# CZY-Code/PHNet

Hardware: AMD Instinct MI355X
Metric: clips/s (5x3x320x800) fwd+bwd (higher is better)
Workload: dtype f32 storage / accumulation, every product as an EXACT three-term bf16 split (6 bf16 MFMAs, f32-MFMA accuracy); 1 GPU; 5-frame clip 3x320x800, resnet34 + router + lane head, fwd+bwd+AdamW, 1 clip/GPU/step, random-init weights; parallelism=dp1, launch=hipGraph replay of the whole step

## Files before the change

include/phnet_hip.h:

```cpp
#ifndef PHNET_HIP_H
#define PHNET_HIP_H
#include <stdint.h>
#ifdef __cplusplus
extern "C" {
#endif

#define PHNET_OK 0
#define PHNET_ERR_ARG (-1)
#define PHNET_ERR_WORKSPACE (-2)
#define PHNET_ERR_LAUNCH (-3)
#define PHNET_ABI_VERSION 1

int phnet_abi_version(void);

int phnet_lane_nms(const float* rows, const float* scores, const int32_t* counts, int64_t frames,
                   int64_t k_max, int32_t n_offsets, float thresh, int64_t top_k,
                   int64_t* keep, int64_t* num_to_keep, int64_t* parent, void* stream);

int phnet_lane_decode(const float* lines, int64_t frames, int32_t N, int32_t n_offsets, float conf_thresh,
                      float nms_thresh, int64_t top_k, float img_w, uint8_t* keep_mask, int64_t* num,
                      int64_t* keep_c, int64_t* anchors, int64_t* anchors_sorted, float* kept_rows, void* stream);

int phnet_roi_pool_fwd(const float* fmap, const float* xs, const float* ys, float* out, float* out_cp,
                       int32_t B, int32_t N, int32_t P, int32_t h, int32_t w, int32_t C, void* stream);
int phnet_roi_pool_bwd(const float* dout, const float* fmap, const float* xs, const float* ys,
                       float* dmap, float* dxs,
                       int32_t B, int32_t N, int32_t P, int32_t h, int32_t w, int32_t C, void* stream);

int phnet_conv2d_fwd(const float* x, const float* w, const float* bias, float* y,
                     int32_t N, int32_t Hi, int32_t Wi, int32_t Ci, int32_t Co, int32_t R, int32_t S,
                     int32_t stride, int32_t pad, int32_t relu, void* workspace, uint64_t ws_bytes, void* stream);
uint64_t phnet_conv2d_stats_blocks(int64_t M, int32_t Co, int32_t K, uint64_t ws_bytes);
int phnet_conv2d_fwd_fused(const float* x, const float* w, const float* bias, const float* addend, float* y, float* stats,
                           int32_t N, int32_t Hi, int32_t Wi, int32_t Ci, int32_t Co, int32_t R, int32_t S,
                           int32_t stride, int32_t pad, int32_t relu, void* workspace, uint64_t ws_bytes, void* stream);
int phnet_conv2d_dgrad(const float* dy, const float* w, const float* addend, float* dx,
                       int32_t N, int32_t Hi, int32_t Wi, int32_t Ci, int32_t Co, int32_t R, int32_t S,
                       int32_t stride, int32_t pad, void* workspace, uint64_t ws_bytes, void* stream);
int phnet_conv3p_applies(int64_t M, int32_t Ca, int32_t Nn);
uint64_t phnet_conv3p_packed_bytes(int32_t Co, int32_t Ci);
int phnet_conv3p_pack(const float* w, void* packed, int32_t Co, int32_t Ci, int32_t dgrad, void* stream);
int phnet_conv3p_pack_jobs(const void* jobs, int32_t njobs, int64_t total, void* stream);
uint64_t phnet_conv3p_stats_blocks(int64_t M, int32_t Ca, int32_t Nn, uint64_t ws_bytes);
int phnet_conv3p_splits(int64_t M, int32_t Ca, int32_t Nn, uint64_t ws_bytes);
int phnet_conv3p_fwd(const float* x, const void* packed, const float* bias, const float* addend, float* y, float* stats,
                     int32_t N, int32_t H, int32_t W, int32_t Ca, int32_t Nn, int32_t relu,
                     void* workspace, uint64_t ws_bytes, void* stream);
int phnet_conv2d_plan(int64_t M, int32_t Co, int32_t K, uint64_t ws_bytes, int32_t* bm, int32_t* bn, int32_t* splits,
                      int32_t* k_tile);
uint64_t phnet_conv2d_wgrad_workspace(int32_t N, int32_t Hi, int32_t Wi, int32_t Ci, int32_t Co,
                                      int32_t R, int32_t S, int32_t stride, int32_t pad);
int phnet_conv2d_wgrad(const float* dy, const float* x, float* dw, float* dbias,
                       int32_t N, int32_t Hi, int32_t Wi, int32_t Ci, int32_t Co, int32_t R, int32_t S,
                       int32_t stride, int32_t pad, int32_t accumulate, void* workspace, uint64_t ws_bytes, void* stream);
int phnet_linear_bwd_fusable(int64_t M, int64_t K, int64_t N);
int phnet_linear_bwd(const float* dy, const float* x, const float* w, const float* relu_y, float* dx, float* dw, float* dbias,
                     int32_t M, int32_t K, int32_t N, int32_t accumulate, void* stream);
int phnet_nchw3_to_nhwc4(const float* x, float* y, int32_t N, int32_t H, int32_t W, void* stream);
int phnet_pad_channels(const float* src, float* dst, int64_t rows, int32_t cs, int32_t cd, void* stream);

uint64_t phnet_ipc_buffer_bytes(int32_t world, uint64_t max_bytes);
int phnet_ipc_alloc(uint64_t bytes, void** ptr);
int phnet_ipc_free(void* ptr);
int phnet_ipc_get_handle(void* ptr, void* handle64);
int phnet_ipc_open_handle(const void* handle64, void** ptr);
int phnet_ipc_close_handle(void* ptr);
int phnet_oneshot_allreduce(void* data, int32_t count, int32_t dtype, const void* peers, int32_t rank, int32_t world,
                            int32_t cap, void* ctrl, void* stream);

uint64_t phnet_channel_partials_size(int64_t M, int32_t C);
int phnet_bn_fwd_stats(const float* x, int64_t M, int32_t C, float eps, float momentum,
                       const float* gamma, const float* beta, float* running_mean, float* running_var,
                       float* save_mean, float* save_invstd, float* scale, float* shift,
                       float* partial, int32_t training, void* stream);
int phnet_bn_finalize_partials(const float* partial, int64_t nblk, int64_t M, int32_t C, float eps, float momentum,
                               const float* gamma, const float* beta, float* running_mean, float* running_var,
                               float* save_mean, float* save_invstd, float* scale, float* shift, void* stream);
int phnet_bn_apply(const float* x, const float* scale, const float* shift, const float* residual, float* y,
                   int64_t M, int32_t C, int32_t relu, void* stream);
int phnet_bn_bwd(const float* dy, const float* x, const float* y, const float* save_mean,
                 const float* save_invstd, const float* gamma, float* dx, float* dres,
                 float* dgamma, float* dbeta, float* partial, float* c1, float* c2,
                 int64_t M, int32_t C, int32_t relu, int32_t dres_accumulate, int32_t param_accumulate, void* stream);

int phnet_bn_bwd_reduce(const float* dy, const float* x, const float* y, const float* mean, const float* invstd,
                        float* sums, float* partial, float* c1_scratch, float* c2_scratch,
                        int64_t M, int32_t C, int32_t relu, void* stream);
int phnet_bn_bwd_apply(const float* dy, const float* x, const float* y, const float* mean, const float* invstd,
                       const float* gamma, const float* c1, const float* c2, float* dx, float* dres,
                       int64_t M, int32_t C, int32_t relu, int32_t dres_accumulate, void* stream);

int phnet_bn_local_sums(const float* x, int64_t M, int32_t C, float* partial, double* sums, void* stream);
int phnet_bn_partials_to_sums(const float* partial, int64_t nblk, int64_t M, int32_t C, double* sums, void* stream);
int phnet_bn_finalize_sums(const double* sums, int32_t C, float eps, float momentum, const float* gamma, const float* beta,
                           float* running_mean, float* running_var, float* save_mean, float* save_invstd,
                           float* scale, float* shift, void* stream);
int phnet_bn_bwd_apply_sums(const float* dy, const float* x, const float* y, const float* mean, const float* invstd,
                            const float* gamma, const float* sums, const double* count, float* c1, float* c2,
                            float* dx, float* dres, int64_t M, int32_t C, int32_t relu, int32_t dres_accumulate, void* stream);

int phnet_preprocess_u8(const uint8_t* frames, float* out, uint8_t* out_u8,
                        const int32_t* xi, const int16_t* xc, const int32_t* yi, const int16_t* yc,
                        int32_t T, int32_t H0, int32_t W0, int32_t crop_top, int32_t out_h, int32_t out_w, int32_t flip,
                        int32_t layout, const float* mean3_host, const float* std3_host, void* stream);

int phnet_lane_raster(const int32_t* segs, int64_t n_segs, uint32_t* masks, int32_t n_lanes, int32_t height, int32_t width,
                      int32_t lane_width, void* stream);
int phnet_lane_mask_stats(const uint32_t* masks, int32_t n_lanes, int32_t height, int32_t width, const int32_t* pairs,
                          int32_t n_pairs, int64_t* area, int64_t* inter, void* stream);

int phnet_maxpool3x3s2_fwd(const float* x, float* y, uint8_t* argmax, int32_t N, int32_t Hi, int32_t Wi, int32_t C, void* stream);
int phnet_maxpool3x3s2_bwd(const float* dy, const uint8_t* argmax, float* dx, int32_t N, int32_t Hi, int32_t Wi, int32_t C, void* stream);

int phnet_upsample_add(float* fine, const float* coarse, int32_t N, int32_t H, int32_t W, int32_t h, int32_t w, int32_t C, void* stream);
int phnet_upsample_add_bwd(const float* dfine, float* dcoarse, int32_t N, int32_t H, int32_t W, int32_t h, int32_t w, int32_t C, void* stream);

int phnet_layernorm_fwd(const float* x, const float* w, const float* b, const float* res, float* y,
                        float* mean, float* rstd, int64_t rows, int32_t L, float eps, int32_t relu, void* stream);
uint64_t phnet_layernorm_bwd_workspace(int64_t rows, int32_t L);
int phnet_layernorm_bwd(const float* dy, const float* x, const float* y, const float* w,
                        const float* mean, const float* rstd, float* dx, float* dres, float* dw, float* db,
                        int64_t rows, int32_t L, int32_t relu, int32_t param_accumulate,
                        void* workspace, uint64_t ws_bytes, void* stream);

int phnet_dwconv3x3(const float* x, const float* w, const float* bias, float* y,
                    int32_t N, int32_t C, int32_t P, int32_t flip, void* stream);
int phnet_dwconv3x3_wgrad(const float* dy, const float* x, float* dw, float* db,
                          int32_t N, int32_t C, int32_t P, int32_t accumulate, void* stream);

int phnet_lane_assign(const float* pred, const float* tgt, int32_t N, int32_t L, int32_t S,
                      float img_w, float img_h, int64_t* rows_by_col, int64_t* rows_sorted,
                      int32_t* n_valid, float* cost, void* stream);
int phnet_lane_assign_one2many(const float* pred, const float* tgt, int32_t N, int32_t L, int32_t S,
                               float img_w, float img_h, int64_t* rows, int64_t* cols, int32_t* n_pairs, void* stream);
int phnet_lane_assign_tokens(const float* pred, const float* tgt, int32_t N, int32_t L, int32_t S, float img_w, float img_h,
                             int64_t* rows_by_col, int64_t* rows_sorted, const float* feat, int32_t E,
                             float* tokens, uint8_t* valid, void* stream);

int phnet_frame_loss(const float* const* pred, const float* const* gate, const float* tgt,
                     int32_t N, int32_t L, int32_t S, float img_w, float img_h,
                     float cls_w, float reg_w, float iou_w,
                     float liou_half_width, float liou_img_h, float liou_img_w,
                     float* loss, float* const* dpred, float* dgate,
                     int64_t* rows_by_col, int64_t* rows_sorted, float* focal, float* scalars, void* stream);
int phnet_clip_loss(const float* const* pred, const float* const* gate, const float* tgt, int32_t T,
                    int32_t N, int32_t L, int32_t S, float img_w, float img_h,
                    float cls_w, float reg_w, float iou_w,
                    float liou_half_width, float liou_img_h, float liou_img_w,
                    float* loss, float* const* dpred, float* dgate,
                    int64_t* rows_by_col, int64_t* rows_sorted, float* focal, float* scalars, void* stream);
int phnet_frame_loss_variant(int32_t variant, const float* const* pred, const float* const* gate, const float* tgt,
                             int32_t N, int32_t L, int32_t S, float img_w, float img_h,
                             float cls_w, float reg_w, float iou_w,
                             float* loss, float* const* dpred, float* dgate,
                             int64_t* pair_rows, int64_t* pair_cols, int64_t* rows_sorted, float* scratch, void* stream);

int phnet_lane_update_fwd(const float* priors, const float* head, const float* ys, float* preds, float* lines,
                          int32_t N, int32_t S, int32_t HW, float img_w, float img_h, void* stream);
int phnet_lane_update_bwd(const float* dpreds, const float* dlines, const float* lines, const float* head,
                          const float* ys, float* dhead, float* dpriors,
                          int32_t N, int32_t S, int32_t HW, float img_w, float img_h, void* stream);

int phnet_relu_bwd(const float* dy, const float* y, float* dx, int64_t n, void* stream);

uint64_t phnet_gate_stack_saved_floats(int32_t N, int32_t C, int32_t P);
uint64_t phnet_gate_stack_bwd_workspace(int32_t N, int32_t C, int32_t P);
int phnet_gate_stack_fwd(const float* x, const float* const* params, float* out, float* saved,
                         int32_t N, int32_t anchors, int32_t C, int32_t P, float eps, void* stream);
int phnet_gate_stack_bwd(const float* gout, const float* x, const float* out, const float* const* params,
                         const float* saved, float* const* grads, int32_t N, int32_t anchors, int32_t C, int32_t P, float eps,
                         int32_t accumulate, void* workspace, uint64_t ws_bytes, void* stream);
int phnet_gate_wave_applies(int32_t C, int32_t P);
int phnet_gate_wave_partial_planes(int32_t N);
int phnet_gate_wave_fwd(const float* x, const float* const* params, float* out, float* saved,
                        int32_t N, int32_t anchors, float eps, void* stream);
int phnet_gate_wave_bwd(const float* gout, const float* x, const float* out, const float* const* params, const float* saved,
                        float* const* grads, int32_t N, int32_t anchors, float eps, int32_t accumulate,
                        void* workspace, void* stream);

int phnet_attention_fwd(const float* q, const float* k, const float* v, const uint8_t* key_valid, const uint8_t* keep,
                        float* o, float* lse, int32_t B, int32_t Lq, int32_t Lk, int32_t H, int32_t E,
                        int64_t sq, int64_t sk, int64_t sv, int64_t so, float keep_scale,
                        const uint64_t* rng_state, uint64_t rng_call, float drop_p, void* stream);
int phnet_attention_bwd(const float* q, const float* k, const float* v, const float* o, const float* dout,
                        const float* lse, const uint8_t* key_valid, const uint8_t* keep,
                        float* dq, float* dk, float* dv, int32_t B, int32_t Lq, int32_t Lk, int32_t H, int32_t E,
                        int64_t sq, int64_t sk, int64_t sv, int64_t so, int64_t sdq, int64_t sdk, int64_t sdv,
                        float keep_scale, const uint64_t* rng_state, uint64_t rng_call, float drop_p, void* stream);

int phnet_dropout_add(const float* x, const float* res, float* y, int64_t n,
                      const uint64_t* rng_state, uint64_t rng_call, float drop_p, void* stream);
int phnet_gelu_dropout_fwd(const float* x, float* y, int64_t n, const uint64_t* rng_state, uint64_t rng_call, float drop_p,
                           void* stream);
int phnet_gelu_dropout_bwd(const float* dy, const float* x, float* dx, int64_t n, const uint64_t* rng_state,
                           uint64_t rng_call, float drop_p, void* stream);

int phnet_memory_tokens(const float* feat, const int64_t* rows, float* tokens, uint8_t* valid,
                        int32_t B, int32_t N, int32_t E, int32_t L, void* stream);
int phnet_gate_tail_fwd(const float* h, const float* w, const float* b, float* out, int32_t N, int32_t K, void* stream);
int phnet_gate_tail_bwd(const float* dout, const float* out, const float* h, const float* w, float* dh, float* dw, float* db,
                        int32_t N, int32_t K, int32_t accumulate, void* stream);
int phnet_blend_priors(const float* gate, const float* a, const float* b, const int64_t* idx, float* priors, float* on_map,
                       int32_t N, int32_t W, int32_t P, void* stream);

int phnet_gate_v2_fwd(const float* x, const float* w1, const float* s1, const float* t1, const float* w2,
                      const float* s2, const float* t2, const float* wl, const float* bl, float* out,
                      int32_t M, int32_t C, int32_t P, int32_t C1, int32_t C2, void* stream);
int phnet_dyn_bmm_ln_relu_fwd_any(const float* x, const float* w, const float* gamma, const float* beta, float* y,
                                  int32_t N, int32_t P, int32_t K, int32_t J, float eps, void* stream);
int phnet_route_lines(const float* gates, const float* a, const float* b, float* out,
                      int32_t S, int32_t M, int32_t W, int32_t hard, void* stream);

int phnet_rowchain_fwd(const float* in, const float* resid, const float* Wa, const float* ba, const float* ln1w, const float* ln1b,
                       const float* W1, const float* b1, const float* W2, const float* b2, const float* ln2w, const float* ln2b,
                       const float* Wg, const float* bg, float* t_out, float* h_out, float* y_out,
                       int32_t R, int32_t E, int32_t FF, int32_t NG, float eps,
                       const uint64_t* rng_state, uint64_t call_a, uint64_t call_f, uint64_t call_3, float drop_p, void* stream);

uint64_t phnet_tower_layout(int32_t T, int32_t C, const int32_t* head_out, int64_t* offsets, int32_t* hw);
int phnet_assemble_towers(const float* const* params, int32_t T, int32_t C, const int32_t* head_out, float* dst, void* stream);
int phnet_scatter_tower_grads(const float* src, float* const* grads, int32_t T, int32_t C, const int32_t* head_out,
                              int32_t accumulate, void* stream);

int phnet_tower_chain_fwd(const float* x, const float* const* params, int32_t T, int32_t C, const int32_t* head_out,
                          const float* priors, const float* ys, float* preds, float* lines, int32_t R, int32_t S,
                          float img_w, float img_h, void* stream);

int phnet_adamw_step(float* p, const float* g, float* m, float* v, int64_t n, int64_t n_decay, const int64_t* step,
                     float lr, const float* lr_dev, float beta1, float beta2, float eps, float weight_decay, void* stream);

int phnet_dropout_add_ln_fwd(const float* x, const float* res, const float* w, const float* b, float* t, float* h,
                             float* mean, float* rstd, int64_t rows, int32_t L, float eps,
                             const uint64_t* rng_state, uint64_t rng_call, float drop_p, void* stream);
int phnet_dropout_add_ln_bwd(const float* dh, const float* dt, const float* t, const float* w, const float* mean,
                             const float* rstd, float* dres, float* dx, float* dw, float* db,
                             int64_t rows, int32_t L, int32_t param_accumulate,
                             const uint64_t* rng_state, uint64_t rng_call, float drop_p,
                             void* workspace, uint64_t ws_bytes, void* stream);

int phnet_dyn_bmm_ln_relu_fwd(const float* x, const float* w, const float* gamma, const float* beta, float* y,
                              float* stats, int32_t N, int32_t P, int32_t K, int32_t J, float eps, void* stream);
int phnet_dyn_bmm_ln_relu_bwd(const float* dy, const float* x, const float* w, const float* y, const float* stats,
                              const float* gamma, float* dx, float* dw, float* dgamma, float* dbeta,
                              int32_t N, int32_t P, int32_t K, int32_t J, float eps, int32_t param_accumulate,
                              void* workspace, uint64_t ws_bytes, void* stream);
int phnet_dyn_mfma_applies(int32_t P, int32_t K, int32_t J);
int phnet_dyn_mfma_fwd(const float* x, const float* w, const float* gamma, const float* beta, float* y, float* stats,
                       int32_t N, int32_t P, int32_t K, int32_t J, float eps, void* stream);
int phnet_dyn_mfma_bwd(const float* dy, const float* x, const float* w, const float* y, const float* stats, const float* gamma,
                       float* dx, float* dw, float* lnpart, int32_t N, int32_t P, int32_t K, int32_t J, void* stream);

uint64_t phnet_colsum_workspace(int64_t M, int32_t C);
int phnet_colsum(const float* a, float* out, int64_t M, int32_t C, int32_t accumulate, void* workspace, uint64_t ws_bytes, void* stream);

#ifdef __cplusplus
}
#endif
#endif
```

phnet_amd/csrc/conv.hip:

```cpp
#include <type_traits>
#include "igemm.h"
#include "wgrad3s.h"
static constexpr bool g_interleave = true;

using namespace igemm;

namespace {

struct ConvShape {
    int N, Hi, Wi, Ci;
    int Ho, Wo, Co;
    int R, S;
    int stride, pad, in_dil;
    int splits;
    int k_per_split;
};

struct RowCoord { int base, iy0, ix0; bool ok; };

template <int N, int I = 0, typename F>
__device__ __forceinline__ void unroll_iterations(F& f, int t) {
    if constexpr (I < N) {
        f(std::integral_constant<int, I>{}, t + I);
        unroll_iterations<N, I + 1>(f, t);
    }
}
template <int N, int I = 0, typename F>
__device__ __forceinline__ void tail_iterations(F& f, int t, int end) {
    if constexpr (I < N) {
        if (t + I < end) {
            f(std::integral_constant<int, I>{}, t + I);
            tail_iterations<N, I + 1>(f, t, end);
        }
    }
}

template <int BM, int BN, bool B_DGRAD, int BKT, bool UNI, bool AMASK = false, int MMA = 0, int PF = 1, bool BUF = false>
__device__ __forceinline__ void igemm_tile(
    const float* __restrict__ X, const float* __restrict__ W, const float* __restrict__ bias,
    const float* __restrict__ addend, float* __restrict__ out, const ConvShape& g, int relu,
    float* lds, unsigned block, unsigned nblocks, unsigned split, const float* __restrict__ amask = nullptr,
    float* __restrict__ stats = nullptr)
{
    constexpr int TM = BM / 2, TN = BN / 2, FM = TM / 32, FN = TN / 32;
    constexpr int A_PITCH = KContigTile<BM, BKT>::PITCH;
    constexpr int A_FLOATS = KContigTile<BM, BKT>::FLOATS;
    constexpr int B_PITCH = B_DGRAD ? KStridedTile<BN, BKT>::PITCH : KContigTile<BN, BKT>::PITCH;
    constexpr int B_FLOATS = B_DGRAD ? KStridedTile<BN, BKT>::FLOATS : KContigTile<BN, BKT>::FLOATS;
    constexpr int CHUNKS = BKT / 4;
    constexpr int ROWS_PER_PASS = THREADS / CHUNKS;
    constexpr int A_LOADS = BM / ROWS_PER_PASS;
    constexpr int B_LOADS = B_DGRAD ? (BKT * BN / 4) / THREADS : BN / ROWS_PER_PASS;
    float* As = lds;
    float* Bs = lds + 2 * A_FLOATS;
    constexpr bool S3 = MMA == 3;
    typedef KContigPlanes<BM, BKT> AP3;
    typedef KContigPlanes<BN, BKT> BP3C;
    typedef KStridedPlanes<BN, BKT> BP3S;
    constexpr int B3_BYTES = B_DGRAD ? BP3S::BYTES : BP3C::BYTES;
    unsigned char* A3 = reinterpret_cast<unsigned char*>(lds);
    unsigned char* B3 = A3 + 2 * AP3::BYTES;

    const int M = g.N * g.Ho * g.Wo;
    const int K = g.R * g.S * g.Ci;
    const int tiles_n = (g.Co + BN - 1) / BN;
    const unsigned tile = xcd_remap(block, nblocks);
    const int m0 = (int)(tile / tiles_n) * BM, n0 = (int)(tile % tiles_n) * BN;
    const int k_begin = split * g.k_per_split;
    const int k_end = min(K, k_begin + g.k_per_split);
    const int tid = threadIdx.x, lane = tid & 63, wave = tid >> 6;
    const int wm = (wave >> 1) * TM, wn = (wave & 1) * TN;

    RowCoord rc[A_LOADS];
    const int a_chunk = tid % CHUNKS, a_row = tid / CHUNKS;
#pragma unroll
    for (int i = 0; i < A_LOADS; ++i) {
        const int m = m0 + a_row + ROWS_PER_PASS * i;
        rc[i].ok = m < M;
        const int mm = rc[i].ok ? m : 0;
        const int n = mm / (g.Ho * g.Wo), rem = mm - n * (g.Ho * g.Wo);
        const int oy = rem / g.Wo, ox = rem - oy * g.Wo;
        rc[i].base = n * g.Hi * g.Wi;
        rc[i].iy0 = oy * g.stride - g.pad;
        rc[i].ix0 = ox * g.stride - g.pad;
    }

    struct KPos { int c, r, q; };
    auto kpos_init = [&](int k, int ci) {
        KPos p;
        const int rs = k / ci;
        p.c = k - rs * ci;
        p.r = rs / g.S;
        p.q = rs - p.r * g.S;
        return p;
    };
    auto kpos_advance = [&](KPos& p, int ci) {
        p.c += BKT;
        while (p.c >= ci) {
            p.c -= ci;
            if (++p.q == g.S) { p.q = 0; ++p.r; }
        }
    };
    KPos ka = kpos_init(k_begin + a_chunk * 4, g.Ci);
    KPos kb[B_LOADS];
    int b_kk[B_LOADS], b_ch[B_LOADS];
    if (B_DGRAD) {
#pragma unroll
        for (int i = 0; i < B_LOADS; ++i) {
            const int idx = tid + THREADS * i;
            b_kk[i] = idx / (BN / 4);
            b_ch[i] = idx - b_kk[i] * (BN / 4);
            kb[i] = kpos_init(k_begin + b_kk[i], g.Ci);
        }
    }

    constexpr bool uni = UNI;
    int ur = 0, uq = 0, uc0 = 0;
    if (uni) {
        const int rs = k_begin / g.Ci;
        uc0 = k_begin - rs * g.Ci;
        ur = rs / g.S;
        uq = rs - ur * g.S;
    }

    f32x4 a_set[PF][A_LOADS], b_set[PF][B_LOADS];
    f32x4 r_set[PF][AMASK ? A_LOADS : 1];
    unsigned mask_set[PF];
    constexpr unsigned OOB = 0x80000000u;
    int a_off[BUF ? A_LOADS : 1], b_off[BUF ? B_LOADS : 1];
    __amdgpu_buffer_rsrc_t x_rsrc, w_rsrc;
    if constexpr (BUF) {
        static_assert(UNI && !AMASK, "buffer-load path: uniform tap, no ReLU mask");
        x_rsrc = __builtin_amdgcn_make_buffer_rsrc((void*)X, 0, (int)min((long)g.N * g.Hi * g.Wi * g.Ci * 4, (long)0x7fffffff), 0x00020000);
        w_rsrc = __builtin_amdgcn_make_buffer_rsrc((void*)W, 0, (int)min((long)g.Co * K * 4, (long)0x7fffffff), 0x00020000);
#pragma unroll
        for (int i = 0; i < A_LOADS; ++i) {
            a_off[i] = ((rc[i].base + rc[i].iy0 * g.Wi + rc[i].ix0) * g.Ci + a_chunk * 4) * 4;
            if (!rc[i].ok) rc[i].iy0 = -(1 << 28);
        }
#pragma unroll
        for (int i = 0; i < B_LOADS; ++i) {
            if (!B_DGRAD) {
                const int n = n0 + a_row + ROWS_PER_PASS * i;
                b_off[i] = n < g.Co ? (n * K + a_chunk * 4) * 4 : (int)OOB;
            } else {
                const int n = n0 + b_ch[i] * 4;
                b_off[i] = n < g.Co ? (b_kk[i] * g.R * g.S * g.Co + n) * 4 : (int)OOB;
            }
        }
    }
    auto load_global = [&](int kt, f32x4 (&a_reg)[A_LOADS], f32x4 (&b_reg)[B_LOADS], f32x4 (&a_relu)[AMASK ? A_LOADS : 1], unsigned& mask) {
        mask = 0;
        if constexpr (BUF) {
            const bool tile_ok = kt < k_end;
            const int s_tap = ((ur * g.Wi + uq) * g.Ci + uc0) * 4;
#pragma unroll
            for (int i = 0; i < A_LOADS; ++i) {
                const bool ok = tile_ok && (unsigned)(rc[i].iy0 + ur) < (unsigned)g.Hi && (unsigned)(rc[i].ix0 + uq) < (unsigned)g.Wi;
                a_reg[i] = __builtin_bit_cast(f32x4, __builtin_amdgcn_raw_buffer_load_b128(x_rsrc, ok ? a_off[i] + s_tap : (int)OOB, 0, 0));
            }
            int s_b;
            if (!B_DGRAD) s_b = kt * 4;
            else s_b = ((uc0 * g.R + (g.R - 1 - ur)) * g.S + (g.S - 1 - uq)) * g.Co * 4;
#pragma unroll
            for (int i = 0; i < B_LOADS; ++i)
                b_reg[i] = __builtin_bit_cast(f32x4, __builtin_amdgcn_raw_buffer_load_b128(w_rsrc, tile_ok ? b_off[i] + s_b : (int)OOB, 0, 0));
            uc0 += BKT;
            const int wc = uc0 >= g.Ci;
            uc0 = wc ? 0 : uc0;
            uq += wc;
            const int wq = uq == g.S;
            uq = wq ? 0 : uq;
            ur += wq;
            return;
        }
        const int k0 = kt + a_chunk * 4;
        const bool kok = k0 < k_end;
        const int tap_r = uni ? ur : ka.r, tap_q = uni ? uq : ka.q, tap_c = uni ? uc0 + a_chunk * 4 : ka.c;
#pragma unroll
        for (int i = 0; i < A_LOADS; ++i) {
            int ty = rc[i].iy0 + tap_r, tx = rc[i].ix0 + tap_q;
            bool ok = kok && rc[i].ok && ty >= 0 && tx >= 0;
            if (g.in_dil == 2) {
                ok = ok && !((ty | tx) & 1);
                ty >>= 1; tx >>= 1;
            }
            ok = ok && ty < g.Hi && tx < g.Wi;
            const int pix = ok ? rc[i].base + ty * g.Wi + tx : 0;
            a_reg[i] = *reinterpret_cast<const f32x4*>(X + (size_t)pix * g.Ci + (kok ? tap_c : 0));
            if (AMASK) a_relu[i] = *reinterpret_cast<const f32x4*>(amask + (size_t)pix * g.Ci + (kok ? tap_c : 0));
            mask |= (unsigned)ok << i;
        }
        if (!uni) kpos_advance(ka, g.Ci);
        if (!B_DGRAD) {
#pragma unroll
            for (int i = 0; i < B_LOADS; ++i) {
                const int n = n0 + a_row + ROWS_PER_PASS * i;
                const bool ok = kok && n < g.Co;
                b_reg[i] = *reinterpret_cast<const f32x4*>(W + (size_t)(ok ? n : 0) * K + (kok ? k0 : 0));
                mask |= (unsigned)ok << (16 + i);
            }
        } else {
#pragma unroll
            for (int i = 0; i < B_LOADS; ++i) {
                const int k = kt + b_kk[i], n = n0 + b_ch[i] * 4;
                const bool ok = k < k_end && n < g.Co;
                const int wc = uni ? uc0 + b_kk[i] : kb[i].c, wr = uni ? ur : kb[i].r, wq = uni ? uq : kb[i].q;
                const int wrow = ok ? (wc * g.R + (g.R - 1 - wr)) * g.S + (g.S - 1 - wq) : 0;
                b_reg[i] = *reinterpret_cast<const f32x4*>(W + (size_t)wrow * g.Co + (ok ? n : 0));
                mask |= (unsigned)ok << (16 + i);
                if (!uni) kpos_advance(kb[i], g.Ci);
            }
        }
        if (uni) {
            uc0 += BKT;
            const int wc = uc0 >= g.Ci;
            uc0 = wc ? 0 : uc0;
            uq += wc;
            const int wq = uq == g.S;
            uq = wq ? 0 : uq;
            ur += wq;
        }
    };
    auto store_lds = [&](int buf, const f32x4 (&a_reg)[A_LOADS], const f32x4 (&b_reg)[B_LOADS], const f32x4 (&a_relu)[AMASK ? A_LOADS : 1],
                         unsigned mask) {
        float* a = As + buf * A_FLOATS;
        float* b = Bs + buf * B_FLOATS;
        unsigned char* a3 = A3 + buf * AP3::BYTES;
        unsigned char* b3 = B3 + buf * B3_BYTES;
        const f32x4 zero{0.f, 0.f, 0.f, 0.f};
#pragma unroll
        for (int i = 0; i < A_LOADS; ++i) {
            f32x4 v = BUF ? a_reg[i] : ((mask >> i) & 1u ? a_reg[i] : zero);
            if (AMASK) {
                v.x = a_relu[i].x > 0.f ? v.x : 0.f; v.y = a_relu[i].y > 0.f ? v.y : 0.f;
                v.z = a_relu[i].z > 0.f ? v.z : 0.f; v.w = a_relu[i].w > 0.f ? v.w : 0.f;
            }
            if (S3) store_split3<AP3::PLANE>(a3, (a_row + ROWS_PER_PASS * i) * AP3::PITCH + a_chunk * 8, v);
            else
            *reinterpret_cast<f32x4*>(a + (a_row + ROWS_PER_PASS * i) * A_PITCH + a_chunk * 4) = v;
        }
        if (!B_DGRAD) {
#pragma unroll
            for (int i = 0; i < B_LOADS; ++i) {
                const f32x4 v = BUF ? b_reg[i] : ((mask >> (16 + i)) & 1u ? b_reg[i] : zero);
                if (S3) store_split3<BP3C::PLANE>(b3, (a_row + ROWS_PER_PASS * i) * BP3C::PITCH + a_chunk * 8, v);
                else *reinterpret_cast<f32x4*>(b + (a_row + ROWS_PER_PASS * i) * B_PITCH + a_chunk * 4) = v;
            }
        } else {
#pragma unroll
            for (int i = 0; i < B_LOADS; ++i) {
                const f32x4 v = BUF ? b_reg[i] : ((mask >> (16 + i)) & 1u ? b_reg[i] : zero);
                if (S3) store_split3<BP3S::PLANE>(b3, b_kk[i] * BP3S::PITCH + b_ch[i] * 8, v);
                else *reinterpret_cast<f32x4*>(b + b_kk[i] * B_PITCH + b_ch[i] * 4) = v;
            }
        }
    };

    const bool final_pass = g.splits == 1;
    f32x16 acc[FM][FN];
#pragma unroll
    for (int j = 0; j < FN; ++j) {
        const int n = n0 + wn + j * 32 + frag_col(lane);
        const bool nok = n < g.Co;
        const float bv = (final_pass && bias && nok) ? bias[n] : 0.f;
#pragma unroll
        for (int i = 0; i < FM; ++i)
#pragma unroll
            for (int e = 0; e < 16; ++e) {
                const int m = m0 + wm + i * 32 + frag_row(lane, e);
                const bool ok = final_pass && addend && nok && m < M;
                acc[i][j][e] = bv + (ok ? addend[(size_t)(ok ? m : 0) * g.Co + (ok ? n : 0)] : 0.f);
            }
    }

    auto multiply_tile = [&](int buf, int kt) {
        if (S3) {
#pragma unroll
            for (int ks = 0; ks < BKT / BK; ++ks) {
                Frag3 a[FM], b[FN];
                read_kcontig3<FM, AP3::PITCH, AP3::PLANE>(A3 + buf * AP3::BYTES + wm * AP3::PITCH, lane, ks, a);
                if (!B_DGRAD) read_kcontig3<FN, BP3C::PITCH, BP3C::PLANE>(B3 + buf * B3_BYTES + wn * BP3C::PITCH, lane, ks, b);
                else read_kstrided3<FN, BP3S::PITCH, BP3S::PLANE>(B3 + buf * B3_BYTES + wn * 2, lane, ks, b);
                mma3_step<FM, FN>(a, b, acc);
            }
            return;
        }
#pragma unroll
        for (int ks = 0; ks < BKT / BK; ++ks) {
            if (BKT > BK && kt + ks * BK >= k_end) break;
            float a[FM][8], b[FN][8];
            read_kcontig<FM, A_PITCH>(As + buf * A_FLOATS + wm * A_PITCH, lane, ks, a);
            if (!B_DGRAD) read_kcontig<FN, B_PITCH>(Bs + buf * B_FLOATS + wn * B_PITCH, lane, ks, b);
            else read_kstrided<FN, B_PITCH>(Bs + buf * B_FLOATS + wn, lane, ks, b);
            mma_any<S3 ? 0 : MMA, FM, FN>(a, b, acc);
        }
    };

    if (k_begin < k_end) {
        const int ntiles = (k_end - k_begin + BKT - 1) / BKT;
#pragma unroll
        for (int d = 0; d < PF; ++d) load_global(k_begin + d * BKT, a_set[d], b_set[d], r_set[d], mask_set[d]);
        store_lds(0, a_set[0], b_set[0], r_set[0], mask_set[0]);
        __syncthreads();
        int buf = 0;
        auto iteration = [&](auto U, int tt) {
            constexpr int u = decltype(U)::value;
            load_global(k_begin + (tt + PF) * BKT, a_set[u], b_set[u], r_set[u], mask_set[u]);
            multiply_tile(buf, k_begin + tt * BKT);
            if (PF == 1) __builtin_amdgcn_sched_barrier(0);
            constexpr int v = (u + 1) % PF;
            store_lds(buf ^ 1, a_set[v], b_set[v], r_set[v], mask_set[v]);
            if (PF > 1 && S3 && g_interleave) {
#pragma unroll
                for (int i = 0; i < 6 * FM * FN * (BKT / BK); ++i) {
                    __builtin_amdgcn_sched_group_barrier(0x008, 1, 0);
                    __builtin_amdgcn_sched_group_barrier(0x002, (14 + FM * FN - 1) / (FM * FN), 0);
                }
            }
            __syncthreads();
            buf ^= 1;
        };
        int t = 0;
        for (; t + PF <= ntiles; t += PF) unroll_iterations<PF>(iteration, t);
        if (PF > 1) tail_iterations<PF - 1>(iteration, t, ntiles);
    }

    if (stats != nullptr && final_pass) {
#pragma unroll
        for (int j = 0; j < FN; ++j) {
            const int n = n0 + wn + j * 32 + frag_col(lane);
#pragma unroll
            for (int i = 0; i < FM; ++i) {
                float sm = 0.f, sq = 0.f;
#pragma unroll
                for (int e = 0; e < 16; ++e) { const float v = acc[i][j][e]; sm += v; sq += v * v; }
                sm += __shfl_xor(sm, 32, 64);
                sq += __shfl_xor(sq, 32, 64);
                if (lane < 32 && n < g.Co) {
                    float* p = stats + (size_t)((m0 + wm + i * 32) >> 5) * 2 * g.Co;
                    p[n] = sm;
                    p[g.Co + n] = sq;
                }
            }
        }
    }

    float* dst = out + (size_t)split * M * g.Co;
#pragma unroll
    for (int j = 0; j < FN; ++j) {
        const int n = n0 + wn + j * 32 + frag_col(lane);
        if (n >= g.Co) continue;
#pragma unroll
        for (int i = 0; i < FM; ++i)
#pragma unroll
            for (int e = 0; e < 16; ++e) {
                const int m = m0 + wm + i * 32 + frag_row(lane, e);
                if (m < M) dst[(size_t)m * g.Co + n] = (final_pass && relu) ? fmaxf(acc[i][j][e], 0.f) : acc[i][j][e];
            }
    }
}

template <int BM, int BN, bool B_DGRAD, int BKT, bool UNI, int MMA = 0, int PF = 1, bool BUF = false>
__global__ __launch_bounds__(THREADS) void conv_igemm_kernel(
    const float* __restrict__ X, const float* __restrict__ W, const float* __restrict__ bias,
    const float* __restrict__ addend, float* __restrict__ out, ConvShape g, int relu, float* __restrict__ stats)
{
    extern __shared__ __attribute__((aligned(16))) float lds[];
    igemm_tile<BM, BN, B_DGRAD, BKT, UNI, false, MMA, PF, BUF>(X, W, bias, addend, out, g, relu, lds, blockIdx.x, gridDim.x, blockIdx.z,
                                                               nullptr, stats);
}

constexpr int T3_AROWS = 66;
int g_taps3 = 1;
template <bool DGRAD>
__global__ __launch_bounds__(THREADS) void conv3x3s1_kernel(
    const float* __restrict__ X, const float* __restrict__ Wt, const float* __restrict__ bias,
    const float* __restrict__ addend, float* __restrict__ out, ConvShape g, int relu, float* __restrict__ stats)
{
    constexpr int APITCH = KContigPlanes<64, 16>::PITCH;
    constexpr int APLANE = T3_AROWS * APITCH, AIMG = 3 * APLANE;
    typedef KContigPlanes<64, 16> BP3C;
    typedef KStridedPlanes<64, 16> BP3S;
    constexpr int BIMG = DGRAD ? BP3S::BYTES : BP3C::BYTES;
    constexpr int BPLANE = DGRAD ? BP3S::PLANE : BP3C::PLANE;
    extern __shared__ __attribute__((aligned(16))) float lds[];
    unsigned char* A3 = reinterpret_cast<unsigned char*>(lds);
    unsigned char* B3 = A3 + 2 * AIMG;
    unsigned char* dump = B3 + 2 * BIMG;

    const int W = g.Wi, H = g.Hi, Ca = g.Ci;
    const int M = g.N * H * W, K = 9 * Ca;
    const int CC = Ca >> 4;
    const int tiles_n = (g.Co + 63) >> 6;
    const unsigned tile = xcd_remap(blockIdx.x, gridDim.x);
    const int m0 = (int)(tile / tiles_n) * 64, n0 = (int)(tile % tiles_n) * 64;
    const int u_begin = blockIdx.z * g.k_per_split, u_end = min(3 * CC, u_begin + g.k_per_split);
    const int tid = threadIdx.x, lane = tid & 63, wave = tid >> 6;
    const int wm = (wave >> 1) * 32, wn = (wave & 1) * 32;

    constexpr unsigned OOB = 0x80000000u;
    __amdgpu_buffer_rsrc_t x_rsrc = __builtin_amdgcn_make_buffer_rsrc((void*)X, 0, (int)min((long)M * Ca * 4, (long)0x7fffffff), 0x00020000);
    __amdgpu_buffer_rsrc_t w_rsrc = __builtin_amdgcn_make_buffer_rsrc((void*)Wt, 0, (int)min((long)g.Co * K * 4, (long)0x7fffffff), 0x00020000);
    int a_off[2], a_ok[2], a_lds[2];
#pragma unroll
    for (int i = 0; i < 2; ++i) {
        const int idx = tid + 256 * i, row = idx >> 2, chunk = idx & 3;
        const bool rowok = idx < 4 * T3_AROWS;
        const int t = m0 - 1 + row;
        const bool tok = rowok && (unsigned)t < (unsigned)M;
        const int tt = tok ? t : 0;
        const int y = (tt / W) % H;
        a_ok[i] = (tok && y >= 1 ? 1 : 0) | (tok ? 2 : 0) | (tok && y + 1 < H ? 4 : 0);
        a_off[i] = (t * Ca + chunk * 4) * 4;
        a_lds[i] = rowok ? row * APITCH + chunk * 8 : -1;
    }
    const int a_row = tid >> 2, a_chunk = tid & 3;
    const int b_kk = tid >> 4, b_ch = tid & 15;
    int b_off, b_lds;
    if (!DGRAD) {
        const int n = n0 + a_row;
        b_off = n < g.Co ? (n * K + a_chunk * 4) * 4 : (int)OOB;
        b_lds = a_row * BP3C::PITCH + a_chunk * 8;
    } else {
        const int n = n0 + b_ch * 4;
        b_off = n < g.Co ? (b_kk * 9 * g.Co + n) * 4 : (int)OOB;
        b_lds = b_kk * BP3S::PITCH + b_ch * 8;
    }
    int la_dy = u_begin / CC, la_cc = u_begin - la_dy * CC, la_u = u_begin;
    int lb_dy = la_dy, lb_cc = la_cc, lb_u = u_begin, lb_dx = 0;
    const bool wave0 = __builtin_amdgcn_readfirstlane(wave) == 0;
    auto load_a = [&](f32x4 (&reg)[2]) {
        const bool uok = la_u < u_end;
        const int s_a = ((la_dy - 1) * W * Ca + la_cc * 16) * 4;
        {
            const bool ok = uok && ((a_ok[0] >> la_dy) & 1);
            reg[0] = __builtin_bit_cast(f32x4, __builtin_amdgcn_raw_buffer_load_b128(x_rsrc, ok ? a_off[0] + s_a : (int)OOB, 0, 0));
        }
        if (wave0) {
            const bool ok = uok && ((a_ok[1] >> la_dy) & 1);
            reg[1] = __builtin_bit_cast(f32x4, __builtin_amdgcn_raw_buffer_load_b128(x_rsrc, ok ? a_off[1] + s_a : (int)OOB, 0, 0));
        }
        ++la_u; ++la_cc;
        const int wrap = la_cc == CC;
        la_cc = wrap ? 0 : la_cc;
        la_dy += wrap;
    };
    auto load_b = [&](f32x4& reg) {
        const bool uok = lb_u < u_end;
        const int s_b = !DGRAD ? ((lb_dy * 3 + lb_dx) * Ca + lb_cc * 16) * 4
                               : ((lb_cc * 16 * 3 + (2 - lb_dy)) * 3 + (2 - lb_dx)) * g.Co * 4;
        reg = __builtin_bit_cast(f32x4, __builtin_amdgcn_raw_buffer_load_b128(w_rsrc, uok ? b_off + s_b : (int)OOB, 0, 0));
        ++lb_dx;
        const int w3 = lb_dx == 3;
        lb_dx = w3 ? 0 : lb_dx;
        lb_u += w3; lb_cc += w3;
        const int wrap = lb_cc == CC;
        lb_cc = wrap ? 0 : lb_cc;
        lb_dy += wrap;
    };
    auto store_a = [&](int aoff, const f32x4 (&reg)[2]) {
        store_split3<APLANE>(A3 + aoff, a_lds[0], reg[0]);
        if (wave0) {
            unsigned h0, m0_, l0, h1, m1, l1;
            split3_pair(reg[1].x, reg[1].y, h0, m0_, l0);
            split3_pair(reg[1].z, reg[1].w, h1, m1, l1);
            const bool has = a_lds[1] >= 0;
            unsigned char* q = has ? A3 + aoff + a_lds[1] : dump + lane * 8;
            const int ps = has ? APLANE : 512;
            *reinterpret_cast<u32x2*>(q) = (u32x2){h0, h1};
            *reinterpret_cast<u32x2*>(q + ps) = (u32x2){m0_, m1};
            *reinterpret_cast<u32x2*>(q + 2 * ps) = (u32x2){l0, l1};
        }
    };
    auto store_b = [&](int boff, const f32x4& reg) { store_split3<BPLANE>(B3 + boff, b_lds, reg); };

    const bool final_pass = g.splits == 1;
    f32x16 acc[1][1];
    {
        const int n = n0 + wn + frag_col(lane);
        const bool nok = n < g.Co;
        const float bv = (final_pass && bias && nok) ? bias[n] : 0.f;
#pragma unroll
        for (int e = 0; e < 16; ++e) {
            const int m = m0 + wm + frag_row(lane, e);
            const bool ok = final_pass && addend && nok && m < M;
            acc[0][0][e] = bv + (ok ? addend[(size_t)(ok ? m : 0) * g.Co + (ok ? n : 0)] : 0.f);
        }
    }
    const int pr = m0 + wm + (lane & 31);
    const int px = (pr < M ? pr : 0) % W;
    const bool edge_l = px == 0, edge_r = px == W - 1;
    const bool any_l = __builtin_amdgcn_ballot_w64(edge_l) != 0, any_r = __builtin_amdgcn_ballot_w64(edge_r) != 0;

    if (u_begin < u_end) {
        f32x4 a_reg[2], b_set[3];
        load_a(a_reg);
#pragma unroll
        for (int d = 0; d < 3; ++d) load_b(b_set[d]);
        store_a(0, a_reg);
        load_a(a_reg);
        store_b(0, b_set[0]);
        load_b(b_set[0]);
        __syncthreads();
        int aoff = 0, boff = 0;
        const int r = lane & 31, hb = (lane >> 5) * 16;
        auto step = [&](auto DX) {
            constexpr int dxi = decltype(DX)::value;
            {
                Frag3 a[1], b[1];
                {
                    const unsigned char* p = A3 + aoff + (wm + r + dxi) * APITCH + hb;
                    a[0].hi = *reinterpret_cast<const bf16x8*>(p);
                    a[0].mid = *reinterpret_cast<const bf16x8*>(p + APLANE);
                    a[0].lo = *reinterpret_cast<const bf16x8*>(p + 2 * APLANE);
                }
                if (!DGRAD) read_kcontig3<1, BP3C::PITCH, BP3C::PLANE>(B3 + boff + wn * BP3C::PITCH, lane, 0, b);
                else read_kstrided3<1, BP3S::PITCH, BP3S::PLANE>(B3 + boff + wn * 2, lane, 0, b);
                if (dxi != 1 && (dxi == 0 ? any_l : any_r)) {
                    const bool z = dxi == 0 ? edge_l : edge_r;
                    typedef unsigned u32x4 __attribute__((ext_vector_type(4)));
                    const u32x4 keep = z ? (u32x4){0u, 0u, 0u, 0u} : (u32x4){~0u, ~0u, ~0u, ~0u};
                    a[0].hi = __builtin_bit_cast(bf16x8, __builtin_bit_cast(u32x4, a[0].hi) & keep);
                    a[0].mid = __builtin_bit_cast(bf16x8, __builtin_bit_cast(u32x4, a[0].mid) & keep);
                    a[0].lo = __builtin_bit_cast(bf16x8, __builtin_bit_cast(u32x4, a[0].lo) & keep);
                }
                mma3_step<1, 1>(a, b, acc);
                store_b(boff ^ BIMG, b_set[(dxi + 1) % 3]);
                load_b(b_set[(dxi + 1) % 3]);
                if (dxi == 2) {
                    store_a(aoff ^ AIMG, a_reg);
                    load_a(a_reg);
                }
#pragma unroll
                for (int i = 0; i < 6; ++i) {
                    __builtin_amdgcn_sched_group_barrier(0x008, 1, 0);
                    __builtin_amdgcn_sched_group_barrier(0x002, dxi == 2 ? 14 : 8, 0);
                }
                __syncthreads();
                boff ^= BIMG;
            }
        };
        for (int u = u_begin; u < u_end; ++u) {
            step(std::integral_constant<int, 0>{});
            step(std::integral_constant<int, 1>{});
            step(std::integral_constant<int, 2>{});
            aoff ^= AIMG;
        }
    }

    if (stats != nullptr && final_pass) {
        const int n = n0 + wn + frag_col(lane);
        float sm = 0.f, sq = 0.f;
#pragma unroll
        for (int e = 0; e < 16; ++e) { const float v = acc[0][0][e]; sm += v; sq += v * v; }
        sm += __shfl_xor(sm, 32, 64);
        sq += __shfl_xor(sq, 32, 64);
        if (lane < 32 && n < g.Co) {
            float* p = stats + (size_t)((m0 + wm) >> 5) * 2 * g.Co;
            p[n] = sm;
            p[g.Co + n] = sq;
        }
    }
    float* dst = out + (size_t)blockIdx.z * M * g.Co;
    const int n = n0 + wn + frag_col(lane);
    if (n < g.Co) {
#pragma unroll
        for (int e = 0; e < 16; ++e) {
            const int m = m0 + wm + frag_row(lane, e);
            if (m < M) dst[(size_t)m * g.Co + n] = (final_pass && relu) ? fmaxf(acc[0][0][e], 0.f) : acc[0][0][e];
        }
    }
}

__global__ __launch_bounds__(256) void splitk_reduce_kernel(const float* __restrict__ part, float* __restrict__ out,
                                                            const float* __restrict__ bias, const float* __restrict__ addend,
                                                            long total4, int ncols, int splits, int relu, int accumulate,
                                                            float* __restrict__ stats)
{
    __shared__ f32x4 red_s[2][256];
    const long i = (long)blockIdx.x * blockDim.x + threadIdx.x;
    if (stats != nullptr) {
        const bool ok = i < total4;
        f32x4 s{0.f, 0.f, 0.f, 0.f};
        if (ok) {
            const f32x4* p = reinterpret_cast<const f32x4*>(part) + i;
            s = p[0];
            for (int z = 1; z < splits; ++z) s += p[(long)z * total4];
            reinterpret_cast<f32x4*>(out)[i] = s;
        }
        red_s[0][threadIdx.x] = s;
        red_s[1][threadIdx.x] = s * s;
        __syncthreads();
        const int c4 = ncols >> 2;
        if ((int)threadIdx.x < c4) {
            f32x4 a = red_s[0][threadIdx.x], b = red_s[1][threadIdx.x];
            for (int r = c4; r < 256; r += c4) { a += red_s[0][r + threadIdx.x]; b += red_s[1][r + threadIdx.x]; }
            float* q = stats + (size_t)blockIdx.x * 2 * ncols + threadIdx.x * 4;
            *reinterpret_cast<f32x4*>(q) = a;
            *reinterpret_cast<f32x4*>(q + ncols) = b;
        }
        return;
    }
    if (i >= total4) return;
    const f32x4* p = reinterpret_cast<const f32x4*>(part) + i;
    const f32x4 zero{0.f, 0.f, 0.f, 0.f};
    f32x4 v[8];
#pragma unroll
    for (int z = 0; z < 8; ++z) v[z] = p[(long)min(z, splits - 1) * total4];
    const f32x4 bv = bias ? *reinterpret_cast<const f32x4*>(bias + (int)((i * 4) % ncols)) : zero;
    const f32x4 av = addend ? reinterpret_cast<const f32x4*>(addend)[i] : zero;
    const f32x4 ov = accumulate ? reinterpret_cast<const f32x4*>(out)[i] : zero;
    f32x4 s = v[0];
#pragma unroll
    for (int z = 1; z < 8; ++z)
        if (z < splits) s += v[z];
    for (int z = 8; z < splits; ++z) s += p[(long)z * total4];
    if (bias) s += bv;
    if (addend) s += av;
    if (relu) { s.x = fmaxf(s.x, 0.f); s.y = fmaxf(s.y, 0.f); s.z = fmaxf(s.z, 0.f); s.w = fmaxf(s.w, 0.f); }
    if (accumulate) s += ov;
    reinterpret_cast<f32x4*>(out)[i] = s;
}

struct WgradShape {
    int N, Hi, Wi, Ci;
    int Ho, Wo, Co;
    int R, S, stride, pad;
    int splits, pix_per_split;
};

template <int BM, int BN, int MMA = 0, int BKW = BK, int PF = 1, bool BUF = false>
__global__ __launch_bounds__(THREADS) void conv_wgrad_kernel(
    const float* __restrict__ dY, const float* __restrict__ X, float* __restrict__ out, float* __restrict__ dbias,
    WgradShape g, int want_bias, int accumulate)
{
    constexpr int TM = BM / 2, TN = BN / 2, FM = TM / 32, FN = TN / 32;
    constexpr int A_PITCH = KStridedTile<BM, BKW>::PITCH, B_PITCH = KStridedTile<BN, BKW>::PITCH;
    constexpr int A_FLOATS = KStridedTile<BM, BKW>::FLOATS, B_FLOATS = KStridedTile<BN, BKW>::FLOATS;
    constexpr int A_LOADS = BKW * BM / 4 / THREADS, B_LOADS = BKW * BN / 4 / THREADS;
    constexpr bool S3 = MMA == 3;
    typedef KStridedPlanes<BM, BKW> AP3;
    typedef KStridedPlanes<BN, BKW> BP3;
    constexpr int LDS_BYTES = S3 ? 2 * (AP3::BYTES + BP3::BYTES) : 2 * (A_FLOATS + B_FLOATS) * 4;
    __shared__ __attribute__((aligned(16))) unsigned char lds_raw[LDS_BYTES];
    float* lds = reinterpret_cast<float*>(lds_raw);
    float* As = lds;
    float* Bs = lds + 2 * A_FLOATS;
    unsigned char* A3 = lds_raw;
    unsigned char* B3 = lds_raw + 2 * AP3::BYTES;

    const int NC = g.R * g.S * g.Ci;
    const int P = g.N * g.Ho * g.Wo;
    const int tiles_n = (NC + BN - 1) / BN;
    const unsigned tile = xcd_remap(blockIdx.x, gridDim.x);
    const int m0 = (int)(tile / tiles_n) * BM, n0 = (int)(tile % tiles_n) * BN;
    const int p_begin = blockIdx.z * g.pix_per_split, p_end = min(P, p_begin + g.pix_per_split);
    const int tid = threadIdx.x, lane = tid & 63, wave = tid >> 6;
    const int wm = (wave >> 1) * TM, wn = (wave & 1) * TN;

    int b_kk[B_LOADS], b_col[B_LOADS], b_r[B_LOADS], b_q[B_LOADS], b_c[B_LOADS];
    bool b_ok[B_LOADS];
#pragma unroll
    for (int i = 0; i < B_LOADS; ++i) {
        const int idx = tid + THREADS * i;
        b_kk[i] = idx / (BN / 4);
        b_col[i] = (idx - b_kk[i] * (BN / 4)) * 4;
        const int col = n0 + b_col[i];
        b_ok[i] = col < NC;
        const int rs = b_ok[i] ? col / g.Ci : 0;
        b_c[i] = col - rs * g.Ci;
        b_r[i] = rs / g.S;
        b_q[i] = rs - b_r[i] * g.S;
    }

    int b_n[B_LOADS], b_oy[B_LOADS], b_ox[B_LOADS];
#pragma unroll
    for (int i = 0; i < B_LOADS; ++i) {
        const int pp = min(p_begin + b_kk[i], max(P - 1, 0));
        b_n[i] = pp / (g.Ho * g.Wo);
        const int rem = pp - b_n[i] * (g.Ho * g.Wo);
        b_oy[i] = rem / g.Wo;
        b_ox[i] = rem - b_oy[i] * g.Wo;
    }
    int a_kk[A_LOADS], a_ch[A_LOADS];
#pragma unroll
    for (int i = 0; i < A_LOADS; ++i) {
        const int idx = tid + THREADS * i;
        a_kk[i] = idx / (BM / 4);
        a_ch[i] = (idx - a_kk[i] * (BM / 4)) * 4;
    }

    f32x4 a_set[PF][A_LOADS], b_set[PF][B_LOADS], bsum[A_LOADS];
    unsigned m_set[PF];
#pragma unroll
    for (int i = 0; i < A_LOADS; ++i) bsum[i] = f32x4{0.f, 0.f, 0.f, 0.f};
    constexpr unsigned OOB = 0x80000000u;
    __amdgpu_buffer_rsrc_t y_rsrc, x_rsrc;
    int a_off[BUF ? A_LOADS : 1];
    float inv_wo = 0.f, inv_ho = 0.f;
    if constexpr (BUF) {
        y_rsrc = __builtin_amdgcn_make_buffer_rsrc((void*)dY, 0, (int)min((long)P * g.Co * 4, (long)0x7fffffff), 0x00020000);
        x_rsrc = __builtin_amdgcn_make_buffer_rsrc((void*)X, 0, (int)min((long)g.N * g.Hi * g.Wi * g.Ci * 4, (long)0x7fffffff), 0x00020000);
#pragma unroll
        for (int i = 0; i < A_LOADS; ++i) a_off[i] = m0 + a_ch[i] < g.Co ? (a_kk[i] * g.Co + m0 + a_ch[i]) * 4 : (int)OOB;
        inv_wo = 1.0f / (float)g.Wo; inv_ho = 1.0f / (float)g.Ho;
    }
    const bool bias_block = want_bias && n0 == 0;
    auto load_global = [&](int pt, bool advance, f32x4 (&a_reg)[A_LOADS], f32x4 (&b_reg)[B_LOADS], unsigned& lmask) {
        lmask = 0;
        if (advance) {
#pragma unroll
            for (int i = 0; i < B_LOADS; ++i) {
                if constexpr (BUF) {
                    int ox = b_ox[i] + BKW;
                    int w = (int)((float)ox * inv_wo);
                    ox -= w * g.Wo;
                    const int lo = ox < 0, hi = ox >= g.Wo;
                    ox += lo ? g.Wo : 0; ox -= hi ? g.Wo : 0; w += hi - lo;
                    int oy = b_oy[i] + w;
                    int v = (int)((float)oy * inv_ho);
                    oy -= v * g.Ho;
                    const int lo2 = oy < 0, hi2 = oy >= g.Ho;
                    oy += lo2 ? g.Ho : 0; oy -= hi2 ? g.Ho : 0; v += hi2 - lo2;
                    b_ox[i] = ox; b_oy[i] = oy; b_n[i] += v;
                } else {
                    b_ox[i] += BKW;
                    while (b_ox[i] >= g.Wo) {
                        b_ox[i] -= g.Wo;
                        if (++b_oy[i] == g.Ho) { b_oy[i] = 0; ++b_n[i]; }
                    }
                }
            }
        }
        if constexpr (BUF) {
            const int s_a = pt * g.Co * 4;
#pragma unroll
            for (int i = 0; i < A_LOADS; ++i) {
                const bool ok = pt + a_kk[i] < p_end;
                a_reg[i] = __builtin_bit_cast(f32x4, __builtin_amdgcn_raw_buffer_load_b128(y_rsrc, ok ? a_off[i] + s_a : (int)OOB, 0, 0));
            }
#pragma unroll
            for (int i = 0; i < B_LOADS; ++i) {
                const int iy = b_oy[i] * g.stride - g.pad + b_r[i], ix = b_ox[i] * g.stride - g.pad + b_q[i];
                const bool ok = b_ok[i] && pt + b_kk[i] < p_end && (unsigned)iy < (unsigned)g.Hi && (unsigned)ix < (unsigned)g.Wi;
                const int off = (((b_n[i] * g.Hi + iy) * g.Wi + ix) * g.Ci + b_c[i]) * 4;
                b_reg[i] = __builtin_bit_cast(f32x4, __builtin_amdgcn_raw_buffer_load_b128(x_rsrc, ok ? off : (int)OOB, 0, 0));
            }
            return;
        }
#pragma unroll
        for (int i = 0; i < A_LOADS; ++i) {
            const int p = pt + a_kk[i], co = m0 + a_ch[i];
            const bool ok = p < p_end && co < g.Co;
            a_reg[i] = *reinterpret_cast<const f32x4*>(dY + (ok ? (size_t)p * g.Co + co : 0));
            lmask |= (unsigned)ok << i;
        }
#pragma unroll
        for (int i = 0; i < B_LOADS; ++i) {
            const int p = pt + b_kk[i];
            const int iy = b_oy[i] * g.stride - g.pad + b_r[i], ix = b_ox[i] * g.stride - g.pad + b_q[i];
            const bool ok = b_ok[i] && p < p_end && iy >= 0 && iy < g.Hi && ix >= 0 && ix < g.Wi;
            const int pix = ok ? (b_n[i] * g.Hi + iy) * g.Wi + ix : 0;
            b_reg[i] = *reinterpret_cast<const f32x4*>(X + (size_t)pix * g.Ci + (ok ? b_c[i] : 0));
            lmask |= (unsigned)ok << (16 + i);
        }
    };
    auto store_lds = [&](int buf, const f32x4 (&a_reg)[A_LOADS], const f32x4 (&b_reg)[B_LOADS], unsigned lmask) {
        const f32x4 zero{0.f, 0.f, 0.f, 0.f};
#pragma unroll
        for (int i = 0; i < A_LOADS; ++i) {
            const f32x4 v = BUF ? a_reg[i] : ((lmask >> i) & 1u ? a_reg[i] : zero);
            if (bias_block) bsum[i] += v;
            if (S3) store_split3<AP3::PLANE>(A3 + buf * AP3::BYTES, a_kk[i] * AP3::PITCH + a_ch[i] * 2, v);
            else *reinterpret_cast<f32x4*>(As + buf * A_FLOATS + a_kk[i] * A_PITCH + a_ch[i]) = v;
        }
#pragma unroll
        for (int i = 0; i < B_LOADS; ++i) {
            const f32x4 v = BUF ? b_reg[i] : ((lmask >> (16 + i)) & 1u ? b_reg[i] : zero);
            if (S3) store_split3<BP3::PLANE>(B3 + buf * BP3::BYTES, b_kk[i] * BP3::PITCH + b_col[i] * 2, v);
            else *reinterpret_cast<f32x4*>(Bs + buf * B_FLOATS + b_kk[i] * B_PITCH + b_col[i]) = v;
        }
    };

    const bool from_old = g.splits == 1 && accumulate;
    f32x16 acc[FM][FN];
#pragma unroll
    for (int i = 0; i < FM; ++i)
#pragma unroll
        for (int j = 0; j < FN; ++j)
#pragma unroll
            for (int e = 0; e < 16; ++e) {
                const int n = n0 + wn + j * 32 + frag_col(lane), m = m0 + wm + i * 32 + frag_row(lane, e);
                const bool ok = from_old && n < NC && m < g.Co;
                const float v = out[ok ? (size_t)m * NC + n : 0];
                acc[i][j][e] = ok ? v : 0.f;
            }

    if (p_begin < p_end) {
        const int nsteps = (p_end - p_begin + BKW - 1) / BKW;
#pragma unroll
        for (int d = 0; d < PF; ++d) load_global(p_begin + d * BKW, d > 0, a_set[d], b_set[d], m_set[d]);
        store_lds(0, a_set[0], b_set[0], m_set[0]);
        __syncthreads();
        int buf = 0;
        auto iteration = [&](auto U, int tt) {
            constexpr int u = decltype(U)::value;
            load_global(p_begin + (tt + PF) * BKW, true, a_set[u], b_set[u], m_set[u]);
#pragma unroll
            for (int ks = 0; ks < BKW / BK; ++ks) {
                if (S3) {
                    Frag3 a[FM], b[FN];
                    read_kstrided3<FM, AP3::PITCH, AP3::PLANE>(A3 + buf * AP3::BYTES + wm * 2, lane, ks, a);
                    read_kstrided3<FN, BP3::PITCH, BP3::PLANE>(B3 + buf * BP3::BYTES + wn * 2, lane, ks, b);
                    mma3_step<FM, FN>(a, b, acc);
                } else {
                    float a[FM][8], b[FN][8];
                    read_kstrided<FM, A_PITCH>(As + buf * A_FLOATS + wm, lane, ks, a);
                    read_kstrided<FN, B_PITCH>(Bs + buf * B_FLOATS + wn, lane, ks, b);
                    mma_any<S3 ? 0 : MMA, FM, FN>(a, b, acc);
                }
            }
            if (PF == 1) __builtin_amdgcn_sched_barrier(0);
            constexpr int v = (u + 1) % PF;
            store_lds(buf ^ 1, a_set[v], b_set[v], m_set[v]);
            if (PF > 1 && S3 && g_interleave) {
#pragma unroll
                for (int i = 0; i < 6 * FM * FN * (BKW / BK); ++i) {
                    __builtin_amdgcn_sched_group_barrier(0x008, 1, 0);
                    __builtin_amdgcn_sched_group_barrier(0x002, (14 + FM * FN - 1) / (FM * FN), 0);
                }
            }
            __syncthreads();
            buf ^= 1;
        };
        int t = 0;
        for (; t + PF <= nsteps; t += PF) unroll_iterations<PF>(iteration, t);
        if (PF > 1) tail_iterations<PF - 1>(iteration, t, nsteps);
    }
    const bool direct = g.splits == 1;
    float* dst = direct ? out : out + (size_t)blockIdx.z * ((size_t)g.Co * NC + g.Co);
#pragma unroll
    for (int j = 0; j < FN; ++j) {
        const int n = n0 + wn + j * 32 + frag_col(lane);
        if (n >= NC) continue;
#pragma unroll
        for (int i = 0; i < FM; ++i)
#pragma unroll
            for (int e = 0; e < 16; ++e) {
                const int m = m0 + wm + i * 32 + frag_row(lane, e);
                if (m < g.Co) {
                    float* q = dst + (size_t)m * NC + n;
                    *q = acc[i][j][e];
                }
            }
    }
    if (bias_block) {
        __syncthreads();
#pragma unroll
        for (int i = 0; i < A_LOADS; ++i)
            *reinterpret_cast<f32x4*>(As + a_kk[i] * A_PITCH + a_ch[i]) = bsum[i];
        __syncthreads();
        if (tid < BM && m0 + tid < g.Co) {
            float t = 0.f;
#pragma unroll
            for (int k = 0; k < BKW; ++k) t += As[k * A_PITCH + tid];
            if (direct) dbias[m0 + tid] = accumulate ? dbias[m0 + tid] + t : t;
            else dst[(size_t)g.Co * NC + m0 + tid] = t;
        }
    }
}

constexpr int W3_THREADS = 768;
int g_wgrad3 = 1, g_wgrad3_target = 256;
int g_wgrad3_bkw = 16;
// ... 109 lines not shown
            read_kstrided3<1, PITCH, PLANE>(b_src + buf_off, lane, ks, b1);
        };
        const int h8 = (lane >> 5) * 8;
        auto mask_edge = [&](Frag3& a, int ke) {
            const int j = ke - h8;
            const int ji = j >> 1;
            const unsigned wmask = (j & 1) ? 0x0000ffffu : 0xffff0000u;
            typedef unsigned u32x4 __attribute__((ext_vector_type(4)));
            u32x4 m;
            m.x = ji == 0 ? wmask : 0xffffffffu; m.y = ji == 1 ? wmask : 0xffffffffu;
            m.z = ji == 2 ? wmask : 0xffffffffu; m.w = ji == 3 ? wmask : 0xffffffffu;
            a.hi = __builtin_bit_cast(bf16x8, __builtin_bit_cast(u32x4, a.hi) & m);
            a.mid = __builtin_bit_cast(bf16x8, __builtin_bit_cast(u32x4, a.mid) & m);
            a.lo = __builtin_bit_cast(bf16x8, __builtin_bit_cast(u32x4, a.lo) & m);
        };
        read_frags(0, 0, fa[0], fb[0]);
        int o_cur = 0, o_nxt = 2 * IMG, o_st = 4 * IMG;
        auto iteration = [&](auto U, int tt) {
            constexpr int u = decltype(U)::value;
            constexpr int slot = (u + 2) % PF;
#pragma unroll
            for (int ks = 0; ks < NSUB; ++ks) {
                const int cur = (u * NSUB + ks) & 1, nxt = cur ^ 1;
                {
                    const int ke = dx < 0 ? (mx == 0 ? 0 : W - mx) : W - 1 - mx;
                    if (dx != 0 && ke < BK) mask_edge(fa[cur], ke);
                    mx += BK;
                    mx -= mx >= W ? W : 0;
                }
                if (ks + 1 < NSUB) read_frags(o_cur, ks + 1, fa[nxt], fb[nxt]);
                else read_frags(o_nxt, 0, fa[nxt], fb[nxt]);
                Frag3 (&a)[1] = *reinterpret_cast<Frag3 (*)[1]>(&fa[cur]);
                Frag3 (&b)[1] = *reinterpret_cast<Frag3 (*)[1]>(&fb[cur]);
                mma3_step<1, 1>(a, b, acc);
            }
            store_lds(o_st, set[slot]);
            load_global(p_begin + (tt + 2 + PF) * BKW, set[slot]);
#pragma unroll
            for (int i = 0; i < 6; ++i) {
                __builtin_amdgcn_sched_group_barrier(0x008, 1, 0);
                __builtin_amdgcn_sched_group_barrier(0x002, 8, 0);
            }
            __syncthreads();
            const int o = o_cur; o_cur = o_nxt; o_nxt = o_st; o_st = o;
        };
        int t = 0;
        for (; t + PF <= nsteps; t += PF) unroll_iterations<PF>(iteration, t);
        if (PF > 1) tail_iterations<PF - 1>(iteration, t, nsteps);
    }
    const bool direct = g.splits == 1;
    float* dst = direct ? out : out + (size_t)blockIdx.z * ((size_t)g.Co * NC + g.Co);
#pragma unroll
    for (int e = 0; e < 16; ++e)
        dst[(size_t)(m0 + wm + frag_row(lane, e)) * NC + n_base + frag_col(lane)] = acc[0][0][e];
    if (bias_block) {
        float* fold = reinterpret_cast<float*>(lds_raw);
        __syncthreads();
        if (role_a) *reinterpret_cast<f32x4*>(fold + kk * 68 + col) = bsum;
        __syncthreads();
        if (tid < 64) {
            float tsum = 0.f;
#pragma unroll
            for (int k = 0; k < BK; ++k) tsum += fold[k * 68 + tid];
            if (direct) dbias[m0 + tid] = accumulate ? dbias[m0 + tid] + tsum : tsum;
            else dst[(size_t)g.Co * NC + m0 + tid] = tsum;
        }
    }
}

constexpr int SMALLP_MAX = 256;
template <int BM, int BN, bool AMASK = false, int MMA = 0>
__device__ __forceinline__ void smallp_tile(
    const float* __restrict__ dY, const float* __restrict__ X, float* __restrict__ dw, float* __restrict__ dbias,
    int P, int Co, int Ci, int want_bias, int accumulate, float* lds, unsigned block, unsigned nblocks,
    const float* __restrict__ ymask = nullptr)
{
    constexpr int TM = BM / 2, TN = BN / 2, FM = TM / 32, FN = TN / 32;
    constexpr int AP = BM + 4, BP = BN + 4;
    constexpr int A_CH = BM / 4, B_CH = BN / 4;
    constexpr int A_LOADS = SMALLP_MAX * A_CH / THREADS, B_LOADS = SMALLP_MAX * B_CH / THREADS;
    const int P16 = (P + 15) & ~15;
    float* As = lds;
    float* Bs = lds + P16 * AP;
    const int tiles_n = (Ci + BN - 1) / BN;
    const unsigned tile = xcd_remap(block, nblocks);
    const int m0 = (int)(tile / tiles_n) * BM, n0 = (int)(tile % tiles_n) * BN;
    const int tid = threadIdx.x, lane = tid & 63, wave = tid >> 6;
    const int wm = (wave >> 1) * TM, wn = (wave & 1) * TN;

    f32x4 ar[A_LOADS], br[B_LOADS], ay[AMASK ? A_LOADS : 1];
    unsigned am = 0, bm = 0;
#pragma unroll
    for (int i = 0; i < A_LOADS; ++i) {
        const int idx = tid + THREADS * i, p = idx / A_CH, m = m0 + (idx - p * A_CH) * 4;
        const bool ok = p < P && m < Co;
        ar[i] = *reinterpret_cast<const f32x4*>(dY + (ok ? (size_t)p * Co + m : 0));
        if (AMASK) ay[i] = *reinterpret_cast<const f32x4*>(ymask + (ok ? (size_t)p * Co + m : 0));
        am |= (unsigned)ok << i;
    }
#pragma unroll
    for (int i = 0; i < B_LOADS; ++i) {
        const int idx = tid + THREADS * i, p = idx / B_CH, n = n0 + (idx - p * B_CH) * 4;
        const bool ok = p < P && n < Ci;
        br[i] = *reinterpret_cast<const f32x4*>(X + (ok ? (size_t)p * Ci + n : 0));
        bm |= (unsigned)ok << i;
    }
    f32x16 acc[FM][FN];
#pragma unroll
    for (int j = 0; j < FN; ++j)
#pragma unroll
        for (int i = 0; i < FM; ++i)
#pragma unroll
            for (int e = 0; e < 16; ++e) {
                const int n = n0 + wn + j * 32 + frag_col(lane), m = m0 + wm + i * 32 + frag_row(lane, e);
                acc[i][j][e] = (accumulate && n < Ci && m < Co) ? dw[(size_t)m * Ci + n] : 0.f;
            }
    const f32x4 zero{0.f, 0.f, 0.f, 0.f};
#pragma unroll
    for (int i = 0; i < A_LOADS; ++i) {
        const int idx = tid + THREADS * i, p = idx / A_CH;
        f32x4 v = (am >> i) & 1u ? ar[i] : zero;
        if (AMASK) {
            v.x = ay[i].x > 0.f ? v.x : 0.f; v.y = ay[i].y > 0.f ? v.y : 0.f;
            v.z = ay[i].z > 0.f ? v.z : 0.f; v.w = ay[i].w > 0.f ? v.w : 0.f;
        }
        if (p < P16) *reinterpret_cast<f32x4*>(As + p * AP + (idx - p * A_CH) * 4) = v;
    }
#pragma unroll
    for (int i = 0; i < B_LOADS; ++i) {
        const int idx = tid + THREADS * i, p = idx / B_CH;
        if (p < P16) *reinterpret_cast<f32x4*>(Bs + p * BP + (idx - p * B_CH) * 4) = (bm >> i) & 1u ? br[i] : zero;
    }
    __syncthreads();

    for (int ks = 0; ks < P16 / BK; ++ks) {
        float a[FM][8], b[FN][8];
        read_kstrided<FM, AP>(As + wm, lane, ks, a);
        read_kstrided<FN, BP>(Bs + wn, lane, ks, b);
        mma_any<MMA, FM, FN>(a, b, acc);
    }
#pragma unroll
    for (int j = 0; j < FN; ++j) {
        const int n = n0 + wn + j * 32 + frag_col(lane);
        if (n >= Ci) continue;
#pragma unroll
        for (int i = 0; i < FM; ++i)
#pragma unroll
            for (int e = 0; e < 16; ++e) {
                const int m = m0 + wm + i * 32 + frag_row(lane, e);
                if (m < Co) dw[(size_t)m * Ci + n] = acc[i][j][e];
            }
    }
    if (want_bias && n0 == 0) {
        static_assert(BM == 64, "bias fold assumes 64 columns x 4 row groups");
        const int c = tid & 63, grp = tid >> 6;
        float t = 0.f;
#pragma unroll 4
        for (int p = grp; p < P16; p += 4) t += As[p * AP + c];
        __syncthreads();
        Bs[grp * 64 + c] = t;
        __syncthreads();
        if (tid < 64 && m0 + tid < Co) {
            const float v = (Bs[tid] + Bs[64 + tid]) + (Bs[128 + tid] + Bs[192 + tid]);
            dbias[m0 + tid] = accumulate ? dbias[m0 + tid] + v : v;
        }
    }
}

template <int BM, int BN, int MMA = 0>
__global__ __launch_bounds__(THREADS) void linear_wgrad_smallp_kernel(
    const float* __restrict__ dY, const float* __restrict__ X, float* __restrict__ dw, float* __restrict__ dbias,
    int P, int Co, int Ci, int want_bias, int accumulate)
{
    extern __shared__ __attribute__((aligned(16))) float lds[];
    smallp_tile<BM, BN, false, MMA>(dY, X, dw, dbias, P, Co, Ci, want_bias, accumulate, lds, blockIdx.x, gridDim.x);
}

template <bool UNI, bool AMASK, int MMA = 0>
__global__ __launch_bounds__(THREADS) void linear_bwd_fused_kernel(
    const float* __restrict__ dY, const float* __restrict__ W, const float* __restrict__ X, const float* __restrict__ ymask,
    float* __restrict__ dX, float* __restrict__ dw, float* __restrict__ dbias,
    ConvShape gd, unsigned dgrad_tiles, int P, int Co, int Ci, int want_bias, int accumulate)
{
    extern __shared__ __attribute__((aligned(16))) float lds[];
    if (blockIdx.x < dgrad_tiles)
        igemm_tile<64, 64, true, 64, UNI, AMASK, MMA>(dY, W, nullptr, nullptr, dX, gd, 0, lds, blockIdx.x, dgrad_tiles, 0, ymask);
    else
        smallp_tile<64, 64, AMASK, MMA>(dY, X, dw, dbias, P, Co, Ci, want_bias, accumulate, lds, blockIdx.x - dgrad_tiles,
                                   gridDim.x - dgrad_tiles, ymask);
}

__global__ __launch_bounds__(256) void wgrad_reduce_kernel(const float* __restrict__ part, float* __restrict__ dw,
                                                           float* __restrict__ dbias, long nw, long nb, int splits, int accumulate)
{
    __shared__ f32x4 red[3][64];
    const int lane = threadIdx.x & 63, zg = threadIdx.x >> 6;
    const long total4 = (nw + nb) >> 2;
    const long i4 = (long)blockIdx.x * 64 + lane;
    const bool ok = i4 < total4;
    const long i = i4 * 4;
    const bool is_w = i < nw;
    const bool writer = zg == 0 && ok && (is_w || dbias);
    const f32x4 zero{0.f, 0.f, 0.f, 0.f};
    f32x4 old = zero;
    if (writer && accumulate) {
        if (is_w) old = *reinterpret_cast<const f32x4*>(dw + i);
        else { const float* b = dbias + (i - nw); old = f32x4{b[0], b[1], b[2], b[3]}; }
    }
    const f32x4* p = reinterpret_cast<const f32x4*>(part) + (ok ? i4 : 0);
    f32x4 s = zero;
    int z = zg;
    for (; z + 12 < splits; z += 16) {
        const f32x4 v0 = p[(long)z * total4], v1 = p[(long)(z + 4) * total4], v2 = p[(long)(z + 8) * total4],
                    v3 = p[(long)(z + 12) * total4];
        s += v0; s += v1; s += v2; s += v3;
    }
    for (; z < splits; z += 4) s += p[(long)z * total4];
    if (zg) red[zg - 1][lane] = s;
    __syncthreads();
    if (writer) {
        const f32x4 t = old + ((s + red[0][lane]) + (red[1][lane] + red[2][lane]));
        if (is_w) *reinterpret_cast<f32x4*>(dw + i) = t;
        else { float* b = dbias + (i - nw); b[0] = t.x; b[1] = t.y; b[2] = t.z; b[3] = t.w; }
    }
}

__global__ void nchw3_to_nhwc4_kernel(const float* __restrict__ x, float* __restrict__ y, int N, int HW)
{
    const long i = (long)blockIdx.x * blockDim.x + threadIdx.x;
    if (i >= (long)N * HW) return;
    const long n = i / HW, p = i - n * HW;
    const float* s = x + n * 3 * (long)HW + p;
    reinterpret_cast<f32x4*>(y)[i] = f32x4{s[0], s[HW], s[2 * (long)HW], 0.f};
}

__global__ void pad_channels_kernel(const float* __restrict__ src, float* __restrict__ dst, long rows, int cs, int cd)
{
    const long i = (long)blockIdx.x * blockDim.x + threadIdx.x;
    if (i >= rows * cd) return;
    const long r = i / cd;
    const int c = (int)(i - r * cd);
    dst[i] = c < cs ? src[r * cs + c] : 0.f;
}

struct TileChoice { int bm, bn; };

int g_mma_mode = 3;
int g_buf_loads = 1;
int g_pf = 4;
int g_deep_kt3 = 64;

TileChoice pick_tile(long M, long N)
{
    if (g_mma_mode == 3 && M <= 2048) return {64, 64};
    if (g_mma_mode >= 1) {
        if (N >= 128 && ceil_div64(M, 128) * ceil_div64(N, 128) >= 300) return {128, 128};
        if (ceil_div64(M, 128) * ceil_div64(N, 64) >= 1250) return {128, 64};
    }
    return {64, 64};
}

struct ConvPlan { int bm, bn, splits; long tiles; };

int k_tile_for(long M, int K, int ci, int bm, int bn)
{
    if (M <= (g_mma_mode == 3 ? 256 : 2048) && K >= 64) return (g_mma_mode == 3 && g_deep_kt3 == 32) ? 32 : 64;
    if (g_mma_mode == 3) return BK;
    if (g_mma_mode >= 1 && bm == 64 && bn == 64 && ci % 32 == 0) return 32;
    return BK;
}

int g_force_bm = 0, g_force_bn = 0, g_force_splits = 0;
int g_force_kt = 0;
int g_uniform_tap = 1;
int g_wgrad_bm128 = 1, g_wgrad_target = 768;
int g_wgrad_bkw = 16;
int g_wgrad_smallp = 1;
int g_smallp_max_tiles = 400;

ConvPlan plan_conv(long M, int Co, int K, bool has_ws, size_t ws_bytes)
{
    TileChoice t = pick_tile(M, Co);
    if (g_force_bm) {
        t = {g_force_bm, g_force_bn};
        ConvPlan f{t.bm, t.bn, 1, ceil_div64(M, t.bm) * ceil_div64(Co, t.bn)};
        int splits = g_force_splits > 0 ? g_force_splits : 1;
        while (splits > 1 && (!has_ws || (size_t)splits * M * Co * sizeof(float) > ws_bytes)) --splits;
        f.splits = splits;
        return f;
    }
    ConvPlan p{t.bm, t.bn, 1, ceil_div64(M, t.bm) * ceil_div64(Co, t.bn)};
    const bool deep = M <= (g_mma_mode == 3 ? 256 : 2048) && K >= 64;
    if (has_ws && p.tiles < (deep ? 400 : 900)) {
        int splits = (int)min((long)8, max((long)1, (1250 + p.tiles / 2) / p.tiles));
        while (splits > 1 && K / splits < 256) --splits;
        while (splits > 1 && (size_t)splits * M * Co * sizeof(float) > ws_bytes) --splits;
        p.splits = splits;
    }
    return p;
}

template <bool DGRAD>
int launch_conv(const float* X, const float* W, const float* bias, const float* addend, float* out, float* workspace,
                size_t ws_bytes, ConvShape g, int relu, hipStream_t st, float* stats = nullptr)
{
    const long M = (long)g.N * g.Ho * g.Wo;
    const int K = g.R * g.S * g.Ci;
    const ConvPlan t = plan_conv(M, g.Co, K, workspace != nullptr, ws_bytes);
    const long tiles = t.tiles;
    const int splits = t.splits;
    g.splits = splits;
    float* dst = splits > 1 ? workspace : out;
    dim3 grid((unsigned)tiles, 1, (unsigned)splits);
    const int bkt = g_force_kt ? g_force_kt : k_tile_for(M, K, g.Ci, t.bm, t.bn);
    const int ksteps = (K + bkt - 1) / bkt;
    g.k_per_split = ((ksteps + splits - 1) / splits) * bkt;
#define PHNET_LAUNCH_CONV___(BM_, BN_, BKT_, UNI_, MMA_, PF_)                                                           \
    do {                                                                                                                \
        if (UNI_ && g.in_dil == 1 && g_buf_loads && MMA_ == 3) PHNET_LAUNCH_CONV____(BM_, BN_, BKT_, UNI_, MMA_, PF_, UNI_); \
        else PHNET_LAUNCH_CONV____(BM_, BN_, BKT_, UNI_, MMA_, PF_, false);                                             \
    } while (0)
#define PHNET_LAUNCH_CONV____(BM_, BN_, BKT_, UNI_, MMA_, PF_, BUF_)                                                    \
    do {                                                                                                                \
        constexpr size_t lds_ = MMA_ == 3                                                                               \
            ? 2 * (size_t)(KContigPlanes<BM_, BKT_>::BYTES +                                                            \
                           (DGRAD ? KStridedPlanes<BN_, BKT_>::BYTES : KContigPlanes<BN_, BKT_>::BYTES))                \
            : 2 * (size_t)(KContigTile<BM_, BKT_>::FLOATS +                                                             \
                           (DGRAD ? KStridedTile<BN_, BKT_>::FLOATS : KContigTile<BN_, BKT_>::FLOATS)) * 4;             \
        static bool attr_set_ = false;                                                                                  \
        if (lds_ > 64 * 1024 && !attr_set_) {                                                                           \
            (void)hipFuncSetAttribute((const void*)conv_igemm_kernel<BM_, BN_, DGRAD, BKT_, UNI_, MMA_, PF_, BUF_>,     \
                                hipFuncAttributeMaxDynamicSharedMemorySize, (int)lds_);                                 \
            attr_set_ = true;                                                                                           \
        }                                                                                                               \
        hipLaunchKernelGGL((conv_igemm_kernel<BM_, BN_, DGRAD, BKT_, UNI_, MMA_, PF_, BUF_>), grid, dim3(THREADS), lds_, st, \
                           X, W, bias, addend, dst, g, relu, splits > 1 ? (float*)nullptr : stats);                     \
    } while (0)
#define PHNET_LAUNCH_CONV__(BM_, BN_, BKT_, UNI_, MMA_) PHNET_LAUNCH_CONV___(BM_, BN_, BKT_, UNI_, MMA_, 1)
#define PHNET_LAUNCH_CONV_(BM_, BN_, BKT_, UNI_)                                                                        \
    do {                                                                                                                \
        if (g_mma_mode == 1) PHNET_LAUNCH_CONV__(BM_, BN_, BKT_, UNI_, 1);                                              \
        else if (g_mma_mode == 2) PHNET_LAUNCH_CONV__(BM_, BN_, BKT_, UNI_, 2);                                         \
        else if (g_mma_mode == 3 && g_pf == 4) PHNET_LAUNCH_CONV___(BM_, BN_, BKT_, UNI_, 3, 4);                        \
        else if (g_mma_mode == 3 && g_pf == 2) PHNET_LAUNCH_CONV___(BM_, BN_, BKT_, UNI_, 3, 2);                        \
        else if (g_mma_mode == 3) PHNET_LAUNCH_CONV___(BM_, BN_, BKT_, UNI_, 3, 1);                                     \
        else if (g_pf == 4) PHNET_LAUNCH_CONV___(BM_, BN_, BKT_, UNI_, 0, 4);                                           \
        else PHNET_LAUNCH_CONV__(BM_, BN_, BKT_, UNI_, 0);                                                              \
    } while (0)
#define PHNET_LAUNCH_CONV(BM_, BN_, UNI_)                                                                               \
    do {                                                                                                                \
        if (bkt == 64) PHNET_LAUNCH_CONV_(BM_, BN_, 64, UNI_);                                                          \
        else if (bkt == 32) PHNET_LAUNCH_CONV_(BM_, BN_, 32, UNI_);                                                     \
        else PHNET_LAUNCH_CONV_(BM_, BN_, 16, UNI_);                                                                    \
    } while (0)
    const bool uni = (g.Ci % bkt) == 0 && g_uniform_tap;
    if (g_taps3 && uni && g.R == 3 && g.S == 3 && g.stride == 1 && g.pad == 1 && g.in_dil == 1 && g.Ho == g.Hi && g.Wo == g.Wi &&
        t.bm == 64 && t.bn == 64 && bkt == 16 && g_mma_mode == 3 && g_buf_loads && g_pf == 4 && g.Wi >= 2 &&
        M * (long)g.Ci * 4 < 0x7fffffffL && (long)g.Co * K * 4 < 0x7fffffffL) {
        const int units = 3 * (g.Ci / 16);
        g.k_per_split = (units + splits - 1) / splits;
        constexpr size_t lds_ = 2 * 3 * T3_AROWS * KContigPlanes<64, 16>::PITCH +
                                2 * (size_t)(DGRAD ? KStridedPlanes<64, 16>::BYTES : KContigPlanes<64, 16>::BYTES) + 3 * 512;
        hipLaunchKernelGGL((conv3x3s1_kernel<DGRAD>), grid, dim3(THREADS), lds_, st,
                           X, W, bias, addend, dst, g, relu, splits > 1 ? (float*)nullptr : stats);
    } else
    {
    if (t.bm == 128 && t.bn == 128) PHNET_LAUNCH_CONV(128, 128, false);
    else if (t.bm == 128 && t.bn == 64) PHNET_LAUNCH_CONV(128, 64, false);
    else if (t.bm == 64 && t.bn == 128) PHNET_LAUNCH_CONV(64, 128, false);
    else if (uni) PHNET_LAUNCH_CONV(64, 64, true);
    else PHNET_LAUNCH_CONV(64, 64, false);
    }
#undef PHNET_LAUNCH_CONV____
#undef PHNET_LAUNCH_CONV___
#undef PHNET_LAUNCH_CONV__
#undef PHNET_LAUNCH_CONV_
#undef PHNET_LAUNCH_CONV
    if (splits > 1) {
        const long total4 = M * g.Co / 4;
        hipLaunchKernelGGL(splitk_reduce_kernel, dim3((unsigned)ceil_div64(total4, 256)), dim3(256), 0, st,
                           workspace, out, bias, addend, total4, g.Co, splits, relu, 0, stats);
    }
    return phnet_launch_status();
}

}

PHNET_API int phnet_conv2d_plan(int64_t M, int32_t Co, int32_t K, uint64_t ws_bytes, int32_t* bm, int32_t* bn, int32_t* splits,
                                int32_t* k_tile)
{
    if (M < 1 || Co < 1 || K < 1 || !bm || !bn || !splits || !k_tile) return PHNET_ERR_ARG;
    const ConvPlan p = plan_conv((long)M, Co, K, ws_bytes > 0, (size_t)ws_bytes);
    *bm = p.bm; *bn = p.bn; *splits = p.splits;
    *k_tile = g_force_kt ? g_force_kt : k_tile_for((long)M, K, K, p.bm, p.bn);
    return PHNET_OK;
}

PHNET_API int phnet_tune_force_conv_tile(int32_t bm, int32_t bn, int32_t splits)
{
    if (bm != 0 && !((bm == 64 || bm == 128) && (bn == 64 || bn == 128))) return PHNET_ERR_ARG;
    g_force_bm = bm; g_force_bn = bn; g_force_splits = splits;
    return PHNET_OK;
}

PHNET_API int phnet_tune_wgrad(int32_t allow_bm128, int32_t target_blocks)
{
    if (target_blocks == 0 || target_blocks < -1024) return PHNET_ERR_ARG;
    g_wgrad_bm128 = allow_bm128 & 1; g_wgrad_smallp = !(allow_bm128 & 2); g_wgrad_bkw = (allow_bm128 & 4) ? 32 : 16;
    g_wgrad3 = !(allow_bm128 & 8);
    g_wgrad3_bkw = (allow_bm128 & 16) ? 32 : 16;
    g_wgrad3s = !(allow_bm128 & 32);
    g_wgrad1s = !(allow_bm128 & 64);
    if (target_blocks < 0) g_wgrad3_target = -target_blocks;
    else g_wgrad_target = target_blocks;
    return PHNET_OK;
}


PHNET_API int phnet_tune_mma(int32_t mode)
{
    if (mode < 0 || mode > 3) return PHNET_ERR_ARG;
    g_mma_mode = mode;
    g_pf = mode == 3 ? 4 : 1;
    return PHNET_OK;
}

PHNET_API int phnet_tune_force_k_tile(int32_t kt)
{
    if (kt == -1 || kt == -2) { g_uniform_tap = kt == -2; return PHNET_OK; }
    if (kt == -5 || kt == -6) { g_taps3 = kt == -6; return PHNET_OK; }
    if (kt == -32 || kt == -64) { g_deep_kt3 = -kt; return PHNET_OK; }
    if (kt == -101 || kt == -102 || kt == -104) { g_pf = -kt - 100; return PHNET_OK; }
    if (kt == -200 || kt == -201) { g_buf_loads = -kt - 200; return PHNET_OK; }
    if (kt != 0 && kt != 16 && kt != 32 && kt != 64) return PHNET_ERR_ARG;
    g_force_kt = kt;
    return PHNET_OK;
}

PHNET_API int phnet_conv2d_fwd(const float* x, const float* w, const float* bias, float* y,
                               int32_t N, int32_t Hi, int32_t Wi, int32_t Ci, int32_t Co, int32_t R, int32_t S,
                               int32_t stride, int32_t pad, int32_t relu,
                               void* workspace, uint64_t ws_bytes, void* stream)
{
    if (N < 0 || Hi < 1 || Wi < 1 || Ci < 4 || Co < 4 || (Ci & 3) || (Co & 3) || R < 1 || S < 1 || stride < 1 || pad < 0)
        return PHNET_ERR_ARG;
    if (N == 0) return PHNET_OK;
    if (!x || !w || !y) return PHNET_ERR_ARG;
    ConvShape g{};
    g.N = N; g.Hi = Hi; g.Wi = Wi; g.Ci = Ci; g.Co = Co; g.R = R; g.S = S;
    g.Ho = (Hi + 2 * pad - R) / stride + 1;
    g.Wo = (Wi + 2 * pad - S) / stride + 1;
    if (g.Ho < 1 || g.Wo < 1) return PHNET_ERR_ARG;
    g.stride = stride; g.pad = pad; g.in_dil = 1;
    return launch_conv<false>(x, w, bias, nullptr, y, (float*)workspace, ws_bytes, g, relu, (hipStream_t)stream);
}

static long conv_stats_blocks(long M, int Co, int K, bool has_ws, size_t ws_bytes)
{
    const ConvPlan t = plan_conv(M, Co, K, has_ws, ws_bytes);
    return t.splits > 1 ? ceil_div64(M * Co / 4, 256) : t.tiles / ceil_div64(Co, t.bn) * (t.bm / 32);
}

PHNET_API uint64_t phnet_conv2d_stats_blocks(int64_t M, int32_t Co, int32_t K, uint64_t ws_bytes)
{
    if (M < 1 || Co < 4 || K < 1) return 0;
    return (uint64_t)conv_stats_blocks((long)M, Co, K, ws_bytes > 0, (size_t)ws_bytes);
}

PHNET_API int phnet_conv2d_fwd_fused(const float* x, const float* w, const float* bias, const float* addend, float* y, float* stats,
                                     int32_t N, int32_t Hi, int32_t Wi, int32_t Ci, int32_t Co, int32_t R, int32_t S,
                                     int32_t stride, int32_t pad, int32_t relu,
                                     void* workspace, uint64_t ws_bytes, void* stream)
{
    if (N < 0 || Hi < 1 || Wi < 1 || Ci < 4 || Co < 4 || (Ci & 3) || (Co & 3) || R < 1 || S < 1 || stride < 1 || pad < 0)
        return PHNET_ERR_ARG;
    if (stats && (bias || addend || relu || (Co & (Co - 1)) || Co > 1024)) return PHNET_ERR_ARG;
    if (N == 0) return PHNET_OK;
    if (!x || !w || !y) return PHNET_ERR_ARG;
    ConvShape g{};
    g.N = N; g.Hi = Hi; g.Wi = Wi; g.Ci = Ci; g.Co = Co; g.R = R; g.S = S;
    g.Ho = (Hi + 2 * pad - R) / stride + 1;
    g.Wo = (Wi + 2 * pad - S) / stride + 1;
    if (g.Ho < 1 || g.Wo < 1) return PHNET_ERR_ARG;
    g.stride = stride; g.pad = pad; g.in_dil = 1;
    return launch_conv<false>(x, w, bias, addend, y, (float*)workspace, ws_bytes, g, relu, (hipStream_t)stream, stats);
}

PHNET_API int phnet_conv2d_dgrad(const float* dy, const float* w, const float* addend, float* dx,
                                 int32_t N, int32_t Hi, int32_t Wi, int32_t Ci, int32_t Co, int32_t R, int32_t S,
                                 int32_t stride, int32_t pad, void* workspace, uint64_t ws_bytes, void* stream)
{
    if (N < 0 || Hi < 1 || Wi < 1 || Ci < 4 || Co < 4 || (Ci & 3) || (Co & 3) || R < 1 || S < 1 || stride < 1 || pad < 0)
        return PHNET_ERR_ARG;
    if (stride > 2) return PHNET_ERR_ARG;
    if (N == 0) return PHNET_OK;
    if (!dy || !w || !dx) return PHNET_ERR_ARG;
    ConvShape g{};
    g.N = N;
    g.Hi = (Hi + 2 * pad - R) / stride + 1;
    g.Wi = (Wi + 2 * pad - S) / stride + 1;
    g.Ci = Co;
    g.Ho = Hi; g.Wo = Wi; g.Co = Ci;
    g.R = R; g.S = S;
    g.stride = 1; g.pad = R - 1 - pad; g.in_dil = stride;
    if (R != S && (S - 1 - pad) != g.pad) return PHNET_ERR_ARG;
    if (g.pad < 0) return PHNET_ERR_ARG;
    return launch_conv<true>(dy, w, nullptr, addend, dx, (float*)workspace, ws_bytes, g, 0, (hipStream_t)stream);
}

static long wgrad_splits(long P, long Co, long NC, int* bm_out)
{
    const int bm = (Co >= 128 && (Co < 256 || P > 8192) && g_wgrad_bm128) ? 128 : 64;
    const long tiles = ceil_div64(Co, bm) * ceil_div64(NC, 64);
    const long target = tiles >= 64 ? max((long)g_wgrad_target, (long)1250) : (long)g_wgrad_target;
    long splits = max((long)1, min((long)256, target / max((long)1, tiles)));
    splits = max((long)1, min(splits, P / 64));
    if (P <= 1024 && tiles >= 32) splits = 1;
    if (bm_out) *bm_out = bm;
    return splits;
}

static bool wgrad3_applies(long P, int Hi, int Wi, int Ci, int Co, int R, int S, int stride, int pad)
{
    return g_wgrad3 && g_mma_mode == 3 && R == 3 && S == 3 && stride == 1 && pad == 1 && (Ci & 63) == 0 && (Co & 63) == 0 &&
           Wi >= BK && P >= 64 && P * (long)max(Ci, Co) * 4 < 0x7fffffffL;
}
static long wgrad3_splits(long P, long Co, long Ci)
{
    const long tiles = (Co / 64) * (Ci / 64) * 3;
    return max((long)1, min(min((long)256, P / 64), (g_wgrad3_target + tiles / 2) / tiles));
}

PHNET_API uint64_t phnet_conv2d_wgrad_workspace(int32_t N, int32_t Hi, int32_t Wi, int32_t Ci, int32_t Co,
                                                int32_t R, int32_t S, int32_t stride, int32_t pad)
{
    const long Ho = (Hi + 2 * pad - R) / stride + 1, Wo = (Wi + 2 * pad - S) / stride + 1;
    const long P = (long)N * Ho * Wo, NC = (long)R * S * Ci;
    long splits = wgrad_splits(P, Co, NC, nullptr);
    if (R == 3 && S == 3 && stride == 1 && pad == 1 && (Ci & 63) == 0 && (Co & 63) == 0)
        splits = max(splits, min(min((long)256, max((long)1, P / 64)), (long)(1024 / ((Co / 64) * (Ci / 64) * 3) + 1)));
    return (uint64_t)(splits * (Co * NC + Co) * sizeof(float));
}

PHNET_API int phnet_conv2d_wgrad(const float* dy, const float* x, float* dw, float* dbias,
                                 int32_t N, int32_t Hi, int32_t Wi, int32_t Ci, int32_t Co, int32_t R, int32_t S,
                                 int32_t stride, int32_t pad, int32_t accumulate,
                                 void* workspace, uint64_t ws_bytes, void* stream)
{
    if (N < 0 || Hi < 1 || Wi < 1 || Ci < 4 || Co < 4 || (Ci & 3) || (Co & 3) || R < 1 || S < 1 || stride < 1 || pad < 0)
        return PHNET_ERR_ARG;
    if (!dy || !x || !dw) return PHNET_ERR_ARG;
    WgradShape g{};
    g.N = N; g.Hi = Hi; g.Wi = Wi; g.Ci = Ci; g.Co = Co; g.R = R; g.S = S; g.stride = stride; g.pad = pad;
    g.Ho = (Hi + 2 * pad - R) / stride + 1;
    g.Wo = (Wi + 2 * pad - S) / stride + 1;
    const long P = (long)N * g.Ho * g.Wo, NC = (long)R * S * Ci;
    hipStream_t st = (hipStream_t)stream;
    if (R == 1 && S == 1 && stride == 1 && pad == 0 && P <= SMALLP_MAX && g_wgrad_smallp &&
        ceil_div64(Co, 64) * ceil_div64(Ci, 64) < g_smallp_max_tiles) {
        const int P16 = ((int)P + 15) & ~15;
        const size_t lds = (size_t)P16 * (64 + 4) * 2 * sizeof(float);
        static bool attr = false;
        if (!attr) {
            const int cap = (int)((size_t)SMALLP_MAX * 68 * 2 * sizeof(float));
            if (hipFuncSetAttribute((const void*)linear_wgrad_smallp_kernel<64, 64, 0>, hipFuncAttributeMaxDynamicSharedMemorySize, cap) != hipSuccess ||
                hipFuncSetAttribute((const void*)linear_wgrad_smallp_kernel<64, 64, 1>, hipFuncAttributeMaxDynamicSharedMemorySize, cap) != hipSuccess)
                return PHNET_ERR_LAUNCH;
            attr = true;
        }
        const long tiles = ceil_div64(Co, 64) * ceil_div64(Ci, 64);
        if (g_mma_mode == 1)
            hipLaunchKernelGGL((linear_wgrad_smallp_kernel<64, 64, 1>), dim3((unsigned)tiles), dim3(THREADS), lds, st, dy, x, dw, dbias,
                               (int)P, Co, Ci, dbias != nullptr, accumulate);
        else
        hipLaunchKernelGGL((linear_wgrad_smallp_kernel<64, 64, 0>), dim3((unsigned)tiles), dim3(THREADS), lds, st, dy, x, dw, dbias,
                           (int)P, Co, Ci, dbias != nullptr, accumulate);
        return phnet_launch_status();
    }
    if (wgrad3_applies(P, Hi, Wi, Ci, Co, R, S, stride, pad)) {
        long splits = wgrad3_splits(P, Co, Ci);
        const long row = (long)Co * NC + Co;
        while (splits > 1 && (!workspace || (uint64_t)(splits * row * sizeof(float)) > ws_bytes)) --splits;
        const bool pc = g_wgrad3s && !dbias && (long)Hi * Wi >= phnet_wgrad3s_kstep();
        const int bkw = pc ? phnet_wgrad3s_kstep() : g_wgrad3_bkw == 16 ? 16 : 32;
        const long psteps = ceil_div64(P, bkw);
        g.splits = (int)splits;
        g.pix_per_split = (int)(ceil_div64(psteps, splits) * bkw);
        float* out = splits > 1 ? (float*)workspace : dw;
        if (pc) {
            Wgrad3sShape s{N, Hi, Wi, Ci, Co, g.splits, g.pix_per_split};
            const int rc = phnet_wgrad3s_launch(dy, x, out, s, accumulate, st);
            if (rc != PHNET_OK) return rc;
            if (splits > 1) {
                const long nw = (long)Co * NC, nb = Co;
                hipLaunchKernelGGL(wgrad_reduce_kernel, dim3((unsigned)ceil_div64((nw + nb) >> 2, 64)), dim3(256), 0, st,
                                   (const float*)workspace, dw, (float*)nullptr, nw, nb, (int)splits, accumulate);
            }
            return phnet_launch_status();
        }
        dim3 grid((unsigned)((Co / 64) * (Ci / 64) * 3), 1, (unsigned)splits);
        static bool attr = false;
        if (!attr) {
            if (hipFuncSetAttribute((const void*)conv_wgrad3x3_kernel<4, 16>, hipFuncAttributeMaxDynamicSharedMemorySize, Wgrad3Lds<16>::BYTES) != hipSuccess ||
                hipFuncSetAttribute((const void*)conv_wgrad3x3_kernel<4, 32>, hipFuncAttributeMaxDynamicSharedMemorySize, Wgrad3Lds<32>::BYTES) != hipSuccess)
                return PHNET_ERR_LAUNCH;
            attr = true;
        }
        if (bkw == 16)
            hipLaunchKernelGGL((conv_wgrad3x3_kernel<4, 16>), grid, dim3(W3_THREADS), Wgrad3Lds<16>::BYTES, st, dy, x, out, dbias, g, dbias != nullptr, accumulate);
        else
            hipLaunchKernelGGL((conv_wgrad3x3_kernel<4, 32>), grid, dim3(W3_THREADS), Wgrad3Lds<32>::BYTES, st, dy, x, out, dbias, g, dbias != nullptr, accumulate);
        if (splits > 1) {
            const long nw = (long)Co * NC, nb = Co;
            hipLaunchKernelGGL(wgrad_reduce_kernel, dim3((unsigned)ceil_div64((nw + nb) >> 2, 64)), dim3(256), 0, st,
                               (const float*)workspace, dw, dbias, nw, nb, (int)splits, accumulate);
        }
        return phnet_launch_status();
    }
    if (g_wgrad1s && g_mma_mode == 3 && R == 1 && S == 1 && stride == 1 && pad == 0 && (Co & 127) == 0 && (Ci & 127) == 0 && P >= 256 &&
        (long)(Co / 128) * (Ci / 128) >= 64 && P * (long)max(Ci, Co) * 4 < 0x7fffffffL) {
        const long tiles1 = (long)(Co / 128) * (Ci / 128);
        long splits1 = max((long)1, min((long)(P / 128), (long)256 / tiles1));
        const long row = (long)Co * NC + Co;
        while (splits1 > 1 && (!workspace || (uint64_t)(splits1 * row * sizeof(float)) > ws_bytes)) --splits1;
        const int ks = phnet_wgrad1s_kstep();
        Wgrad1sShape s1{(int)P, Ci, Co, (int)splits1, (int)(ceil_div64(ceil_div64(P, ks), splits1) * ks)};
        const int rc = phnet_wgrad1s_launch(dy, x, splits1 > 1 ? (float*)workspace : dw, dbias, s1, accumulate, st);
        if (rc != PHNET_OK) return rc;
        if (splits1 > 1) {
            const long nw = (long)Co * NC, nb = Co;
            hipLaunchKernelGGL(wgrad_reduce_kernel, dim3((unsigned)ceil_div64((nw + nb) >> 2, 64)), dim3(256), 0, st,
                               (const float*)workspace, dw, dbias, nw, nb, (int)splits1, accumulate);
        }
        return phnet_launch_status();
    }
    int bm = 64;
    const int bn = 64;
    long splits = wgrad_splits(P, Co, NC, &bm);
    const long tiles = ceil_div64(Co, bm) * ceil_div64(NC, bn);
    const long row = (long)Co * NC + Co;
    while (splits > 1 && (!workspace || (uint64_t)(splits * row * sizeof(float)) > ws_bytes)) --splits;
    const int bkw = (g_mma_mode == 3 && g_wgrad_bkw == 32) ? 32 : BK;
    const long psteps = ceil_div64(max(P, (long)1), bkw);
    g.splits = (int)splits;
    g.pix_per_split = (int)(ceil_div64(psteps, splits) * bkw);
    float* out = splits > 1 ? (float*)workspace : dw;
    dim3 grid((unsigned)tiles, 1, (unsigned)splits);
    const int want_bias = dbias != nullptr;
    if (g_mma_mode == 3 && bkw == 32 && bm == 128)
        hipLaunchKernelGGL((conv_wgrad_kernel<128, 64, 3, 32, 2, true>), grid, dim3(THREADS), 0, st, dy, x, out, dbias, g, want_bias, accumulate);
    else if (g_mma_mode == 3 && bkw == 32)
        hipLaunchKernelGGL((conv_wgrad_kernel<64, 64, 3, 32, 2, true>), grid, dim3(THREADS), 0, st, dy, x, out, dbias, g, want_bias, accumulate);
    else if (g_mma_mode == 3 && bm == 128)
        hipLaunchKernelGGL((conv_wgrad_kernel<128, 64, 3, 16, 4, true>), grid, dim3(THREADS), 0, st, dy, x, out, dbias, g, want_bias, accumulate);
    else if (g_mma_mode == 3)
        hipLaunchKernelGGL((conv_wgrad_kernel<64, 64, 3, 16, 4, true>), grid, dim3(THREADS), 0, st, dy, x, out, dbias, g, want_bias, accumulate);
    else if (bm == 128 && g_mma_mode == 2)
        hipLaunchKernelGGL((conv_wgrad_kernel<128, 64, 2>), grid, dim3(THREADS), 0, st, dy, x, out, dbias, g, want_bias, accumulate);
    else if (g_mma_mode == 2)
        hipLaunchKernelGGL((conv_wgrad_kernel<64, 64, 2>), grid, dim3(THREADS), 0, st, dy, x, out, dbias, g, want_bias, accumulate);
    else if (bm == 128 && g_mma_mode == 1)
        hipLaunchKernelGGL((conv_wgrad_kernel<128, 64, 1>), grid, dim3(THREADS), 0, st, dy, x, out, dbias, g, want_bias, accumulate);
    else if (g_mma_mode == 1)
        hipLaunchKernelGGL((conv_wgrad_kernel<64, 64, 1>), grid, dim3(THREADS), 0, st, dy, x, out, dbias, g, want_bias, accumulate);
    else if (bm == 128) hipLaunchKernelGGL((conv_wgrad_kernel<128, 64>), grid, dim3(THREADS), 0, st, dy, x, out, dbias, g, want_bias, accumulate);
    else hipLaunchKernelGGL((conv_wgrad_kernel<64, 64>), grid, dim3(THREADS), 0, st, dy, x, out, dbias, g, want_bias, accumulate);
    if (splits > 1) {
        const long nw = (long)Co * NC, nb = Co;
        hipLaunchKernelGGL(wgrad_reduce_kernel, dim3((unsigned)ceil_div64((nw + nb) >> 2, 64)), dim3(256), 0, st,
                           (const float*)workspace, dw, dbias, nw, nb, (int)splits, accumulate);
    }
    return phnet_launch_status();
}

PHNET_API int phnet_nchw3_to_nhwc4(const float* x, float* y, int32_t N, int32_t H, int32_t W, void* stream)
{
    if (N < 0 || H < 1 || W < 1) return PHNET_ERR_ARG;
    if (N == 0) return PHNET_OK;
    if (!x || !y) return PHNET_ERR_ARG;
    const long total = (long)N * H * W;
    hipLaunchKernelGGL(nchw3_to_nhwc4_kernel, dim3((unsigned)ceil_div64(total, 256)), dim3(256), 0, (hipStream_t)stream,
                       x, y, N, H * W);
    return phnet_launch_status();
}

PHNET_API int phnet_pad_channels(const float* src, float* dst, int64_t rows, int32_t cs, int32_t cd, void* stream)
{
    if (rows < 0 || cs < 1 || cd < 1) return PHNET_ERR_ARG;
    if (rows == 0) return PHNET_OK;
    if (!src || !dst) return PHNET_ERR_ARG;
    hipLaunchKernelGGL(pad_channels_kernel, dim3((unsigned)ceil_div64(rows * cd, 256)), dim3(256), 0, (hipStream_t)stream,
                       src, dst, (long)rows, cs, cd);
    return phnet_launch_status();
}

static bool linear_bwd_fusable(long M, long K, long N)
{
    if (!g_wgrad_smallp || M < 1 || M > SMALLP_MAX || (K & 3) || (N & 3) || K < 4 || N < 4) return false;
    const long wt = ceil_div64(N, 64) * ceil_div64(K, 64), dt = ceil_div64(M, 64) * ceil_div64(K, 64);
    return wt < g_smallp_max_tiles && N <= 640 && dt <= 256;
}

PHNET_API int phnet_linear_bwd_fusable(int64_t M, int64_t K, int64_t N) { return linear_bwd_fusable(M, K, N) ? 1 : 0; }

PHNET_API int phnet_linear_bwd(const float* dy, const float* x, const float* w, const float* relu_y, float* dx, float* dw,
                               float* dbias, int32_t M, int32_t K, int32_t N, int32_t accumulate, void* stream)
{
    if (!linear_bwd_fusable(M, K, N) || !dy || !x || !w || !dx || !dw) return PHNET_ERR_ARG;
    ConvShape g{};
    g.N = M; g.Hi = 1; g.Wi = 1; g.Ci = N;
    g.Ho = 1; g.Wo = 1; g.Co = K;
    g.R = 1; g.S = 1; g.stride = 1; g.pad = 0; g.in_dil = 1;
    g.splits = 1;
    g.k_per_split = (int)(ceil_div64(N, 64) * 64);
    const unsigned dt = (unsigned)(ceil_div64(M, 64) * ceil_div64(K, 64)), wt = (unsigned)(ceil_div64(N, 64) * ceil_div64(K, 64));
    const int P16 = (M + 15) & ~15;
    const size_t lds_dgrad = 2 * (size_t)(KContigTile<64, 64>::FLOATS + KStridedTile<64, 64>::FLOATS) * sizeof(float);
    const size_t lds_wgrad = (size_t)P16 * 68 * 2 * sizeof(float);
    const size_t lds = lds_dgrad > lds_wgrad ? lds_dgrad : lds_wgrad;
    static bool attr = false;
    if (!attr) {
        const int cap = (int)((size_t)SMALLP_MAX * 68 * 2 * sizeof(float));
        const void* fns[8] = {(const void*)linear_bwd_fused_kernel<true, true, 0>, (const void*)linear_bwd_fused_kernel<true, false, 0>,
                              (const void*)linear_bwd_fused_kernel<false, true, 0>, (const void*)linear_bwd_fused_kernel<false, false, 0>,
                              (const void*)linear_bwd_fused_kernel<true, true, 1>, (const void*)linear_bwd_fused_kernel<true, false, 1>,
                              (const void*)linear_bwd_fused_kernel<false, true, 1>, (const void*)linear_bwd_fused_kernel<false, false, 1>};
        for (const void* f : fns)
            if (hipFuncSetAttribute(f, hipFuncAttributeMaxDynamicSharedMemorySize, cap) != hipSuccess) return PHNET_ERR_LAUNCH;
        attr = true;
    }
    hipStream_t st = (hipStream_t)stream;
    const bool uni = N % 64 == 0 && g_uniform_tap;
#define PHNET_LAUNCH_BWD_(U_, A_, MMA_)                                                                                 \
    hipLaunchKernelGGL((linear_bwd_fused_kernel<U_, A_, MMA_>), dim3(dt + wt), dim3(THREADS), lds, st, dy, w, x, relu_y, dx, \
                       dw, dbias, g, dt, (int)M, (int)N, (int)K, dbias != nullptr, accumulate)
#define PHNET_LAUNCH_BWD(U_, A_)                                                                                        \
    do {                                                                                                                \
        if (g_mma_mode == 1) PHNET_LAUNCH_BWD_(U_, A_, 1);                                                              \
        else PHNET_LAUNCH_BWD_(U_, A_, 0);                                                                              \
    } while (0)
    if (uni && relu_y) PHNET_LAUNCH_BWD(true, true);
    else if (uni) PHNET_LAUNCH_BWD(true, false);
    else if (relu_y) PHNET_LAUNCH_BWD(false, true);
    else PHNET_LAUNCH_BWD(false, false);
#undef PHNET_LAUNCH_BWD
#undef PHNET_LAUNCH_BWD_
    return phnet_launch_status();
}
```

phnet_amd/csrc/conv3p.hip:

```cpp
#include "igemm.h"

using namespace igemm;

namespace {

struct P3Shape {
    int N, H, W;
    int Ca, Nn;
    int splits, units_per_split;
};

constexpr int P3_BM = 128, P3_ROWS = P3_BM + 2, P3_THREADS = 256;
constexpr int P3_APITCH = 48;
constexpr int P3_ZROW = P3_ROWS;
constexpr int P3_APLANE = (P3_ROWS + 1) * P3_APITCH, P3_AIMG = 3 * P3_APLANE;
constexpr int P3_PFB = 3;
constexpr size_t P3_LDS = 2 * P3_AIMG + 3 * 512;

struct P3PackJob { const float* w; unsigned char* dst; int Co, Ci, dgrad, pad_; long first; };

__device__ __forceinline__ void conv3p_pack_item(const float* __restrict__ w, unsigned char* __restrict__ packed, int Co, int Ci,
                                                 int dgrad, long i)
{
    const int Ca = dgrad ? Co : Ci, Nn = dgrad ? Ci : Co;
    const int CC = Ca >> 4, NF = Nn >> 5;
    const int lane = (int)(i & 63);
    const long qj = i >> 6;
    const int j = (int)(qj % NF);
    const int q = (int)(qj / NF);
    const int dx = q % 3, cc = (q / 3) % CC, dy = q / (3 * CC);
    const int r = lane & 31, h = lane >> 5;
    const int n = 32 * j + r, k0 = cc * 16 + 8 * h;
    float v[8];
#pragma unroll
    for (int e = 0; e < 8; ++e) {
        v[e] = !dgrad ? w[(((long)n * 3 + dy) * 3 + dx) * Ci + k0 + e]
                      : w[(((long)(k0 + e) * 3 + (2 - dy)) * 3 + (2 - dx)) * Ci + n];
    }
    unsigned hi[4], mid[4], lo[4];
#pragma unroll
    for (int e = 0; e < 4; ++e) split3_pair(v[2 * e], v[2 * e + 1], hi[e], mid[e], lo[e]);
    typedef unsigned u32x4 __attribute__((ext_vector_type(4)));
    unsigned char* dst = packed + ((qj * 3) * 64 + lane) * 16;
    *reinterpret_cast<u32x4*>(dst) = (u32x4){hi[0], hi[1], hi[2], hi[3]};
    *reinterpret_cast<u32x4*>(dst + 1024) = (u32x4){mid[0], mid[1], mid[2], mid[3]};
    *reinterpret_cast<u32x4*>(dst + 2048) = (u32x4){lo[0], lo[1], lo[2], lo[3]};
}

__global__ __launch_bounds__(256) void conv3p_pack_kernel(const float* __restrict__ w, unsigned char* __restrict__ packed,
                                                          int Co, int Ci, int dgrad)
{
    const int Ca = dgrad ? Co : Ci, Nn = dgrad ? Ci : Co;
    const long total = (long)9 * (Ca >> 4) * (Nn >> 5) * 64;
    const long i = (long)blockIdx.x * blockDim.x + threadIdx.x;
    if (i < total) conv3p_pack_item(w, packed, Co, Ci, dgrad, i);
}

__global__ __launch_bounds__(256) void conv3p_pack_jobs_kernel(const P3PackJob* __restrict__ jobs, int njobs, long total)
{
    const long i = (long)blockIdx.x * blockDim.x + threadIdx.x;
    if (i >= total) return;
    int lo = 0, hi = njobs - 1;
    while (lo < hi) {
        const int mid = (lo + hi + 1) >> 1;
        if (jobs[mid].first <= i) lo = mid; else hi = mid - 1;
    }
    const P3PackJob jb = jobs[lo];
    conv3p_pack_item(jb.w, jb.dst, jb.Co, jb.Ci, jb.dgrad, i - jb.first);
}

template <int FN>
__global__ __launch_bounds__(P3_THREADS, FN == 1 ? 3 : 2) void conv3p_kernel(
    const float* __restrict__ X, const unsigned char* __restrict__ Bp, const float* __restrict__ bias,
    const float* __restrict__ addend, float* __restrict__ out, P3Shape g, int relu, float* __restrict__ stats)
{
    extern __shared__ __attribute__((aligned(16))) float lds[];
    unsigned char* A3 = reinterpret_cast<unsigned char*>(lds);
    unsigned char* dump = A3 + 2 * P3_AIMG;

    const int W = g.W, H = g.H, Ca = g.Ca;
    const int M = g.N * H * W;
    const int CC = Ca >> 4, NF = g.Nn >> 5;
    constexpr int BN = 64 * FN;
    const int tiles_n = g.Nn / BN;
    const unsigned tile = xcd_remap(blockIdx.x, gridDim.x);
    const int m0 = (int)(tile / tiles_n) * P3_BM, n0 = (int)(tile % tiles_n) * BN;
    const int u_begin = blockIdx.z * g.units_per_split, u_end = min(3 * CC, u_begin + g.units_per_split);
    const int tid = threadIdx.x, lane = tid & 63, wave = tid >> 6;
    const int wm = (wave >> 1) * 64, wn = (wave & 1) * 32 * FN;

    constexpr unsigned OOB = 0x80000000u;
    __amdgpu_buffer_rsrc_t x_rsrc = __builtin_amdgcn_make_buffer_rsrc((void*)X, 0, (int)min((long)M * Ca * 4, (long)0x7fffffff), 0x00020000);
    __amdgpu_buffer_rsrc_t b_rsrc = __builtin_amdgcn_make_buffer_rsrc((void*)Bp, 0, (int)min((long)9 * Ca * g.Nn * 6, (long)0x7fffffff), 0x00020000);

    int a_off[3], a_ok[3], a_lds[3];
#pragma unroll
    for (int i = 0; i < 3; ++i) {
        const int idx = tid + 256 * i, row = idx >> 2, chunk = idx & 3;
        const bool rowok = idx < 4 * P3_ROWS;
        const int t = m0 - 1 + row;
        const bool tok = rowok && (unsigned)t < (unsigned)M;
        const int tt = tok ? t : 0;
        const int y = (tt / W) % H;
        a_ok[i] = (tok && y >= 1 ? 1 : 0) | (tok ? 2 : 0) | (tok && y + 1 < H ? 4 : 0);
        a_off[i] = (t * Ca + chunk * 4) * 4;
        a_lds[i] = rowok ? row * P3_APITCH + chunk * 8 : -1;
    }
    const bool wave0 = __builtin_amdgcn_readfirstlane(wave) == 0;
    int la_dy = u_begin / CC, la_cc = u_begin - la_dy * CC, la_u = u_begin;
    auto load_a = [&](f32x4 (&reg)[3]) {
        const bool uok = la_u < u_end;
        const int s_a = ((la_dy - 1) * W * Ca + la_cc * 16) * 4;
#pragma unroll
        for (int i = 0; i < 2; ++i) {
            const bool ok = uok && ((a_ok[i] >> la_dy) & 1);
            reg[i] = __builtin_bit_cast(f32x4, __builtin_amdgcn_raw_buffer_load_b128(x_rsrc, ok ? a_off[i] + s_a : (int)OOB, 0, 0));
        }
        if (wave0) {
            const bool ok = uok && ((a_ok[2] >> la_dy) & 1);
            reg[2] = __builtin_bit_cast(f32x4, __builtin_amdgcn_raw_buffer_load_b128(x_rsrc, ok ? a_off[2] + s_a : (int)OOB, 0, 0));
        }
        ++la_u; ++la_cc;
        const int wrap = la_cc == CC;
        la_cc = wrap ? 0 : la_cc;
        la_dy += wrap;
    };
    auto store_a = [&](int aoff, const f32x4 (&reg)[3]) {
        store_split3<P3_APLANE>(A3 + aoff, a_lds[0], reg[0]);
        store_split3<P3_APLANE>(A3 + aoff, a_lds[1], reg[1]);
        if (wave0) {
            unsigned h0, m0_, l0, h1, m1, l1;
            split3_pair(reg[2].x, reg[2].y, h0, m0_, l0);
            split3_pair(reg[2].z, reg[2].w, h1, m1, l1);
            const bool has = a_lds[2] >= 0;
            unsigned char* q = has ? A3 + aoff + a_lds[2] : dump + lane * 8;
            const int ps = has ? P3_APLANE : 512;
            *reinterpret_cast<u32x2*>(q) = (u32x2){h0, h1};
            *reinterpret_cast<u32x2*>(q + ps) = (u32x2){m0_, m1};
            *reinterpret_cast<u32x2*>(q + 2 * ps) = (u32x2){l0, l1};
        }
    };
    const int jfrag = (n0 + wn) >> 5;
    const int b_lane = (jfrag * 3 * 64 + lane) * 16;
    const int b_step = NF * 3 * 64 * 16;
    int lb_q = u_begin * 3;
    const int q_end = u_end * 3;
    auto load_b = [&](Frag3 (&f)[FN]) {
        const bool ok = lb_q < q_end;
        const int off = b_lane + lb_q * b_step;
#pragma unroll
        for (int jn = 0; jn < FN; ++jn) {
            f[jn].hi = __builtin_bit_cast(bf16x8, __builtin_amdgcn_raw_buffer_load_b128(b_rsrc, ok ? off + jn * 3072 : (int)OOB, 0, 0));
            f[jn].mid = __builtin_bit_cast(bf16x8, __builtin_amdgcn_raw_buffer_load_b128(b_rsrc, ok ? off + jn * 3072 + 1024 : (int)OOB, 0, 0));
            f[jn].lo = __builtin_bit_cast(bf16x8, __builtin_amdgcn_raw_buffer_load_b128(b_rsrc, ok ? off + jn * 3072 + 2048 : (int)OOB, 0, 0));
        }
        ++lb_q;
    };

    const bool final_pass = g.splits == 1;
    f32x16 acc[2][FN];
    {
        const bool use_add = final_pass && addend != nullptr;
        __amdgpu_buffer_rsrc_t add_rsrc = __builtin_amdgcn_make_buffer_rsrc((void*)addend, 0, use_add ? (int)min((long)M * g.Nn * 4, (long)0x7fffffff) : 0, 0x00020000);
#pragma unroll
        for (int jn = 0; jn < FN; ++jn) {
            const int n = n0 + wn + 32 * jn + frag_col(lane);
            const float bv = (final_pass && bias) ? bias[n] : 0.f;
#pragma unroll
            for (int f = 0; f < 2; ++f)
#pragma unroll
                for (int e = 0; e < 16; ++e) {
                    const int m = m0 + wm + 32 * f + frag_row(lane, e);
                    const int off = (use_add && m < M) ? (m * g.Nn + n) * 4 : (int)OOB;
                    acc[f][jn][e] = bv + __builtin_bit_cast(float, __builtin_amdgcn_raw_buffer_load_b32(add_rsrc, off, 0, 0));
                }
        }
    }
    int a_rel[2][3];
#pragma unroll
    for (int f = 0; f < 2; ++f) {
        const int rr = wm + 32 * f + (lane & 31);
        const int pr = m0 + rr;
        const int px = (pr < M ? pr : 0) % W;
        const int hb = (lane >> 5) * 16;
        a_rel[f][0] = (px == 0 ? P3_ZROW : rr) * P3_APITCH + hb;
        a_rel[f][1] = (rr + 1) * P3_APITCH + hb;
        a_rel[f][2] = (px == W - 1 ? P3_ZROW : rr + 2) * P3_APITCH + hb;
    }
    for (int i = tid; i < 2 * 3 * (P3_APITCH / 4); i += P3_THREADS) {
        const int img = i / (3 * (P3_APITCH / 4)), rem = i % (3 * (P3_APITCH / 4)), pl = rem / (P3_APITCH / 4), w4 = rem % (P3_APITCH / 4);
        *reinterpret_cast<unsigned*>(A3 + img * P3_AIMG + pl * P3_APLANE + P3_ZROW * P3_APITCH + w4 * 4) = 0u;
    }

    if (u_begin < u_end) {
        f32x4 a_reg[3];
        Frag3 bq[P3_PFB][FN];
        load_a(a_reg);
#pragma unroll
        for (int d = 0; d < P3_PFB; ++d) load_b(bq[d]);
        store_a(0, a_reg);
        load_a(a_reg);
        __syncthreads();
        int aoff = 0;
        auto step = [&](auto DX) {
            constexpr int dxi = decltype(DX)::value;
            Frag3 a[2];
#pragma unroll
            for (int f = 0; f < 2; ++f) {
                const unsigned char* p = A3 + aoff + a_rel[f][dxi];
                a[f].hi = *reinterpret_cast<const bf16x8*>(p);
                a[f].mid = *reinterpret_cast<const bf16x8*>(p + P3_APLANE);
                a[f].lo = *reinterpret_cast<const bf16x8*>(p + 2 * P3_APLANE);
            }
            mma3_step<2, FN>(a, bq[dxi], acc);
            load_b(bq[dxi]);
        };
        for (int u = u_begin; u < u_end; ++u) {
            step(std::integral_constant<int, 0>{});
            __builtin_amdgcn_sched_barrier(0);
            step(std::integral_constant<int, 1>{});
            __builtin_amdgcn_sched_barrier(0);
            store_a(aoff ^ P3_AIMG, a_reg);
            load_a(a_reg);
            step(std::integral_constant<int, 2>{});
            __syncthreads();
            aoff ^= P3_AIMG;
        }
    }

    if (stats != nullptr && final_pass) {
#pragma unroll
        for (int jn = 0; jn < FN; ++jn) {
            const int n = n0 + wn + 32 * jn + frag_col(lane);
            float sm = 0.f, sq = 0.f;
#pragma unroll
            for (int f = 0; f < 2; ++f)
#pragma unroll
                for (int e = 0; e < 16; ++e) { const float v = acc[f][jn][e]; sm += v; sq += v * v; }
            sm += __shfl_xor(sm, 32, 64);
            sq += __shfl_xor(sq, 32, 64);
            if (lane < 32) {
                float* p = stats + (size_t)((m0 + wm) >> 6) * 2 * g.Nn;
                p[n] = sm;
                p[g.Nn + n] = sq;
            }
        }
    }
    float* dst = out + (size_t)blockIdx.z * M * g.Nn;
#pragma unroll
    for (int jn = 0; jn < FN; ++jn) {
        const int n = n0 + wn + 32 * jn + frag_col(lane);
#pragma unroll
        for (int f = 0; f < 2; ++f)
#pragma unroll
            for (int e = 0; e < 16; ++e) {
                const int m = m0 + wm + 32 * f + frag_row(lane, e);
                if (m < M) dst[(size_t)m * g.Nn + n] = (final_pass && relu) ? fmaxf(acc[f][jn][e], 0.f) : acc[f][jn][e];
            }
    }
}

constexpr int P3_RCH = 4;

__device__ __forceinline__ f32x4 conv3p_reduce_one(const float* __restrict__ part, float* __restrict__ out, const float* __restrict__ bias,
                                                   const float* __restrict__ addend, long i, long total4, int ncols, int splits, int relu)
{
    const f32x4* p = reinterpret_cast<const f32x4*>(part) + i;
    f32x4 v[8];
#pragma unroll
    for (int z = 0; z < 8; ++z) v[z] = p[(long)min(z, splits - 1) * total4];
    f32x4 s = v[0];
#pragma unroll
    for (int z = 1; z < 8; ++z)
        if (z < splits) s += v[z];
    for (int z = 8; z < splits; ++z) s += p[(long)z * total4];
    if (bias) s += *reinterpret_cast<const f32x4*>(bias + (int)((i * 4) % ncols));
    if (addend) s += reinterpret_cast<const f32x4*>(addend)[i];
    if (relu) { s.x = fmaxf(s.x, 0.f); s.y = fmaxf(s.y, 0.f); s.z = fmaxf(s.z, 0.f); s.w = fmaxf(s.w, 0.f); }
    reinterpret_cast<f32x4*>(out)[i] = s;
    return s;
}

__global__ __launch_bounds__(256) void conv3p_reduce_kernel(const float* __restrict__ part, float* __restrict__ out,
                                                            const float* __restrict__ bias, const float* __restrict__ addend,
                                                            long total4, int ncols, int splits, int relu, float* __restrict__ stats)
{
    __shared__ f32x4 red_s[2][256];
    if (stats == nullptr) {
        const long i = (long)blockIdx.x * 256 + threadIdx.x;
        if (i < total4) conv3p_reduce_one(part, out, bias, addend, i, total4, ncols, splits, relu);
        return;
    }
    f32x4 a{0.f, 0.f, 0.f, 0.f}, b{0.f, 0.f, 0.f, 0.f};
#pragma unroll
    for (int c = 0; c < P3_RCH; ++c) {
        const long i = ((long)blockIdx.x * P3_RCH + c) * 256 + threadIdx.x;
        if (i < total4) {
            const f32x4 s = conv3p_reduce_one(part, out, bias, addend, i, total4, ncols, splits, relu);
            a += s; b += s * s;
        }
    }
    red_s[0][threadIdx.x] = a;
    red_s[1][threadIdx.x] = b;
    __syncthreads();
    const int c4 = ncols >> 2;
    if ((int)threadIdx.x < c4) {
        f32x4 sa = red_s[0][threadIdx.x], sb = red_s[1][threadIdx.x];
        for (int r = c4; r < 256; r += c4) { sa += red_s[0][r + threadIdx.x]; sb += red_s[1][r + threadIdx.x]; }
        float* q = stats + (size_t)blockIdx.x * 2 * ncols + threadIdx.x * 4;
        *reinterpret_cast<f32x4*>(q) = sa;
        *reinterpret_cast<f32x4*>(q + ncols) = sb;
    }
}

inline long cdiv(long a, long b) { return (a + b - 1) / b; }

int g_p3_target = 512;
int g_p3_wide = 1;

struct P3Plan { long tiles; int fn, splits, units_per_split; };

P3Plan p3_plan(long M, int Ca, int Nn, size_t ws_bytes)
{
    P3Plan p;
    p.fn = (g_p3_wide && Nn % 128 == 0 && M >= 16384) ? 2 : 1;
    p.tiles = cdiv(M, P3_BM) * (Nn / (64 * p.fn));
    const int units = 3 * (Ca / 16);
    int splits = 1;
    if (ws_bytes > 0 && p.tiles * 2 <= g_p3_target) {
        splits = (int)min((long)8, (long)g_p3_target / p.tiles);
        while (splits > 1 && units / splits < 4) --splits;
        while (splits > 1 && (size_t)splits * M * Nn * sizeof(float) > ws_bytes) --splits;
    }
    p.units_per_split = (units + splits - 1) / splits;
    p.splits = (units + p.units_per_split - 1) / p.units_per_split;
    return p;
}

bool p3_applies(long M, int Ca, int Nn)
{
    return M >= 1 && Ca >= 16 && (Ca % 16) == 0 && Nn >= 64 && (Nn % 64) == 0 &&
           M * (long)Ca * 4 < 0x7fffffffL && (long)9 * Ca * Nn * 6 < 0x7fffffffL && M * (long)Nn * 4 < 0x7fffffffL * 4;
}

}

PHNET_API int phnet_conv3p_applies(int64_t M, int32_t Ca, int32_t Nn) { return p3_applies((long)M, Ca, Nn) ? 1 : 0; }

PHNET_API uint64_t phnet_conv3p_packed_bytes(int32_t Co, int32_t Ci) { return (uint64_t)9 * Co * Ci * 6; }

PHNET_API int phnet_conv3p_pack(const float* w, void* packed, int32_t Co, int32_t Ci, int32_t dgrad, void* stream)
{
    if (!w || !packed || Co < 16 || Ci < 16) return PHNET_ERR_ARG;
    const int Ca = dgrad ? Co : Ci, Nn = dgrad ? Ci : Co;
    if ((Ca % 16) || (Nn % 32)) return PHNET_ERR_ARG;
    const long total = (long)9 * (Ca / 16) * (Nn / 32) * 64;
    hipLaunchKernelGGL(conv3p_pack_kernel, dim3((unsigned)cdiv(total, 256)), dim3(256), 0, (hipStream_t)stream,
                       w, (unsigned char*)packed, Co, Ci, dgrad);
    return phnet_launch_status();
}

PHNET_API int phnet_conv3p_pack_jobs(const void* jobs, int32_t njobs, int64_t total, void* stream)
{
    if (!jobs || njobs < 1 || total < 1) return PHNET_ERR_ARG;
    hipLaunchKernelGGL(conv3p_pack_jobs_kernel, dim3((unsigned)cdiv((long)total, 256)), dim3(256), 0, (hipStream_t)stream,
                       (const P3PackJob*)jobs, njobs, (long)total);
    return phnet_launch_status();
}

PHNET_API uint64_t phnet_conv3p_stats_blocks(int64_t M, int32_t Ca, int32_t Nn, uint64_t ws_bytes)
{
    if (!p3_applies((long)M, Ca, Nn)) return 0;
    const P3Plan p = p3_plan((long)M, Ca, Nn, (size_t)ws_bytes);
    return (uint64_t)(p.splits > 1 ? cdiv((long)M * Nn / 4, 256 * P3_RCH) : cdiv((long)M, P3_BM) * (P3_BM / 64));
}

PHNET_API int phnet_conv3p_splits(int64_t M, int32_t Ca, int32_t Nn, uint64_t ws_bytes)
{
    if (!p3_applies((long)M, Ca, Nn)) return 0;
    return p3_plan((long)M, Ca, Nn, (size_t)ws_bytes).splits;
}

PHNET_API int phnet_conv3p_tune(int32_t target_workgroups)
{
    if (target_workgroups == -1 || target_workgroups == -2) { g_p3_wide = target_workgroups == -2; return PHNET_OK; }
    if (target_workgroups < 1) return PHNET_ERR_ARG;
    g_p3_target = target_workgroups;
    return PHNET_OK;
}

PHNET_API int phnet_conv3p_fwd(const float* x, const void* packed, const float* bias, const float* addend, float* y, float* stats,
                               int32_t N, int32_t H, int32_t W, int32_t Ca, int32_t Nn, int32_t relu,
                               void* workspace, uint64_t ws_bytes, void* stream)
{
    if (N < 0 || H < 1 || W < 2 || Ca < 16 || Nn < 64) return PHNET_ERR_ARG;
    if (N == 0) return PHNET_OK;
    const long M = (long)N * H * W;
    if (!x || !packed || !y || !p3_applies(M, Ca, Nn)) return PHNET_ERR_ARG;
    if (stats && (bias || addend || relu || (Nn & (Nn - 1)) || Nn > 1024)) return PHNET_ERR_ARG;
    const P3Plan p = p3_plan(M, Ca, Nn, workspace ? (size_t)ws_bytes : 0);
    P3Shape g{N, H, W, Ca, Nn, p.splits, p.units_per_split};
    float* dst = p.splits > 1 ? (float*)workspace : y;
    hipStream_t st = (hipStream_t)stream;
    if (p.fn == 2)
        hipLaunchKernelGGL(conv3p_kernel<2>, dim3((unsigned)p.tiles, 1, (unsigned)p.splits), dim3(P3_THREADS), P3_LDS, st,
                           x, (const unsigned char*)packed, bias, addend, dst, g, relu, p.splits > 1 ? (float*)nullptr : stats);
    else
        hipLaunchKernelGGL(conv3p_kernel<1>, dim3((unsigned)p.tiles, 1, (unsigned)p.splits), dim3(P3_THREADS), P3_LDS, st,
                           x, (const unsigned char*)packed, bias, addend, dst, g, relu, p.splits > 1 ? (float*)nullptr : stats);
    if (p.splits > 1) {
        const long total4 = M * Nn / 4;
        hipLaunchKernelGGL(conv3p_reduce_kernel, dim3((unsigned)cdiv(total4, stats ? 256 * P3_RCH : 256)), dim3(256), 0, st,
                           (const float*)workspace, y, bias, addend, total4, Nn, p.splits, relu, stats);
    }
    return phnet_launch_status();
}
```

phnet_amd/hip_ops.py:

```python
import os
"""Tensor-level wrappers over the C-ABI (include/phnet_hip.h): shape checks, output allocation, stream plumbing.

PyTorch is used here only for device memory and the current HIP stream.  No op in this file has a
fallback: a non-CUDA tensor or a missing library raises.
"""
from typing import Optional, Tuple

import torch

from ._lib import check, lib

_WS = {}

TIMER = None


_MMA_MODE = 3


_TAPS3 = True


def _gemm_symbol(m, co, k, ws_bytes, dgrad, ci_a, in_dil=1, taps3=False):
    import ctypes
    bm, bn, sp, kt = ctypes.c_int32(), ctypes.c_int32(), ctypes.c_int32(), ctypes.c_int32()
    check(lib().phnet_conv2d_plan(m, co, k, ws_bytes, ctypes.byref(bm), ctypes.byref(bn), ctypes.byref(sp), ctypes.byref(kt)),
          "phnet_conv2d_plan")
    uni = bm.value == 64 and bn.value == 64 and ci_a % kt.value == 0
    pf = 4 if _MMA_MODE == 3 else 1
    buf = uni and _MMA_MODE == 3 and in_dil == 1
    if taps3 and buf and kt.value == 16 and _TAPS3:
        return f"conv3x3s1_kernel<{'true' if dgrad else 'false'}>", sp.value
    return (f"conv_igemm_kernel<{bm.value}, {bn.value}, {'true' if dgrad else 'false'}, {kt.value}, {'true' if uni else 'false'}, "
            f"{_MMA_MODE}, {pf}, {'true' if buf else 'false'}>", sp.value)


def _timed_launch(sym_fn, flops, launch, shape=None, nbytes=None):
    if TIMER is None:
        return launch()
    sym, splits = sym_fn()
    e0, e1 = torch.cuda.Event(enable_timing=True), torch.cuda.Event(enable_timing=True)
    e0.record()
    out = launch()
    e1.record()
    TIMER.append((sym, splits, flops, e0, e1, launch, shape, nbytes))
    return out


def _stream() -> int:
    return torch.cuda.current_stream().cuda_stream


def _ptr(t: Optional[torch.Tensor]) -> Optional[int]:
    return None if t is None else t.data_ptr()


def _req(t: torch.Tensor, dtype=torch.float32, name="tensor"):
    if not t.is_cuda:
        raise RuntimeError(f"{name} must be a CUDA(HIP) tensor; phnet_amd has no CPU path")
    if t.dtype != dtype:
        raise RuntimeError(f"{name} must be {dtype}, got {t.dtype}")
    if not t.is_contiguous():
        raise RuntimeError(f"{name} must be contiguous")
    return t


_WS_RETIRED = []


def workspace(nbytes: int, device, slot: int = 0) -> torch.Tensor:
    key = (torch.device(device).index, slot)
    cur = _WS.get(key)
    if cur is None or cur.numel() < nbytes:
        if cur is not None:
            _WS_RETIRED.append(cur)
        cur = torch.empty(max(int(nbytes), 1 << 20), dtype=torch.uint8, device=device)
        _WS[key] = cur
    return cur


def lane_nms(rows: torch.Tensor, scores: torch.Tensor, thresh: float, top_k: int,
             counts: Optional[torch.Tensor] = None) -> Tuple[torch.Tensor, torch.Tensor, torch.Tensor]:
    _req(rows, name="rows"); _req(scores, name="scores")
    batched = rows.dim() == 3
    f = rows.shape[0] if batched else 1
    k, prop = rows.shape[-2], rows.shape[-1]
    if scores.numel() != f * k:
        raise RuntimeError("scores must have one entry per row")
    if counts is not None:
        _req(counts, torch.int32, "counts")
    keep = torch.empty((f, k), dtype=torch.int64, device=rows.device)
    parent = torch.empty((f, k), dtype=torch.int64, device=rows.device)
    num = torch.empty((f,), dtype=torch.int64, device=rows.device)
    check(lib().phnet_lane_nms(_ptr(rows), _ptr(scores), _ptr(counts), f, k, prop - 5, float(thresh), int(top_k),
                               _ptr(keep), _ptr(num), _ptr(parent), _stream()), "phnet_lane_nms")
    if batched:
        return keep, num, parent
    return keep[0], num[0], parent[0]


def roi_pool_fwd(fmap: torch.Tensor, xs: torch.Tensor, ys: torch.Tensor, with_cp: bool = False):
    _req(fmap, name="fmap"); _req(xs, name="xs"); _req(ys, name="ys")
    b, h, w, c = fmap.shape
    _, n, p = xs.shape
    out = torch.empty((b, n, p, c), dtype=torch.float32, device=fmap.device)
    out_cp = torch.empty((b, n, c, p), dtype=torch.float32, device=fmap.device) if with_cp else None
    check(lib().phnet_roi_pool_fwd(_ptr(fmap), _ptr(xs), _ptr(ys), _ptr(out), _ptr(out_cp), b, n, p, h, w, c, _stream()),
          "phnet_roi_pool_fwd")
    return (out, out_cp) if with_cp else out


def roi_pool_bwd(dout, fmap, xs, ys, dmap: Optional[torch.Tensor], need_dxs: bool):
    _req(dout, name="dout")
    b, h, w, c = fmap.shape
    _, n, p = xs.shape
    dxs = torch.empty_like(xs) if need_dxs else None
    check(lib().phnet_roi_pool_bwd(_ptr(dout), _ptr(fmap), _ptr(xs), _ptr(ys), _ptr(dmap), _ptr(dxs),
                                   b, n, p, h, w, c, _stream()), "phnet_roi_pool_bwd")
    return dxs


def conv_out_hw(hi, wi, r, s, stride, pad):
    return (hi + 2 * pad - r) // stride + 1, (wi + 2 * pad - s) // stride + 1


def conv2d_fwd(x, w, bias, stride: int, pad: int, relu: bool = False, out: Optional[torch.Tensor] = None,
               addend: Optional[torch.Tensor] = None, stats: bool = False):
    _req(x, name="x"); _req(w, name="w")
    n, hi, wi, ci = x.shape
    co, r, s, ci2 = w.shape
    assert ci == ci2, (x.shape, w.shape)
    ho, wo = conv_out_hw(hi, wi, r, s, stride, pad)
    if out is None:
        out = torch.empty((n, ho, wo, co), dtype=torch.float32, device=x.device)
    need = 8 * n * ho * wo * co * 4 if n * ho * wo * co < (1 << 23) else 0
    ws = workspace(need, x.device) if need else None
    m, k = n * ho * wo, r * s * ci
    if addend is not None or stats:
        part, nblk = None, 0
        if stats:
            nblk = int(lib().phnet_conv2d_stats_blocks(m, co, k, need))
            part = workspace(nblk * 2 * co * 4, x.device, 1)
        if addend is not None:
            _req(addend, name="addend")
            assert addend.shape == out.shape
        _timed_launch(lambda: _gemm_symbol(m, co, k, need, False, ci, taps3=(r == 3 and s == 3 and stride == 1 and pad == 1)), 2.0 * m * co * k,
                      lambda: check(lib().phnet_conv2d_fwd_fused(_ptr(x), _ptr(w), _ptr(bias), _ptr(addend), _ptr(out), _ptr(part), n, hi, wi,
                                                                 ci, co, r, s, stride, pad, int(relu), _ptr(ws), need, _stream()),
                                    "phnet_conv2d_fwd_fused"), shape=("fwd", m, co, k, r), nbytes=4.0 * (n * hi * wi * ci + m * co + co * k))
        return (out, (part, nblk)) if stats else out
    _timed_launch(lambda: _gemm_symbol(m, co, k, need, False, ci, taps3=(r == 3 and s == 3 and stride == 1 and pad == 1)), 2.0 * m * co * k,
                  lambda: check(lib().phnet_conv2d_fwd(_ptr(x), _ptr(w), _ptr(bias), _ptr(out), n, hi, wi, ci, co, r, s, stride,
                                                       pad, int(relu), _ptr(ws), need, _stream()), "phnet_conv2d_fwd"),
                  shape=("fwd", m, co, k, r), nbytes=4.0 * (n * hi * wi * ci + m * co + co * k))
    return out


def conv3p_applies(m: int, ca: int, nn: int) -> bool:
    return bool(lib().phnet_conv3p_applies(int(m), int(ca), int(nn)))


def conv3p_pack(w: torch.Tensor, dgrad: bool, out: Optional[torch.Tensor] = None) -> torch.Tensor:
    _req(w, name="w")
    co, r, s_, ci = w.shape
    assert r == 3 and s_ == 3, w.shape
    nbytes = int(lib().phnet_conv3p_packed_bytes(co, ci))
    if out is None:
        out = torch.empty(nbytes, dtype=torch.uint8, device=w.device)
    assert out.numel() >= nbytes and out.is_contiguous()
    check(lib().phnet_conv3p_pack(_ptr(w), _ptr(out), co, ci, int(dgrad), _stream()), "phnet_conv3p_pack")
    return out


class Conv3pPackPlan:

    def __init__(self, weights, with_dgrad: bool = True):
        dev = weights[0].device
        self.ptrs = tuple(int(w.data_ptr()) for w in weights)
        sizes = [int(lib().phnet_conv3p_packed_bytes(w.shape[0], w.shape[3])) for w in weights]
        kinds = (False, True) if with_dgrad else (False,)
        self.buf = torch.empty(sum(sizes) * len(kinds), dtype=torch.uint8, device=dev)
        self.images, rows, off, first = [], [], 0, 0
        for w, nbytes in zip(weights, sizes):
            _req(w, name="w")
            co, _, _, ci = w.shape
            per = {}
            for dg in kinds:
                ca, nn = (co, ci) if dg else (ci, co)
                assert ca % 16 == 0 and nn % 32 == 0, w.shape
                img = self.buf[off:off + nbytes]
                rows.append([int(w.data_ptr()), int(img.data_ptr()), co | (ci << 32), int(dg), first])
                first += 9 * (ca // 16) * (nn // 32) * 64
                off += nbytes
                per[dg] = img
            self.images.append(per)
        self.total = first
        self.jobs = torch.tensor(rows, dtype=torch.int64).to(dev)

    def matches(self, weights) -> bool:
        return self.ptrs == tuple(int(w.data_ptr()) for w in weights)

    def refresh(self):
        check(lib().phnet_conv3p_pack_jobs(_ptr(self.jobs), self.jobs.shape[0], self.total, _stream()), "phnet_conv3p_pack_jobs")


def conv3p(x: torch.Tensor, packed: torch.Tensor, nn: int, dgrad: bool = False, bias=None, addend=None, relu: bool = False,
           stats: bool = False):
    _req(x, name="x")
    n, h, w_, ca = x.shape
    out = torch.empty((n, h, w_, nn), dtype=torch.float32, device=x.device)
    m = n * h * w_
    need = 8 * m * nn * 4 if m * nn < (1 << 23) else 0
    ws = workspace(need, x.device) if need else None
    part, nblk = None, 0
    if stats:
        nblk = int(lib().phnet_conv3p_stats_blocks(m, ca, nn, need))
        part = workspace(nblk * 2 * nn * 4, x.device, 1)
    if addend is not None:
        _req(addend, name="addend")
        assert addend.shape == out.shape
    _timed_launch(lambda: (f"conv3p_kernel<{2 if (nn % 128 == 0 and m >= 16384) else 1}>", int(lib().phnet_conv3p_splits(m, ca, nn, need))),
                  2.0 * m * nn * 9 * ca,
                  lambda: check(lib().phnet_conv3p_fwd(_ptr(x), _ptr(packed), _ptr(bias), _ptr(addend), _ptr(out), _ptr(part), n, h, w_, ca, nn,
                                                       int(relu), _ptr(ws), need, _stream()), "phnet_conv3p_fwd"),
                  shape=("dgrad" if dgrad else "fwd", m, nn, 9 * ca, 3),
                  nbytes=4.0 * m * (ca + nn) + 6.0 * 9 * ca * nn + (4.0 * m * nn if addend is not None else 0.0))
    return (out, (part, nblk)) if stats else out


def conv2d_dgrad(dy, w, in_hw: Tuple[int, int], stride: int, pad: int, addend: Optional[torch.Tensor] = None):
    _req(dy, name="dy"); _req(w, name="w")
    n = dy.shape[0]
    co, r, s, ci = w.shape
    hi, wi = in_hw
    dx = torch.empty((n, hi, wi, ci), dtype=torch.float32, device=dy.device)
    need = 8 * n * hi * wi * ci * 4 if n * hi * wi * ci < (1 << 23) else 0
    ws = workspace(need, dy.device) if need else None
    m, k = n * hi * wi, r * s * co
    _timed_launch(lambda: _gemm_symbol(m, ci, k, need, True, co, stride, taps3=(r == 3 and s == 3 and stride == 1 and pad == 1)), 2.0 * dy.shape[0] * dy.shape[1] * dy.shape[2] * co * r * s * ci,
                  lambda: check(lib().phnet_conv2d_dgrad(_ptr(dy), _ptr(w), _ptr(addend), _ptr(dx), n, hi, wi, ci, co, r, s, stride,
                                                         pad, _ptr(ws), need, _stream()), "phnet_conv2d_dgrad"),
                  shape=("dgrad", m, ci, k, r), nbytes=4.0 * (dy.numel() + m * ci + co * r * s * ci))
    return dx


CONV3P = os.environ.get("PHNET_CONV3P", "1") != "0"
_WGRAD3 = True
_WGRAD3S = True
_WGRAD1S = True


def conv2d_wgrad(dy, x, w_shape, stride: int, pad: int, dw: Optional[torch.Tensor] = None, accumulate: bool = False,
                 dbias: Optional[torch.Tensor] = None):
    _req(dy, name="dy"); _req(x, name="x")
    n, hi, wi, ci = x.shape
    co, r, s, _ = w_shape
    if dw is None:
        dw = torch.empty((co, r, s, ci), dtype=torch.float32, device=x.device)
        assert not accumulate
    need = lib().phnet_conv2d_wgrad_workspace(n, hi, wi, ci, co, r, s, stride, pad)
    ws = workspace(need, x.device) if need else None
    ho, wo = conv_out_hw(hi, wi, r, s, stride, pad)
    smallp = (r == 1 and s == 1 and stride == 1 and pad == 0 and n * ho * wo <= 256 and
              ((co + 63) // 64) * ((ci + 63) // 64) < 400)
    taps3 = (_MMA_MODE == 3 and r == 3 and s == 3 and stride == 1 and pad == 1 and ci % 64 == 0 and co % 64 == 0 and wi >= 16 and
             n * ho * wo >= 64 and _WGRAD3)
    _timed_launch(lambda: (f"linear_wgrad_smallp_kernel<64, 64, {1 if _MMA_MODE == 1 else 0}>" if smallp
                           else "wgrad1s_kernel" if (_WGRAD1S and _MMA_MODE == 3 and r == 1 and s == 1 and stride == 1 and pad == 0 and co % 128 == 0
                                                     and ci % 128 == 0 and n * ho * wo >= 256 and (co // 128) * (ci // 128) >= 64)
                           else "wgrad3s_kernel<2>" if taps3 and dbias is None and _WGRAD3S
                           else "conv_wgrad3x3_kernel<4, 16>" if taps3
                           else f"conv_wgrad_kernel<{128 if (co >= 128 and (co < 256 or n * ho * wo > 8192)) else 64}, 64, {_MMA_MODE}, 16, {4 if _MMA_MODE == 3 else 1}, {'true' if _MMA_MODE == 3 else 'false'}>", 0),
                  2.0 * n * ho * wo * co * r * s * ci,
                  lambda: check(lib().phnet_conv2d_wgrad(_ptr(dy), _ptr(x), _ptr(dw), _ptr(dbias), n, hi, wi, ci, co, r, s, stride,
                                                         pad, int(accumulate), _ptr(ws), need, _stream()), "phnet_conv2d_wgrad"),
                  shape=("wgrad", co, r * s * ci, n * ho * wo, r), nbytes=4.0 * (dy.numel() + x.numel() + co * r * s * ci))
    return dw


def linear_fwd(x2d, w, bias, relu: bool = False):
    m, k = x2d.shape
    return conv2d_fwd(x2d.view(m, 1, 1, k), w.view(w.shape[0], 1, 1, k), bias, 1, 0, relu).view(m, w.shape[0])


def linear_dgrad(dy2d, w):
    m, n = dy2d.shape
    k = w.shape[1]
    return conv2d_dgrad(dy2d.view(m, 1, 1, n), w.view(n, 1, 1, k), (1, 1), 1, 0).view(m, k)


def linear_wgrad(dy2d, x2d, dw: Optional[torch.Tensor] = None, accumulate: bool = False, dbias: Optional[torch.Tensor] = None):
    m, n = dy2d.shape
    k = x2d.shape[1]
    out = conv2d_wgrad(dy2d.view(m, 1, 1, n), x2d.view(m, 1, 1, k), (n, 1, 1, k), 1, 0,
                       None if dw is None else dw.view(n, 1, 1, k), accumulate, dbias)
    return out.view(n, k)


def linear_bwd_fusable(m: int, k: int, n: int) -> bool:
    return bool(lib().phnet_linear_bwd_fusable(m, k, n))


def linear_bwd(dy2d, x2d, w, dw: torch.Tensor, dbias: Optional[torch.Tensor], accumulate: bool, relu_y: Optional[torch.Tensor] = None):
    _req(dy2d, name="dy"); _req(x2d, name="x"); _req(w, name="w"); _req(dw, name="dw")
    m, n = dy2d.shape
    k = x2d.shape[1]
    dx = torch.empty((m, k), dtype=torch.float32, device=dy2d.device)
    sym = f"linear_bwd_fused_kernel<{'true' if n % 64 == 0 else 'false'}, {'true' if relu_y is not None else 'false'}, {1 if _MMA_MODE == 1 else 0}>"
    _timed_launch(lambda: (sym, 0), 4.0 * m * n * k,
                  lambda: check(lib().phnet_linear_bwd(_ptr(dy2d), _ptr(x2d), _ptr(w), _ptr(relu_y), _ptr(dx), _ptr(dw), _ptr(dbias), m, k, n,
                                                       int(accumulate), _stream()), "phnet_linear_bwd"), shape=("linbwd", m, n, k, 1))
    return dx


def nchw3_to_nhwc4(x):
    _req(x, name="frames")
    n, c, h, w = x.shape
    assert c == 3
    y = torch.empty((n, h, w, 4), dtype=torch.float32, device=x.device)
    check(lib().phnet_nchw3_to_nhwc4(_ptr(x), _ptr(y), n, h, w, _stream()), "phnet_nchw3_to_nhwc4")
    return y


def pad_channels(src2d, cd: int):
    _req(src2d, name="src")
    rows, cs = src2d.shape
    dst = torch.empty((rows, cd), dtype=torch.float32, device=src2d.device)
    check(lib().phnet_pad_channels(_ptr(src2d), _ptr(dst), rows, cs, cd, _stream()), "phnet_pad_channels")
    return dst


def _partials(m, c, device, slot=1):
    nfloats = lib().phnet_channel_partials_size(m, c)
    return workspace(nfloats * 4, device, slot)


def bn_fwd(x, gamma, beta, running_mean, running_var, training: bool, eps: float, momentum: float,
           residual=None, relu: bool = True, partials=None):
    _req(x, name="x")
    c = x.shape[-1]
    m = x.numel() // c
    dev = x.device
    scale = torch.empty(c, dtype=torch.float32, device=dev)
    shift = torch.empty(c, dtype=torch.float32, device=dev)
    sm = torch.empty(c, dtype=torch.float32, device=dev) if training else None
    si = torch.empty(c, dtype=torch.float32, device=dev) if training else None
    if training and partials is not None:
        check(lib().phnet_bn_finalize_partials(_ptr(partials[0]), int(partials[1]), m, c, eps, momentum, _ptr(gamma), _ptr(beta),
                                               _ptr(running_mean), _ptr(running_var), _ptr(sm), _ptr(si), _ptr(scale), _ptr(shift),
                                               _stream()), "phnet_bn_finalize_partials")
    else:
        part = _partials(m, c, dev) if training else None
        check(lib().phnet_bn_fwd_stats(_ptr(x), m, c, eps, momentum, _ptr(gamma), _ptr(beta), _ptr(running_mean),
                                       _ptr(running_var), _ptr(sm), _ptr(si), _ptr(scale), _ptr(shift), _ptr(part),
                                       int(training), _stream()), "phnet_bn_fwd_stats")
    y = torch.empty_like(x)
    check(lib().phnet_bn_apply(_ptr(x), _ptr(scale), _ptr(shift), _ptr(residual), _ptr(y), m, c, int(relu), _stream()),
          "phnet_bn_apply")
    return y, sm, si


def bn_bwd(dy, x, y, save_mean, save_invstd, gamma, relu: bool, dres: Optional[torch.Tensor] = None,
           dres_accumulate: bool = False, dgamma: Optional[torch.Tensor] = None, dbeta: Optional[torch.Tensor] = None,
           param_accumulate: bool = False):
    _req(dy, name="dy")
    c = x.shape[-1]
    m = x.numel() // c
    dev = x.device
    dx = torch.empty_like(x)
    dgamma = torch.empty(c, dtype=torch.float32, device=dev) if dgamma is None else dgamma
    dbeta = torch.empty(c, dtype=torch.float32, device=dev) if dbeta is None else dbeta
    c12 = torch.empty(2, c, dtype=torch.float32, device=dev)
    part = _partials(m, c, dev)
    check(lib().phnet_bn_bwd(_ptr(dy), _ptr(x), _ptr(y), _ptr(save_mean), _ptr(save_invstd), _ptr(gamma), _ptr(dx),
                             _ptr(dres), _ptr(dgamma), _ptr(dbeta), _ptr(part), _ptr(c12[0]), _ptr(c12[1]),
                             m, c, int(relu), int(dres_accumulate), int(param_accumulate), _stream()), "phnet_bn_bwd")
    return dx, dgamma, dbeta


def bn_fwd_sync(x, gamma, beta, running_mean, running_var, eps: float, momentum: float, residual=None, relu: bool = True,
                group=None, partials=None):
    from . import parallel
    _req(x, name="x")
    c = x.shape[-1]
    m = x.numel() // c
    dev = x.device
    stats = torch.empty(4, c, dtype=torch.float32, device=dev)
    sums = torch.empty(2 * c + 1, dtype=torch.float64, device=dev)
    if partials is not None and partials[0] is not None:
        check(lib().phnet_bn_partials_to_sums(_ptr(partials[0]), int(partials[1]), m, c, _ptr(sums), _stream()), "phnet_bn_partials_to_sums")
    else:
        part = _partials(m, c, dev)
        check(lib().phnet_bn_local_sums(_ptr(x), m, c, _ptr(part), _ptr(sums), _stream()), "phnet_bn_local_sums")
    parallel.allreduce_sum_(sums, group)
    check(lib().phnet_bn_finalize_sums(_ptr(sums), c, eps, momentum, _ptr(gamma), _ptr(beta), _ptr(running_mean), _ptr(running_var),
                                       _ptr(stats[0]), _ptr(stats[1]), _ptr(stats[2]), _ptr(stats[3]), _stream()), "phnet_bn_finalize_sums")
    y = torch.empty_like(x)
    check(lib().phnet_bn_apply(_ptr(x), _ptr(stats[2]), _ptr(stats[3]), _ptr(residual), _ptr(y), m, c, int(relu), _stream()),
          "phnet_bn_apply")
    return y, stats[0], stats[1], sums[2 * c:]


def bn_bwd_sync(dy, x, y, mean, invstd, gamma, relu: bool, count, dres: Optional[torch.Tensor] = None, group=None,
                dres_accumulate: bool = False, dgamma: Optional[torch.Tensor] = None, dbeta: Optional[torch.Tensor] = None,
                param_accumulate: bool = False):
    from . import parallel
    _req(dy, name="dy")
    c = x.shape[-1]
    m = x.numel() // c
    dev = x.device
    sums = torch.empty(2, c, dtype=torch.float32, device=dev)
    scratch = torch.empty(2, c, dtype=torch.float32, device=dev)
    part = _partials(m, c, dev)
    check(lib().phnet_bn_bwd_reduce(_ptr(dy), _ptr(x), _ptr(y), _ptr(mean), _ptr(invstd), _ptr(sums), _ptr(part),
                                    _ptr(scratch[0]), _ptr(scratch[1]), m, c, int(relu), _stream()), "phnet_bn_bwd_reduce")
    if dgamma is None:
        dgamma, dbeta = sums[0].clone(), sums[1].clone()
    elif param_accumulate:
        dgamma.add_(sums[0]); dbeta.add_(sums[1])
    else:
        dgamma.copy_(sums[0]); dbeta.copy_(sums[1])
    parallel.allreduce_sum_(sums, group)
    dx = torch.empty_like(x)
    check(lib().phnet_bn_bwd_apply_sums(_ptr(dy), _ptr(x), _ptr(y), _ptr(mean), _ptr(invstd), _ptr(gamma), _ptr(sums), _ptr(count),
                                        _ptr(scratch[0]), _ptr(scratch[1]), _ptr(dx), _ptr(dres), m, c, int(relu),
                                        int(dres_accumulate), _stream()), "phnet_bn_bwd_apply_sums")
    return dx, dgamma, dbeta


def maxpool_fwd(x):
    _req(x, name="x")
    n, hi, wi, c = x.shape
    ho, wo = (hi - 1) // 2 + 1, (wi - 1) // 2 + 1
    y = torch.empty((n, ho, wo, c), dtype=torch.float32, device=x.device)
    arg = torch.empty((n, ho, wo, c), dtype=torch.uint8, device=x.device)
    check(lib().phnet_maxpool3x3s2_fwd(_ptr(x), _ptr(y), _ptr(arg), n, hi, wi, c, _stream()), "phnet_maxpool3x3s2_fwd")
    return y, arg


def maxpool_bwd(dy, arg, in_shape):
    n, hi, wi, c = in_shape
    dx = torch.empty(in_shape, dtype=torch.float32, device=dy.device)
    check(lib().phnet_maxpool3x3s2_bwd(_ptr(_req(dy)), _ptr(arg), _ptr(dx), n, hi, wi, c, _stream()), "phnet_maxpool3x3s2_bwd")
    return dx


def upsample_add_(fine, coarse):
    n, H, W, c = fine.shape
    _, h, w, _ = coarse.shape
    check(lib().phnet_upsample_add(_ptr(_req(fine)), _ptr(_req(coarse)), n, H, W, h, w, c, _stream()), "phnet_upsample_add")
    return fine


def upsample_add_bwd_(dfine, dcoarse):
    n, H, W, c = dfine.shape
    _, h, w, _ = dcoarse.shape
    check(lib().phnet_upsample_add_bwd(_ptr(_req(dfine)), _ptr(_req(dcoarse)), n, H, W, h, w, c, _stream()),
          "phnet_upsample_add_bwd")
    return dcoarse


def colsum(a2d, out: Optional[torch.Tensor] = None, accumulate: bool = False):
    _req(a2d, name="a")
    m, c = a2d.shape
    if out is None:
        out = torch.empty(c, dtype=torch.float32, device=a2d.device)
        accumulate = False
    ws = workspace(lib().phnet_colsum_workspace(m, c), a2d.device, 2)
    check(lib().phnet_colsum(_ptr(a2d), _ptr(out), m, c, int(accumulate), _ptr(ws), ws.numel(), _stream()), "phnet_colsum")
    return out


def layernorm_fwd(x, w, b, eps: float = 1e-5, res=None, relu: bool = False, save_stats: bool = True):
    _req(x, name="x")
    L = w.numel()
    rows = x.numel() // L
    y = torch.empty_like(x)
    mean = torch.empty(rows, dtype=torch.float32, device=x.device) if save_stats else None
    rstd = torch.empty(rows, dtype=torch.float32, device=x.device) if save_stats else None
    check(lib().phnet_layernorm_fwd(_ptr(x), _ptr(w), _ptr(b), _ptr(res), _ptr(y), _ptr(mean), _ptr(rstd), rows, L, eps,
                                    int(relu), _stream()), "phnet_layernorm_fwd")
    return y, mean, rstd


def layernorm_bwd(dy, x, y, w, mean, rstd, relu: bool, need_dres: bool = False,
                  dw: Optional[torch.Tensor] = None, db: Optional[torch.Tensor] = None, accumulate: bool = False):
    _req(dy, name="dy")
    L = w.numel()
    rows = x.numel() // L
    dx = torch.empty_like(x)
    dres = torch.empty_like(x) if need_dres else None
    if dw is None:
        dw, db, accumulate = torch.empty_like(w), torch.empty_like(w), False
    ws = workspace(lib().phnet_layernorm_bwd_workspace(rows, L), x.device, 2)
    check(lib().phnet_layernorm_bwd(_ptr(dy), _ptr(x), _ptr(y), _ptr(w), _ptr(mean), _ptr(rstd), _ptr(dx), _ptr(dres),
                                    _ptr(dw), _ptr(db), rows, L, int(relu), int(accumulate), _ptr(ws), ws.numel(), _stream()),
          "phnet_layernorm_bwd")
    return dx, dres, dw, db


def dyn_bmm_ln_relu_fwd(x, w, gamma, beta, eps: float, save_stats: bool = True):
    _req(x, name="x"); _req(w, name="w")
    n, p, k = x.shape
    j = w.shape[2]
    if w.shape[0] != n or w.shape[1] != k or gamma.numel() != j:
        raise ValueError(f"dyn_bmm_ln_relu: x {tuple(x.shape)} / w {tuple(w.shape)} / gamma {tuple(gamma.shape)} mismatch")
    y = torch.empty((n, p, j), dtype=torch.float32, device=x.device)
    stats = torch.empty((n, p, 2), dtype=torch.float32, device=x.device) if save_stats else None
    check(lib().phnet_dyn_bmm_ln_relu_fwd(_ptr(x), _ptr(w), _ptr(gamma), _ptr(beta), _ptr(y), _ptr(stats), n, p, k, j, eps, _stream()),
          "phnet_dyn_bmm_ln_relu_fwd")
    return y, stats


def dyn_bmm_ln_relu_bwd(dy, x, w, y, stats, gamma, eps: float, need_dx: bool = True,
                        dgamma: Optional[torch.Tensor] = None, dbeta: Optional[torch.Tensor] = None, accumulate: bool = False):
    _req(dy, name="dy")
    n, p, k = x.shape
    j = w.shape[2]
    dx = torch.empty_like(x) if need_dx else None
    dw = torch.empty_like(w)
    if dgamma is None:
        dgamma, dbeta, accumulate = torch.empty_like(gamma), torch.empty_like(gamma), False
    ws = workspace(n * 2 * j * 4, x.device, 2)
    check(lib().phnet_dyn_bmm_ln_relu_bwd(_ptr(dy), _ptr(x), _ptr(w), _ptr(y), _ptr(stats), _ptr(gamma), _ptr(dx), _ptr(dw),
                                          _ptr(dgamma), _ptr(dbeta), n, p, k, j, eps, int(accumulate), _ptr(ws), ws.numel(), _stream()),
          "phnet_dyn_bmm_ln_relu_bwd")
    return dx, dw, dgamma, dbeta


def dwconv3x3(x, w, bias, flip: bool = False):
    _req(x, name="x"); _req(w, name="w")
    n, c, p = x.shape
    y = torch.empty_like(x)
    check(lib().phnet_dwconv3x3(_ptr(x), _ptr(w), _ptr(bias), _ptr(y), n, c, p, int(flip), _stream()), "phnet_dwconv3x3")
    return y


def dwconv3x3_wgrad(dy, x, dw: Optional[torch.Tensor] = None, db: Optional[torch.Tensor] = None, accumulate: bool = False):
    _req(dy, name="dy")
    n, c, p = x.shape
    if dw is None:
        dw = torch.empty((n, 1, 3, 3), dtype=torch.float32, device=x.device)
        db = torch.empty((n,), dtype=torch.float32, device=x.device)
        accumulate = False
# ... 479 lines not shown
```

Measured before the change: 64.61 clips/s.

## Fuse split-K reduction into conv kernels via last-arriver ticket combine

Result: no change. 64.56 clips/s (median of 2 runs) (-0.1%).

```diff
diff --git a/include/phnet_hip.h b/include/phnet_hip.h
--- a/include/phnet_hip.h
+++ b/include/phnet_hip.h
@@ -37,6 +37,19 @@
 int phnet_conv2d_dgrad(const float* dy, const float* w, const float* addend, float* dx,
                        int32_t N, int32_t Hi, int32_t Wi, int32_t Ci, int32_t Co, int32_t R, int32_t S,
                        int32_t stride, int32_t pad, void* workspace, uint64_t ws_bytes, void* stream);
+int phnet_conv2d_fwd_tk(const float* x, const float* w, const float* bias, float* y,
+                        int32_t N, int32_t Hi, int32_t Wi, int32_t Ci, int32_t Co, int32_t R, int32_t S,
+                        int32_t stride, int32_t pad, int32_t relu, void* workspace, uint64_t ws_bytes, void* stream,
+                        uint32_t* tickets, uint64_t tickets_cap);
+uint64_t phnet_conv2d_stats_blocks_tk(int64_t M, int32_t Co, int32_t K, uint64_t ws_bytes, uint64_t tickets_cap);
+int phnet_conv2d_fwd_fused_tk(const float* x, const float* w, const float* bias, const float* addend, float* y, float* stats,
+                              int32_t N, int32_t Hi, int32_t Wi, int32_t Ci, int32_t Co, int32_t R, int32_t S,
+                              int32_t stride, int32_t pad, int32_t relu, void* workspace, uint64_t ws_bytes, void* stream,
+                              uint32_t* tickets, uint64_t tickets_cap);
+int phnet_conv2d_dgrad_tk(const float* dy, const float* w, const float* addend, float* dx,
+                          int32_t N, int32_t Hi, int32_t Wi, int32_t Ci, int32_t Co, int32_t R, int32_t S,
+                          int32_t stride, int32_t pad, void* workspace, uint64_t ws_bytes, void* stream,
+                          uint32_t* tickets, uint64_t tickets_cap);
 int phnet_conv3p_applies(int64_t M, int32_t Ca, int32_t Nn);
 uint64_t phnet_conv3p_packed_bytes(int32_t Co, int32_t Ci);
 int phnet_conv3p_pack(const float* w, void* packed, int32_t Co, int32_t Ci, int32_t dgrad, void* stream);
@@ -46,6 +59,10 @@
 int phnet_conv3p_fwd(const float* x, const void* packed, const float* bias, const float* addend, float* y, float* stats,
                      int32_t N, int32_t H, int32_t W, int32_t Ca, int32_t Nn, int32_t relu,
                      void* workspace, uint64_t ws_bytes, void* stream);
+uint64_t phnet_conv3p_stats_blocks_tk(int64_t M, int32_t Ca, int32_t Nn, uint64_t ws_bytes, uint64_t tickets_cap);
+int phnet_conv3p_fwd_tk(const float* x, const void* packed, const float* bias, const float* addend, float* y, float* stats,
+                        int32_t N, int32_t H, int32_t W, int32_t Ca, int32_t Nn, int32_t relu,
+                        void* workspace, uint64_t ws_bytes, void* stream, uint32_t* tickets, uint64_t tickets_cap);
 int phnet_conv2d_plan(int64_t M, int32_t Co, int32_t K, uint64_t ws_bytes, int32_t* bm, int32_t* bn, int32_t* splits,
                       int32_t* k_tile);
 uint64_t phnet_conv2d_wgrad_workspace(int32_t N, int32_t Hi, int32_t Wi, int32_t Ci, int32_t Co,
diff --git a/phnet_amd/csrc/conv.hip b/phnet_amd/csrc/conv.hip
--- a/phnet_amd/csrc/conv.hip
+++ b/phnet_amd/csrc/conv.hip
@@ -1,5 +1,6 @@
 #include <type_traits>
 #include "igemm.h"
+#include "splitk.h"
 #include "wgrad3s.h"
 static constexpr bool g_interleave = true;
 
@@ -40,7 +41,7 @@
     const float* __restrict__ X, const float* __restrict__ W, const float* __restrict__ bias,
     const float* __restrict__ addend, float* __restrict__ out, const ConvShape& g, int relu,
     float* lds, unsigned block, unsigned nblocks, unsigned split, const float* __restrict__ amask = nullptr,
-    float* __restrict__ stats = nullptr)
+    float* __restrict__ stats = nullptr, float* y = nullptr, unsigned* __restrict__ tickets = nullptr)
 {
     constexpr int TM = BM / 2, TN = BN / 2, FM = TM / 32, FN = TN / 32;
     constexpr int A_PITCH = KContigTile<BM, BKT>::PITCH;
@@ -347,6 +348,7 @@
     }
 
     float* dst = out + (size_t)split * M * g.Co;
+    const bool publish = !final_pass && tickets != nullptr;
 #pragma unroll
     for (int j = 0; j < FN; ++j) {
         const int n = n0 + wn + j * 32 + frag_col(lane);
@@ -356,19 +358,23 @@
 #pragma unroll
             for (int e = 0; e < 16; ++e) {
                 const int m = m0 + wm + i * 32 + frag_row(lane, e);
-                if (m < M) dst[(size_t)m * g.Co + n] = (final_pass && relu) ? fmaxf(acc[i][j][e], 0.f) : acc[i][j][e];
-            }
-    }
+                if (m < M) splitk::store(dst + (size_t)m * g.Co + n, (final_pass && relu) ? fmaxf(acc[i][j][e], 0.f) : acc[i][j][e], publish);
+            }
+    }
+    if (!final_pass && tickets != nullptr && splitk::last_arriver(tickets, tile, g.splits, reinterpret_cast<unsigned char*>(lds)))
+        splitk::combine_tile<BM, BN, 32>(out, (size_t)M * g.Co, y, bias, addend, M, g.Co, m0, n0, g.splits, relu, stats,
+                                         reinterpret_cast<unsigned char*>(lds));
 }
 
 template <int BM, int BN, bool B_DGRAD, int BKT, bool UNI, int MMA = 0, int PF = 1, bool BUF = false>
 __global__ __launch_bounds__(THREADS) void conv_igemm_kernel(
     const float* __restrict__ X, const float* __restrict__ W, const float* __restrict__ bias,
-    const float* __restrict__ addend, float* __restrict__ out, ConvShape g, int relu, float* __restrict__ stats)
+    const float* __restrict__ addend, float* __restrict__ out, ConvShape g, int relu, float* __restrict__ stats,
+    float* y, unsigned* __restrict__ tickets)
 {
     extern __shared__ __attribute__((aligned(16))) float lds[];
     igemm_tile<BM, BN, B_DGRAD, BKT, UNI, false, MMA, PF, BUF>(X, W, bias, addend, out, g, relu, lds, blockIdx.x, gridDim.x, blockIdx.z,
-                                                               nullptr, stats);
+                                                               nullptr, stats, y, tickets);
 }
 
 constexpr int T3_AROWS = 66;
@@ -376,7 +382,8 @@
 template <bool DGRAD>
 __global__ __launch_bounds__(THREADS) void conv3x3s1_kernel(
     const float* __restrict__ X, const float* __restrict__ Wt, const float* __restrict__ bias,
-    const float* __restrict__ addend, float* __restrict__ out, ConvShape g, int relu, float* __restrict__ stats)
+    const float* __restrict__ addend, float* __restrict__ out, ConvShape g, int relu, float* __restrict__ stats,
+    float* y, unsigned* __restrict__ tickets)
 {
     constexpr int APITCH = KContigPlanes<64, 16>::PITCH;
     constexpr int APLANE = T3_AROWS * APITCH, AIMG = 3 * APLANE;
@@ -563,14 +570,18 @@
         }
     }
     float* dst = out + (size_t)blockIdx.z * M * g.Co;
+    const bool publish = !final_pass && tickets != nullptr;
     const int n = n0 + wn + frag_col(lane);
     if (n < g.Co) {
 #pragma unroll
         for (int e = 0; e < 16; ++e) {
             const int m = m0 + wm + frag_row(lane, e);
-            if (m < M) dst[(size_t)m * g.Co + n] = (final_pass && relu) ? fmaxf(acc[0][0][e], 0.f) : acc[0][0][e];
-        }
-    }
+            if (m < M) splitk::store(dst + (size_t)m * g.Co + n, (final_pass && relu) ? fmaxf(acc[0][0][e], 0.f) : acc[0][0][e], publish);
+        }
+    }
+    if (!final_pass && tickets != nullptr && splitk::last_arriver(tickets, tile, g.splits, reinterpret_cast<unsigned char*>(lds)))
+        splitk::combine_tile<64, 64, 32>(out, (size_t)M * g.Co, y, bias, addend, M, g.Co, m0, n0, g.splits, relu, stats,
+                                         reinterpret_cast<unsigned char*>(lds));
 }
 
 __global__ __launch_bounds__(256) void splitk_reduce_kernel(const float* __restrict__ part, float* __restrict__ out,
@@ -1286,7 +1297,8 @@
 
 template <bool DGRAD>
 int launch_conv(const float* X, const float* W, const float* bias, const float* addend, float* out, float* workspace,
-                size_t ws_bytes, ConvShape g, int relu, hipStream_t st, float* stats = nullptr)
+                size_t ws_bytes, ConvShape g, int relu, hipStream_t st, float* stats = nullptr, unsigned* tickets = nullptr,
+                uint64_t tickets_cap = 0)
 {
     const long M = (long)g.N * g.Ho * g.Wo;
     const int K = g.R * g.S * g.Ci;
@@ -1295,6 +1307,9 @@
     const int splits = t.splits;
     g.splits = splits;
     float* dst = splits > 1 ? workspace : out;
+    const bool inkernel = splits > 1 && tickets != nullptr && (uint64_t)tiles <= tickets_cap;
+    float* kstats = (splits == 1 || inkernel) ? stats : nullptr;
+    unsigned* tk = inkernel ? tickets : nullptr;
     dim3 grid((unsigned)tiles, 1, (unsigned)splits);
     const int bkt = g_force_kt ? g_force_kt : k_tile_for(M, K, g.Ci, t.bm, t.bn);
     const int ksteps = (K + bkt - 1) / bkt;
@@ -1318,7 +1333,7 @@
             attr_set_ = true;                                                                                           \
         }                                                                                                               \
         hipLaunchKernelGGL((conv_igemm_kernel<BM_, BN_, DGRAD, BKT_, UNI_, MMA_, PF_, BUF_>), grid, dim3(THREADS), lds_, st, \
-                           X, W, bias, addend, dst, g, relu, splits > 1 ? (float*)nullptr : stats);                     \
+                           X, W, bias, addend, dst, g, relu, kstats, out, tk);                                          \
     } while (0)
 #define PHNET_LAUNCH_CONV__(BM_, BN_, BKT_, UNI_, MMA_) PHNET_LAUNCH_CONV___(BM_, BN_, BKT_, UNI_, MMA_, 1)
 #define PHNET_LAUNCH_CONV_(BM_, BN_, BKT_, UNI_)                                                                        \
@@ -1346,7 +1361,7 @@
         constexpr size_t lds_ = 2 * 3 * T3_AROWS * KContigPlanes<64, 16>::PITCH +
                                 2 * (size_t)(DGRAD ? KStridedPlanes<64, 16>::BYTES : KContigPlanes<64, 16>::BYTES) + 3 * 512;
         hipLaunchKernelGGL((conv3x3s1_kernel<DGRAD>), grid, dim3(THREADS), lds_, st,
-                           X, W, bias, addend, dst, g, relu, splits > 1 ? (float*)nullptr : stats);
+                           X, W, bias, addend, dst, g, relu, kstats, out, tk);
     } else
     {
     if (t.bm == 128 && t.bn == 128) PHNET_LAUNCH_CONV(128, 128, false);
@@ -1360,7 +1375,7 @@
 #undef PHNET_LAUNCH_CONV__
 #undef PHNET_LAUNCH_CONV_
 #undef PHNET_LAUNCH_CONV
-    if (splits > 1) {
+    if (splits > 1 && !inkernel) {
         const long total4 = M * g.Co / 4;
         hipLaunchKernelGGL(splitk_reduce_kernel, dim3((unsigned)ceil_div64(total4, 256)), dim3(256), 0, st,
                            workspace, out, bias, addend, total4, g.Co, splits, relu, 0, stats);
@@ -1421,10 +1436,10 @@
     return PHNET_OK;
 }
 
-PHNET_API int phnet_conv2d_fwd(const float* x, const float* w, const float* bias, float* y,
-                               int32_t N, int32_t Hi, int32_t Wi, int32_t Ci, int32_t Co, int32_t R, int32_t S,
-                               int32_t stride, int32_t pad, int32_t relu,
-                               void* workspace, uint64_t ws_bytes, void* stream)
+PHNET_API int phnet_conv2d_fwd_tk(const float* x, const float* w, const float* bias, float* y,
+                                  int32_t N, int32_t Hi, int32_t Wi, int32_t Ci, int32_t Co, int32_t R, int32_t S,
+                                  int32_t stride, int32_t pad, int32_t relu,
+                                  void* workspace, uint64_t ws_bytes, void* stream, uint32_t* tickets, uint64_t tickets_cap)
 {
     if (N < 0 || Hi < 1 || Wi < 1 || Ci < 4 || Co < 4 || (Ci & 3) || (Co & 3) || R < 1 || S < 1 || stride < 1 || pad < 0)
         return PHNET_ERR_ARG;
@@ -1436,13 +1451,23 @@
     g.Wo = (Wi + 2 * pad - S) / stride + 1;
     if (g.Ho < 1 || g.Wo < 1) return PHNET_ERR_ARG;
     g.stride = stride; g.pad = pad; g.in_dil = 1;
-    return launch_conv<false>(x, w, bias, nullptr, y, (float*)workspace, ws_bytes, g, relu, (hipStream_t)stream);
-}
-
-static long conv_stats_blocks(long M, int Co, int K, bool has_ws, size_t ws_bytes)
+    return launch_conv<false>(x, w, bias, nullptr, y, (float*)workspace, ws_bytes, g, relu, (hipStream_t)stream, nullptr,
+                              (unsigned*)tickets, tickets_cap);
+}
+
+PHNET_API int phnet_conv2d_fwd(const float* x, const float* w, const float* bias, float* y,
+                               int32_t N, int32_t Hi, int32_t Wi, int32_t Ci, int32_t Co, int32_t R, int32_t S,
+                               int32_t stride, int32_t pad, int32_t relu,
+                               void* workspace, uint64_t ws_bytes, void* stream)
+{
+    return phnet_conv2d_fwd_tk(x, w, bias, y, N, Hi, Wi, Ci, Co, R, S, stride, pad, relu, workspace, ws_bytes, stream, nullptr, 0);
+}
+
+static long conv_stats_blocks(long M, int Co, int K, bool has_ws, size_t ws_bytes, uint64_t tickets_cap = 0)
 {
     const ConvPlan t = plan_conv(M, Co, K, has_ws, ws_bytes);
-    return t.splits > 1 ? ceil_div64(M * Co / 4, 256) : t.tiles / ceil_div64(Co, t.bn) * (t.bm / 32);
+    const bool reduce = t.splits > 1 && (uint64_t)t.tiles > tickets_cap;
+    return reduce ? ceil_div64(M * Co / 4, 256) : t.tiles / ceil_div64(Co, t.bn) * (t.bm / 32);
 }
 
 PHNET_API uint64_t phnet_conv2d_stats_blocks(int64_t M, int32_t Co, int32_t K, uint64_t ws_bytes)
@@ -1450,11 +1475,35 @@
     if (M < 1 || Co < 4 || K < 1) return 0;
     return (uint64_t)conv_stats_blocks((long)M, Co, K, ws_bytes > 0, (size_t)ws_bytes);
 }
+
+PHNET_API uint64_t phnet_conv2d_stats_blocks_tk(int64_t M, int32_t Co, int32_t K, uint64_t ws_bytes, uint64_t tickets_cap)
+{
+    if (M < 1 || Co < 4 || K < 1) return 0;
+    return (uint64_t)conv_stats_blocks((long)M, Co, K, ws_bytes > 0, (size_t)ws_bytes, tickets_cap);
+}
+
+PHNET_API int phnet_conv2d_fwd_fused_tk(const float* x, const float* w, const float* bias, const float* addend, float* y,
+                                        float* stats, int32_t N, int32_t Hi, int32_t Wi, int32_t Ci, int32_t Co, int32_t R,
+                                        int32_t S, int32_t stride, int32_t pad, int32_t relu,
+                                        void* workspace, uint64_t ws_bytes, void* stream, uint32_t* tickets, uint64_t tickets_cap);
+PHNET_API int phnet_conv2d_dgrad_tk(const float* dy, const float* w, const float* addend, float* dx,
+                                    int32_t N, int32_t Hi, int32_t Wi, int32_t Ci, int32_t Co, int32_t R, int32_t S,
+                                    int32_t stride, int32_t pad, void* workspace, uint64_t ws_bytes, void* stream,
+                                    uint32_t* tickets, uint64_t tickets_cap);
 
 PHNET_API int phnet_conv2d_fwd_fused(const float* x, const float* w, const float* bias, const float* addend, float* y, float* stats,
                                      int32_t N, int32_t Hi, int32_t Wi, int32_t Ci, int32_t Co, int32_t R, int32_t S,
                                      int32_t stride, int32_t pad, int32_t relu,
                                      void* workspace, uint64_t ws_bytes, void* stream)
+{
+    return phnet_conv2d_fwd_fused_tk(x, w, bias, addend, y, stats, N, Hi, Wi, Ci, Co, R, S, stride, pad, relu, workspace, ws_bytes,
+                                     stream, nullptr, 0);
+}
+
+PHNET_API int phnet_conv2d_fwd_fused_tk(const float* x, const float* w, const float* bias, const float* addend, float* y,
+                                        float* stats, int32_t N, int32_t Hi, int32_t Wi, int32_t Ci, int32_t Co, int32_t R,
+                                        int32_t S, int32_t stride, int32_t pad, int32_t relu,
+                                        void* workspace, uint64_t ws_bytes, void* stream, uint32_t* tickets, uint64_t tickets_cap)
 {
     if (N < 0 || Hi < 1 || Wi < 1 || Ci < 4 || Co < 4 || (Ci & 3) || (Co & 3) || R < 1 || S < 1 || stride < 1 || pad < 0)
         return PHNET_ERR_ARG;
@@ -1467,12 +1516,21 @@
     g.Wo = (Wi + 2 * pad - S) / stride + 1;
     if (g.Ho < 1 || g.Wo < 1) return PHNET_ERR_ARG;
     g.stride = stride; g.pad = pad; g.in_dil = 1;
-    return launch_conv<false>(x, w, bias, addend, y, (float*)workspace, ws_bytes, g, relu, (hipStream_t)stream, stats);
+    return launch_conv<false>(x, w, bias, addend, y, (float*)workspace, ws_bytes, g, relu, (hipStream_t)stream, stats,
+                              (unsigned*)tickets, tickets_cap);
 }
 
 PHNET_API int phnet_conv2d_dgrad(const float* dy, const float* w, const float* addend, float* dx,
                                  int32_t N, int32_t Hi, int32_t Wi, int32_t Ci, int32_t Co, int32_t R, int32_t S,
                                  int32_t stride, int32_t pad, void* workspace, uint64_t ws_bytes, void* stream)
+{
+    return phnet_conv2d_dgrad_tk(dy, w, addend, dx, N, Hi, Wi, Ci, Co, R, S, stride, pad, workspace, ws_bytes, stream, nullptr, 0);
+}
+
+PHNET_API int phnet_conv2d_dgrad_tk(const float* dy, const float* w, const float* addend, float* dx,
+                                    int32_t N, int32_t Hi, int32_t Wi, int32_t Ci, int32_t Co, int32_t R, int32_t S,
+                                    int32_t stride, int32_t pad, void* workspace, uint64_t ws_bytes, void* stream,
+                                    uint32_t* tickets, uint64_t tickets_cap)
 {
     if (N < 0 || Hi < 1 || Wi < 1 || Ci < 4 || Co < 4 || (Ci & 3) || (Co & 3) || R < 1 || S < 1 || stride < 1 || pad < 0)
         return PHNET_ERR_ARG;
@@ -1489,7 +1547,8 @@
     g.stride = 1; g.pad = R - 1 - pad; g.in_dil = stride;
     if (R != S && (S - 1 - pad) != g.pad) return PHNET_ERR_ARG;
     if (g.pad < 0) return PHNET_ERR_ARG;
-    return launch_conv<true>(dy, w, nullptr, addend, dx, (float*)workspace, ws_bytes, g, 0, (hipStream_t)stream);
+    return launch_conv<true>(dy, w, nullptr, addend, dx, (float*)workspace, ws_bytes, g, 0, (hipStream_t)stream, nullptr,
+                             (unsigned*)tickets, tickets_cap);
 }
 
 static long wgrad_splits(long P, long Co, long NC, int* bm_out)
diff --git a/phnet_amd/csrc/conv3p.hip b/phnet_amd/csrc/conv3p.hip
--- a/phnet_amd/csrc/conv3p.hip
+++ b/phnet_amd/csrc/conv3p.hip
@@ -1,4 +1,5 @@
 #include "igemm.h"
+#include "splitk.h"
 
 using namespace igemm;
 
@@ -16,6 +17,7 @@
 constexpr int P3_APLANE = (P3_ROWS + 1) * P3_APITCH, P3_AIMG = 3 * P3_APLANE;
 constexpr int P3_PFB = 3;
 constexpr size_t P3_LDS = 2 * P3_AIMG + 3 * 512;
+static_assert(P3_LDS >= splitk::LDS_BYTES, "the in-launch combine reuses the staging LDS");
 
 struct P3PackJob { const float* w; unsigned char* dst; int Co, Ci, dgrad, pad_; long first; };
 
@@ -72,7 +74,8 @@
 template <int FN>
 __global__ __launch_bounds__(P3_THREADS, FN == 1 ? 3 : 2) void conv3p_kernel(
     const float* __restrict__ X, const unsigned char* __restrict__ Bp, const float* __restrict__ bias,
-    const float* __restrict__ addend, float* __restrict__ out, P3Shape g, int relu, float* __restrict__ stats)
+    const float* __restrict__ addend, float* __restrict__ out, P3Shape g, int relu, float* __restrict__ stats,
+    float* y, unsigned* __restrict__ tickets)
 {
     extern __shared__ __attribute__((aligned(16))) float lds[];
     unsigned char* A3 = reinterpret_cast<unsigned char*>(lds);
@@ -247,6 +250,7 @@
         }
     }
     float* dst = out + (size_t)blockIdx.z * M * g.Nn;
+    const bool publish = !final_pass && tickets != nullptr;
 #pragma unroll
     for (int jn = 0; jn < FN; ++jn) {
         const int n = n0 + wn + 32 * jn + frag_col(lane);
@@ -255,9 +259,13 @@
 #pragma unroll
             for (int e = 0; e < 16; ++e) {
                 const int m = m0 + wm + 32 * f + frag_row(lane, e);
-                if (m < M) dst[(size_t)m * g.Nn + n] = (final_pass && relu) ? fmaxf(acc[f][jn][e], 0.f) : acc[f][jn][e];
+                if (m < M) splitk::store(dst + (size_t)m * g.Nn + n, (final_pass && relu) ? fmaxf(acc[f][jn][e], 0.f) : acc[f][jn][e], publish);
             }
     }
+    if (!final_pass && tickets != nullptr &&
+        splitk::last_arriver(tickets, tile, g.splits, reinterpret_cast<unsigned char*>(lds)))
+        splitk::combine_tile<P3_BM, BN, 64>(out, (size_t)M * g.Nn, y, bias, addend, M, g.Nn, m0, n0, g.splits, relu, stats,
+                                            reinterpret_cast<unsigned char*>(lds));
 }
 
 constexpr int P3_RCH = 4;
@@ -368,11 +376,29 @@
     return phnet_launch_status();
 }
 
+static bool p3_inkernel(const P3Plan& p, const uint32_t* tickets, uint64_t tickets_cap)
+{
+    return p.splits > 1 && tickets != nullptr && (uint64_t)p.tiles <= tickets_cap;
+}
+
+static uint64_t p3_stats_blocks(long M, int Ca, int Nn, size_t ws_bytes, bool inkernel_ok)
+{
+    if (!p3_applies(M, Ca, Nn)) return 0;
+    const P3Plan p = p3_plan(M, Ca, Nn, ws_bytes);
+    const bool reduce = p.splits > 1 && !inkernel_ok;
+    return (uint64_t)(reduce ? cdiv(M * Nn / 4, 256 * P3_RCH) : cdiv(M, P3_BM) * (P3_BM / 64));
+}
+
 PHNET_API uint64_t phnet_conv3p_stats_blocks(int64_t M, int32_t Ca, int32_t Nn, uint64_t ws_bytes)
+{
+    return p3_stats_blocks((long)M, Ca, Nn, (size_t)ws_bytes, false);
+}
+
+PHNET_API uint64_t phnet_conv3p_stats_blocks_tk(int64_t M, int32_t Ca, int32_t Nn, uint64_t ws_bytes, uint64_t tickets_cap)
 {
     if (!p3_applies((long)M, Ca, Nn)) return 0;
     const P3Plan p = p3_plan((long)M, Ca, Nn, (size_t)ws_bytes);
-    return (uint64_t)(p.splits > 1 ? cdiv((long)M * Nn / 4, 256 * P3_RCH) : cdiv((long)M, P3_BM) * (P3_BM / 64));
+    return p3_stats_blocks((long)M, Ca, Nn, (size_t)ws_bytes, (uint64_t)p.tiles <= tickets_cap);
 }
 
 PHNET_API int phnet_conv3p_splits(int64_t M, int32_t Ca, int32_t Nn, uint64_t ws_bytes)
@@ -389,9 +415,9 @@
     return PHNET_OK;
 }
 
-PHNET_API int phnet_conv3p_fwd(const float* x, const void* packed, const float* bias, const float* addend, float* y, float* stats,
-                               int32_t N, int32_t H, int32_t W, int32_t Ca, int32_t Nn, int32_t relu,
-                               void* workspace, uint64_t ws_bytes, void* stream)
+PHNET_API int phnet_conv3p_fwd_tk(const float* x, const void* packed, const float* bias, const float* addend, float* y, float* stats,
+                                  int32_t N, int32_t H, int32_t W, int32_t Ca, int32_t Nn, int32_t relu,
+                                  void* workspace, uint64_t ws_bytes, void* stream, uint32_t* tickets, uint64_t tickets_cap)
 {
     if (N < 0 || H < 1 || W < 2 || Ca < 16 || Nn < 64) return PHNET_ERR_ARG;
     if (N == 0) return PHNET_OK;
@@ -400,18 +426,28 @@
     if (stats && (bias || addend || relu || (Nn & (Nn - 1)) || Nn > 1024)) return PHNET_ERR_ARG;
     const P3Plan p = p3_plan(M, Ca, Nn, workspace ? (size_t)ws_bytes : 0);
     P3Shape g{N, H, W, Ca, Nn, p.splits, p.units_per_split};
+    const bool inkernel = p3_inkernel(p, tickets, tickets_cap);
     float* dst = p.splits > 1 ? (float*)workspace : y;
+    float* kstats = (p.splits == 1 || inkernel) ? stats : nullptr;
+    unsigned* tk = inkernel ? (unsigned*)tickets : nullptr;
     hipStream_t st = (hipStream_t)stream;
     if (p.fn == 2)
         hipLaunchKernelGGL(conv3p_kernel<2>, dim3((unsigned)p.tiles, 1, (unsigned)p.splits), dim3(P3_THREADS), P3_LDS, st,
-                           x, (const unsigned char*)packed, bias, addend, dst, g, relu, p.splits > 1 ? (float*)nullptr : stats);
+                           x, (const unsigned char*)packed, bias, addend, dst, g, relu, kstats, y, tk);
     else
         hipLaunchKernelGGL(conv3p_kernel<1>, dim3((unsigned)p.tiles, 1, (unsigned)p.splits), dim3(P3_THREADS), P3_LDS, st,
-                           x, (const unsigned char*)packed, bias, addend, dst, g, relu, p.splits > 1 ? (float*)nullptr : stats);
-    if (p.splits > 1) {
+                           x, (const unsigned char*)packed, bias, addend, dst, g, relu, kstats, y, tk);
+    if (p.splits > 1 && !inkernel) {
         const long total4 = M * Nn / 4;
         hipLaunchKernelGGL(conv3p_reduce_kernel, dim3((unsigned)cdiv(total4, stats ? 256 * P3_RCH : 256)), dim3(256), 0, st,
                            (const float*)workspace, y, bias, addend, total4, Nn, p.splits, relu, stats);
     }
     return phnet_launch_status();
 }
+
+PHNET_API int phnet_conv3p_fwd(const float* x, const void* packed, const float* bias, const float* addend, float* y, float* stats,
+                               int32_t N, int32_t H, int32_t W, int32_t Ca, int32_t Nn, int32_t relu,
+                               void* workspace, uint64_t ws_bytes, void* stream)
+{
+    return phnet_conv3p_fwd_tk(x, packed, bias, addend, y, stats, N, H, W, Ca, Nn, relu, workspace, ws_bytes, stream, nullptr, 0);
+}
diff --git a/phnet_amd/csrc/splitk.h b/phnet_amd/csrc/splitk.h
--- /dev/null
+++ b/phnet_amd/csrc/splitk.h
@@ -0,0 +1,112 @@
+#pragma once
+#include "igemm.h"
+
+namespace splitk {
+
+using igemm::f32x4;
+
+constexpr int SCRATCH_BYTES = 2 * 256 * 16;
+constexpr int LDS_BYTES = SCRATCH_BYTES + 16;
+
+__device__ __forceinline__ void store(float* p, float v, bool publish)
+{
+    if (publish) __hip_atomic_store(p, v, __ATOMIC_RELAXED, __HIP_MEMORY_SCOPE_AGENT);
+    else *p = v;
+}
+
+__device__ __forceinline__ bool last_arriver(unsigned* tickets, unsigned tile, int splits, unsigned char* lds)
+{
+    int* flag = reinterpret_cast<int*>(lds + SCRATCH_BYTES);
+    asm volatile("s_waitcnt vmcnt(0)" ::: "memory");
+    __syncthreads();
+    if (threadIdx.x == 0) {
+        const unsigned t = __hip_atomic_fetch_add(tickets + tile, 1u, __ATOMIC_RELAXED, __HIP_MEMORY_SCOPE_AGENT);
+        const int last = t == (unsigned)splits - 1u;
+        if (last) {
+            __builtin_amdgcn_fence(__ATOMIC_ACQUIRE, "agent");
+            asm volatile("s_waitcnt vmcnt(0)" ::: "memory");
+            __hip_atomic_store(tickets + tile, 0u, __ATOMIC_RELAXED, __HIP_MEMORY_SCOPE_AGENT);
+        }
+        *flag = last;
+    }
+    __syncthreads();
+    return __builtin_amdgcn_readfirstlane(*flag) != 0;
+}
+
+template <int BM, int BN, int SR>
+__device__ __forceinline__ void combine_tile(const float* part, size_t slab, float* out, const float* __restrict__ bias,
+                                             const float* addend, int M, int ncols, int m0, int n0, int splits, int relu,
+                                             float* __restrict__ stats, unsigned char* lds)
+{
+    constexpr int C4 = BN / 4, RP = 256 / C4, P = BM / RP;
+    constexpr int PC = P < 8 ? P : 8;
+    constexpr int G = BM / SR, PG = SR / RP;
+    static_assert(256 % C4 == 0 && BM % RP == 0 && SR % RP == 0 && BM % SR == 0 && P % PC == 0, "combine_tile shape");
+    const int tid = threadIdx.x, c = tid % C4, r = tid / C4;
+    const int n = n0 + 4 * c;
+    const bool nok = n < ncols;
+    const f32x4 zero{0.f, 0.f, 0.f, 0.f};
+    const f32x4 bv = (bias && nok) ? *reinterpret_cast<const f32x4*>(bias + n) : zero;
+    f32x4 sa[G], sb[G];
+#pragma unroll
+    for (int gi = 0; gi < G; ++gi) { sa[gi] = zero; sb[gi] = zero; }
+#pragma unroll
+    for (int p0 = 0; p0 < P; p0 += PC) {
+        size_t off[PC];
+        bool ok[PC];
+#pragma unroll
+        for (int p = 0; p < PC; ++p) {
+            const int m = m0 + r + RP * (p0 + p);
+            ok[p] = nok && m < M;
+            off[p] = ok[p] ? (size_t)m * ncols + n : 0;
+        }
+        f32x4 s[PC];
+#pragma unroll
+        for (int p = 0; p < PC; ++p) s[p] = *reinterpret_cast<const f32x4*>(part + off[p]);
+        for (int z = 1; z < splits; ++z) {
+            const float* pz = part + (size_t)z * slab;
+            f32x4 v[PC];
+#pragma unroll
+            for (int p = 0; p < PC; ++p) v[p] = *reinterpret_cast<const f32x4*>(pz + off[p]);
+#pragma unroll
+            for (int p = 0; p < PC; ++p) s[p] += v[p];
+        }
+        if (bias) {
+#pragma unroll
+            for (int p = 0; p < PC; ++p) s[p] += bv;
+        }
+        if (addend) {
+            f32x4 a[PC];
+#pragma unroll
+            for (int p = 0; p < PC; ++p) a[p] = *reinterpret_cast<const f32x4*>(addend + off[p]);
+#pragma unroll
+            for (int p = 0; p < PC; ++p) s[p] += a[p];
+        }
+#pragma unroll
+        for (int p = 0; p < PC; ++p) {
+            if (relu) { s[p].x = fmaxf(s[p].x, 0.f); s[p].y = fmaxf(s[p].y, 0.f); s[p].z = fmaxf(s[p].z, 0.f); s[p].w = fmaxf(s[p].w, 0.f); }
+            if (ok[p]) *reinterpret_cast<f32x4*>(out + off[p]) = s[p];
+            const f32x4 t = ok[p] ? s[p] : zero;
+            sa[(p0 + p) / PG] += t;
+            sb[(p0 + p) / PG] += t * t;
+        }
+    }
+    if (stats == nullptr) return;
+    f32x4* red = reinterpret_cast<f32x4*>(lds);
+#pragma unroll
+    for (int gi = 0; gi < G; ++gi) {
+        red[tid] = sa[gi];
+        red[256 + tid] = sb[gi];
+        __syncthreads();
+        if (tid < C4 && nok) {
+            f32x4 a = red[tid], b = red[256 + tid];
+            for (int rr = 1; rr < RP; ++rr) { a += red[rr * C4 + tid]; b += red[256 + rr * C4 + tid]; }
+            float* q = stats + ((size_t)(m0 / SR) + gi) * 2 * ncols + n;
+            *reinterpret_cast<f32x4*>(q) = a;
+            *reinterpret_cast<f32x4*>(q + ncols) = b;
+        }
+        __syncthreads();
+    }
+}
+
+}
diff --git a/phnet_amd/hip_ops.py b/phnet_amd/hip_ops.py
--- a/phnet_amd/hip_ops.py
+++ b/phnet_amd/hip_ops.py
@@ -77,6 +77,22 @@
         cur = torch.empty(max(int(nbytes), 1 << 20), dtype=torch.uint8, device=device)
         _WS[key] = cur
     return cur
+
+
+SPLITK_INKERNEL = os.environ.get("PHNET_SPLITK_INKERNEL", "1") != "0"
+_TICKETS = {}
+_TICKETS_CAP = 4096
+
+
+def tickets(device):
+    if not SPLITK_INKERNEL:
+        return None, 0
+    idx = torch.device(device).index
+    cur = _TICKETS.get(idx)
+    if cur is None:
+        cur = torch.zeros(_TICKETS_CAP, dtype=torch.int32, device=device)
+        _TICKETS[idx] = cur
+    return cur.data_ptr(), _TICKETS_CAP
 
 
 def lane_nms(rows: torch.Tensor, scores: torch.Tensor, thresh: float, top_k: int,
@@ -136,22 +152,23 @@
     need = 8 * n * ho * wo * co * 4 if n * ho * wo * co < (1 << 23) else 0
     ws = workspace(need, x.device) if need else None
     m, k = n * ho * wo, r * s * ci
+    tk, tk_cap = tickets(x.device)
     if addend is not None or stats:
         part, nblk = None, 0
         if stats:
-            nblk = int(lib().phnet_conv2d_stats_blocks(m, co, k, need))
+            nblk = int(lib().phnet_conv2d_stats_blocks_tk(m, co, k, need, tk_cap if tk else 0))
             part = workspace(nblk * 2 * co * 4, x.device, 1)
         if addend is not None:
             _req(addend, name="addend")
             assert addend.shape == out.shape
         _timed_launch(lambda: _gemm_symbol(m, co, k, need, False, ci, taps3=(r == 3 and s == 3 and stride == 1 and pad == 1)), 2.0 * m * co * k,
-                      lambda: check(lib().phnet_conv2d_fwd_fused(_ptr(x), _ptr(w), _ptr(bias), _ptr(addend), _ptr(out), _ptr(part), n, hi, wi,
-                                                                 ci, co, r, s, stride, pad, int(relu), _ptr(ws), need, _stream()),
-                                    "phnet_conv2d_fwd_fused"), shape=("fwd", m, co, k, r), nbytes=4.0 * (n * hi * wi * ci + m * co + co * k))
+                      lambda: check(lib().phnet_conv2d_fwd_fused_tk(_ptr(x), _ptr(w), _ptr(bias), _ptr(addend), _ptr(out), _ptr(part), n, hi,
+                                                                    wi, ci, co, r, s, stride, pad, int(relu), _ptr(ws), need, _stream(),
+                                                                    tk, tk_cap), "phnet_conv2d_fwd_fused_tk"), shape=("fwd", m, co, k, r), nbytes=4.0 * (n * hi * wi * ci + m * co + co * k))
         return (out, (part, nblk)) if stats else out
     _timed_launch(lambda: _gemm_symbol(m, co, k, need, False, ci, taps3=(r == 3 and s == 3 and stride == 1 and pad == 1)), 2.0 * m * co * k,
-                  lambda: check(lib().phnet_conv2d_fwd(_ptr(x), _ptr(w), _ptr(bias), _ptr(out), n, hi, wi, ci, co, r, s, stride,
-                                                       pad, int(relu), _ptr(ws), need, _stream()), "phnet_conv2d_fwd"),
+                  lambda: check(lib().phnet_conv2d_fwd_tk(_ptr(x), _ptr(w), _ptr(bias), _ptr(out), n, hi, wi, ci, co, r, s, stride,
+                                                          pad, int(relu), _ptr(ws), need, _stream(), tk, tk_cap), "phnet_conv2d_fwd_tk"),
                   shape=("fwd", m, co, k, r), nbytes=4.0 * (n * hi * wi * ci + m * co + co * k))
     return out
 
@@ -213,16 +230,17 @@
     need = 8 * m * nn * 4 if m * nn < (1 << 23) else 0
     ws = workspace(need, x.device) if need else None
     part, nblk = None, 0
+    tk, tk_cap = tickets(x.device)
     if stats:
-        nblk = int(lib().phnet_conv3p_stats_blocks(m, ca, nn, need))
+        nblk = int(lib().phnet_conv3p_stats_blocks_tk(m, ca, nn, need, tk_cap if tk else 0))
         part = workspace(nblk * 2 * nn * 4, x.device, 1)
     if addend is not None:
         _req(addend, name="addend")
         assert addend.shape == out.shape
     _timed_launch(lambda: (f"conv3p_kernel<{2 if (nn % 128 == 0 and m >= 16384) else 1}>", int(lib().phnet_conv3p_splits(m, ca, nn, need))),
                   2.0 * m * nn * 9 * ca,
-                  lambda: check(lib().phnet_conv3p_fwd(_ptr(x), _ptr(packed), _ptr(bias), _ptr(addend), _ptr(out), _ptr(part), n, h, w_, ca, nn,
-                                                       int(relu), _ptr(ws), need, _stream()), "phnet_conv3p_fwd"),
+                  lambda: check(lib().phnet_conv3p_fwd_tk(_ptr(x), _ptr(packed), _ptr(bias), _ptr(addend), _ptr(out), _ptr(part), n, h, w_, ca,
+                                                          nn, int(relu), _ptr(ws), need, _stream(), tk, tk_cap), "phnet_conv3p_fwd_tk"),
                   shape=("dgrad" if dgrad else "fwd", m, nn, 9 * ca, 3),
                   nbytes=4.0 * m * (ca + nn) + 6.0 * 9 * ca * nn + (4.0 * m * nn if addend is not None else 0.0))
     return (out, (part, nblk)) if stats else out
@@ -237,9 +255,10 @@
     need = 8 * n * hi * wi * ci * 4 if n * hi * wi * ci < (1 << 23) else 0
     ws = workspace(need, dy.device) if need else None
     m, k = n * hi * wi, r * s * co
+    tk, tk_cap = tickets(dy.device)
     _timed_launch(lambda: _gemm_symbol(m, ci, k, need, True, co, stride, taps3=(r == 3 and s == 3 and stride == 1 and pad == 1)), 2.0 * dy.shape[0] * dy.shape[1] * dy.shape[2] * co * r * s * ci,
-                  lambda: check(lib().phnet_conv2d_dgrad(_ptr(dy), _ptr(w), _ptr(addend), _ptr(dx), n, hi, wi, ci, co, r, s, stride,
-                                                         pad, _ptr(ws), need, _stream()), "phnet_conv2d_dgrad"),
+                  lambda: check(lib().phnet_conv2d_dgrad_tk(_ptr(dy), _ptr(w), _ptr(addend), _ptr(dx), n, hi, wi, ci, co, r, s, stride,
+                                                            pad, _ptr(ws), need, _stream(), tk, tk_cap), "phnet_conv2d_dgrad_tk"),
                   shape=("dgrad", m, ci, k, r), nbytes=4.0 * (dy.numel() + m * ci + co * r * s * ci))
     return dx
 
```
